# theEricMa/TriplaneTurbo

Hardware: AMD Instinct MI355X
Metric: rendered rays/sec (fwd+bwd) at 256x256 rays x 128 samples (higher is better)
Workload: dtype f32 (fp32-grade: exact 3-piece fp16 operand split, 6 x v_mfma_f32_32x32x16_f16 per k-step, fp32 accumulation)

## Files before the change

### include/tt_abi.h

```cpp
#ifndef TT_ABI_H
#define TT_ABI_H

#include <stdint.h>

#ifdef __cplusplus
extern "C" {
#endif

#define TT_ABI_VERSION 17
#define TT_CHANNELS 32
#define TT_HIDDEN 64

typedef enum {
    TT_OK = 0,
    TT_ERR_BAD_ARG = -1,
    TT_ERR_UNSUPPORTED = -2,
    TT_ERR_LAUNCH = -3,
    TT_ERR_DEVICE = -4
} tt_status;

typedef struct {
    const float* w1;
    const float* w2;
    const float* w3;
    const float* v1;
    const float* v2;
    const float* v3;
} tt_mlp_weights;

typedef struct {
    float* w1;
    float* w2;
    float* w3;
    float* v1;
    float* v2;
    float* v3;
} tt_mlp_grads;

typedef struct {
    int32_t n_prompts;
    int32_t views_per_prompt;
    int32_t plane_h, plane_w;
    int32_t rays_per_view;
    int32_t n_samples;
    int64_t n_rays;
    float radius;
    float sdf_bias_radius;
    float inv_std;
    float cos_anneal_ratio;
    float rgb_grad_shrink;
    int32_t flags;
    int32_t image_w;
    int32_t tile_sb;
    int32_t grad_copies;
    int32_t tile_chunk;
    float skip_eps_tex;
    float skip_eps_geo;
    const float* inv_std_dev;
    uint64_t* stats;
} tt_render_cfg;

#define TT_R_PER_SAMPLE 1
#define TT_R_EXACT_F32 2
#define TT_R_SPLIT2 32
#define TT_R_SPLIT3 64

#define TT_R_VOLSDF 128

#define TT_R_WGRAD_F32 4
#define TT_R_BWD_SOLO 8
#define TT_R_BWD_PAIR 16

#define TT_Q_NORMAL 1
#define TT_Q_TEX 2
#define TT_Q_EXACT_F32 4
#define TT_Q_SPLIT2 8
#define TT_Q_SPLIT3 16

const char* tt_strerror(int status);
int tt_abi_version(void);
const char* tt_source_hash(void);
int tt_debug_poison_queue(void* stream);

int tt_planes_pack(const float* space_cache, float* packed, int32_t n_prompts, int32_t plane_h, int32_t plane_w,
                   void* stream);
int tt_planes_unpack_grad(const float* grad_packed, float* grad_space_cache, int32_t n_prompts, int32_t plane_h,
                          int32_t plane_w, int32_t n_copies, void* stream);

int tt_query_points(const float* packed, const tt_mlp_weights* w, const float* points, int32_t n_batch,
                    int64_t n_points, int32_t n_prompts, int32_t views_per_prompt, int32_t plane_h, int32_t plane_w,
                    float radius, float sdf_bias_radius, int32_t flags, float* out_sdf, float* out_sdf_grad,
                    float* out_features, void* stream);

int tt_query_field(const float* packed, const tt_mlp_weights* w, const float* points, int32_t n_batch,
                   int64_t n_points, int32_t n_prompts, int32_t views_per_prompt, int32_t plane_h, int32_t plane_w,
                   float radius, float sdf_bias_radius, int32_t flags, float* out_sdf, float* out_deformation,
                   void* stream);

int tt_decode_rays(const float* packed, const tt_mlp_weights* w, const float* rays_o, const float* rays_d,
                   const float* t_starts, const float* t_ends, const tt_render_cfg* cfg, int32_t flags, float* sdf,
                   float* sdf_grad, float* features, void* stream);

enum tt_sample_placement { TT_PLACE_TT = 0, TT_PLACE_CENTER = 1 };
#define TT_PLACE_VOLSDF 0x100

int tt_sample_uniform(int64_t n_rays, int32_t n_samples, float near_plane, float far_plane, const float* jitter,
                      int32_t placement, float* t_starts, float* t_ends, void* stream);

int tt_sample_importance(const float* t_starts, const float* t_ends, const float* sdf, int64_t n_rays,
                         int32_t n_proposal, int32_t n_fine, float inv_std, const float* inv_std_dev,
                         float render_step_size, const float* u_jitter, int32_t placement, float* out_t_starts,
                         float* out_t_ends, void* stream);

int tt_render_fwd(const float* packed, const tt_mlp_weights* w, const float* rays_o, const float* rays_d,
                  const float* t_starts, const float* t_ends, const tt_render_cfg* cfg, float* opacity, float* depth,
                  float* rgb_fg, float* z_variance, float* normal_acc, float* weights, float* trans, float* sdf,
                  float* sdf_grad, float* features, void* stream);

int tt_render_fwd_h2mask(const float* packed, const tt_mlp_weights* w, const float* rays_o, const float* rays_d,
                         const float* t_starts, const float* t_ends, const tt_render_cfg* cfg, float* opacity,
                         float* depth, float* rgb_fg, float* z_variance, float* normal_acc, float* weights, float* trans,
                         float* sdf, float* sdf_grad, float* features, uint32_t* h2_mask, void* stream);

int tt_render_eval(const float* packed, const tt_mlp_weights* w, const float* rays_o, const float* rays_d,
                   const float* t_starts, const float* t_ends, const tt_render_cfg* cfg, float transmittance_eps,
                   float weight_eps, float* opacity, float* depth, float* rgb_fg, float* z_variance, float* normal_acc,
                   uint64_t* stats, void* stream);

int tt_march_fwd(const float* rays_d, const float* t_starts, const float* t_ends, const tt_render_cfg* cfg,
                 const float* sdf, const float* sdf_grad, const float* features, float* opacity, float* depth,
                 float* rgb_fg, float* z_variance, float* normal_acc, float* weights, float* trans, void* stream);

int tt_march_bwd(const float* rays_d, const float* t_starts, const float* t_ends, const tt_render_cfg* cfg,
                 const float* opacity, const float* depth, const float* trans, const float* sdf,
                 const float* sdf_grad, const float* features, const float* g_opacity, const float* g_depth,
                 const float* g_rgb_fg, const float* g_z_variance, const float* g_normal_acc, const float* g_weights,
                 const float* g_sdf, const float* g_sdf_grad, float* g_inv_std_rays, float* out_grad, void* stream);

int tt_render_bwd_geo(const float* packed, const tt_mlp_weights* w, const float* rays_o, const float* rays_d,
                      const float* t_starts, const float* t_ends, const tt_render_cfg* cfg, const float* opacity,
                      const float* depth, const float* trans, const float* sdf, const float* sdf_grad,
                      const float* features, const float* g_opacity, const float* g_depth, const float* g_rgb_fg,
                      const float* g_z_variance, const float* g_normal_acc, const float* g_weights,
                      const float* g_sdf, const float* g_sdf_grad, float* g_inv_std_rays, float* workspace,
                      float* grad_packed, const tt_mlp_grads* grads, void* stream);

int tt_render_bwd_geo_h2mask(const float* packed, const tt_mlp_weights* w, const float* rays_o, const float* rays_d,
                             const float* t_starts, const float* t_ends, const tt_render_cfg* cfg,
                             const float* opacity, const float* depth, const float* trans, const float* sdf,
                             const float* sdf_grad, const float* features, const float* g_opacity,
                             const float* g_depth, const float* g_rgb_fg, const float* g_z_variance,
                             const float* g_normal_acc, const float* g_weights, const float* g_sdf,
                             const float* g_sdf_grad, float* g_inv_std_rays, float* workspace, float* grad_packed,
                             const tt_mlp_grads* grads, const uint32_t* h2_mask, void* stream);

int tt_render_bwd_tex(const float* packed, const tt_mlp_weights* w, const float* rays_o, const float* rays_d,
                      const float* t_starts, const float* t_ends, const tt_render_cfg* cfg, const float* weights,
                      const float* features, const float* g_rgb_fg, const float* g_features, float* grad_packed,
                      const tt_mlp_grads* grads, void* stream);

int tt_points_bwd_geo(const float* packed, const tt_mlp_weights* w, const float* points, int32_t n_batch,
                      int64_t n_points, int32_t n_prompts, int32_t views_per_prompt, int32_t plane_h, int32_t plane_w,
                      float radius, float sdf_bias_radius, int32_t flags, const float* g_sdf, const float* g_sdf_grad,
                      float* workspace, float* grad_packed, const tt_mlp_grads* grads, void* stream);
int tt_points_bwd_tex(const float* packed, const tt_mlp_weights* w, const float* points, int32_t n_batch,
                      int64_t n_points, int32_t n_prompts, int32_t views_per_prompt, int32_t plane_h, int32_t plane_w,
                      float radius, int32_t plane_base, int32_t flags, const float* g_features, float* grad_packed,
                      const tt_mlp_grads* grads, void* stream);

int tt_points_bwd_x(const float* packed, const tt_mlp_weights* w, const float* points, int32_t n_batch,
                    int64_t n_points, int32_t n_prompts, int32_t views_per_prompt, int32_t plane_h, int32_t plane_w,
                    float radius, int32_t flags, const float* g_sdf, const float* g_sdf_grad, const float* g_features,
                    float* grad_points, void* stream);

typedef struct {
    int32_t n_levels;
    int32_t n_features_per_level;
    int32_t log2_hashmap_size;
    int32_t base_resolution;
    float per_level_scale;
} tt_hashgrid_cfg;
int64_t tt_hashgrid_n_params(const tt_hashgrid_cfg* cfg);
int tt_hashgrid_fwd(const float* x, int64_t n, const float* params, const tt_hashgrid_cfg* cfg, float* out,
                    void* stream);
int tt_hashgrid_bwd(const float* x, int64_t n, const float* g_out, const tt_hashgrid_cfg* cfg, float* grad_params,
                    void* stream);

int tt_patch_composite_fwd(const float* low, const float* patch, float* out, int32_t B, int32_t h, int32_t w, int32_t H,
                           int32_t W, int32_t C, int32_t PS, int32_t py, int32_t px, void* stream);
int tt_patch_composite_bwd(const float* g_out, float* g_low, float* g_patch, int32_t B, int32_t h, int32_t w, int32_t H,
                           int32_t W, int32_t C, int32_t PS, int32_t py, int32_t px, void* stream);

int tt_eikonal_fwd(const float* sdf_grad, int64_t n, float* loss, void* stream);
int tt_eikonal_bwd(const float* sdf_grad, const float* g_loss, int64_t n, float* g_sdf_grad, void* stream);

int tt_composite_fwd(const float* opacity, const float* depth, const float* rgb_fg, const float* normal_acc,
                     const float* bg, int32_t bg_stride, const float* camera_distances, const float* c2w, int64_t n_rays,
                     int32_t rays_per_view, int32_t mode, int32_t view_group, float* comp_rgb, float* disparity,
                     float* comp_normal, float* normal_cam_vis, float* normal_cam_vis_white, void* stream);
int tt_composite_bwd(const float* opacity, const float* depth, const float* rgb_fg, const float* normal_acc,
                     const float* bg, int32_t bg_stride, const float* camera_distances, const float* c2w, int64_t n_rays,
                     int32_t rays_per_view, int32_t mode, int32_t view_group, const float* g_comp_rgb,
                     const float* g_disparity, const float* g_comp_normal, const float* g_normal_cam_vis,
                     const float* g_normal_cam_vis_white, float* g_opacity, float* g_depth, float* g_rgb_fg,
                     float* g_normal_acc, float* g_bg, void* stream);

#define TT_DTYPE_F32 0
#define TT_DTYPE_F16 1
#define TT_DTYPE_F64 2
int tt_grid_sample_2d_grad2_typed(int32_t dtype, const void* grad2_grad_input, const void* grad2_grad_grid,
                                  const void* grad_output, const void* input, const void* grid, int32_t n, int32_t c,
                                  int32_t h, int32_t w, int64_t n_points_per_batch, int32_t padding_mode,
                                  int32_t align_corners, void* grad_grad_output, void* grad_input, void* grad_grid,
                                  void* stream);
int tt_grid_sample_2d_grad2(const float* grad2_grad_input, const float* grad2_grad_grid, const float* grad_output,
                            const float* input, const float* grid, int32_t n, int32_t c, int32_t h, int32_t w,
                            int64_t n_points_per_batch, int32_t padding_mode, int32_t align_corners,
                            float* grad_grad_output, float* grad_input, float* grad_grid, void* stream);

#define TT_MC_MAX_RES 512
int64_t tt_mc_workspace_bytes(int32_t res);
int tt_mc_count(const float* level, int32_t res, float isovalue, void* workspace, int32_t* out_totals, void* stream);
int tt_mc_emit(const float* level, const float* deformation, int32_t res, float isovalue, void* workspace, float* v_pos,
               int32_t* t_pos_idx, void* stream);
int tt_mc_bwd(const float* level, const float* deformation, int32_t res, float isovalue, void* workspace,
              const float* grad_v, float* grad_level, float* grad_deformation, void* stream);

int64_t tt_mt_workspace_bytes(int32_t n_edges, int32_t n_tets);
int tt_mt_count(const float* level, const int32_t* edges, const int32_t* tets, int32_t n_edges, int32_t n_tets,
                void* workspace, int32_t* out_totals, void* stream);
int tt_mt_emit(const float* pos, const float* level, const int32_t* edges, const int32_t* tet_edge, int32_t n_edges,
               int32_t n_tets, void* workspace, float* v_pos, int32_t* t_pos_idx, void* stream);
int tt_mt_bwd(const float* pos, const float* level, const int32_t* edges, const int32_t* vert_ptr,
              const int32_t* vert_col, int32_t n_vertices, int32_t n_edges, int32_t n_tets, void* workspace,
              const float* grad_v, float* grad_level, float* grad_pos, void* stream);

#define TT_RAST_MAX_TRIS (1 << 24)
int64_t tt_rast_workspace_bytes(int32_t B, int32_t T, int32_t H, int32_t W);
int tt_rast_fwd(const float* pos, const int32_t* tri, int32_t B, int32_t V, int32_t T, int32_t H, int32_t W,
                void* workspace, float* rast, void* stream);
int tt_rast_bwd(const float* pos, const int32_t* tri, const float* rast, const float* grad_rast, int32_t B, int32_t V,
                int32_t T, int32_t H, int32_t W, float* grad_pos, void* stream);
// ... 143 lines not shown
```

### triplaneturbo_amd/csrc/tt_backward.hip

```cpp
#include "tt_backward_common.h"

struct BwdGeoParams {
    const float* packed;
    MlpPtrs w;
    const float* rays_o;
    const float* rays_d;
    const float* t_starts;
    const float* t_ends;
    tt_render_cfg cfg;
    TileGeom geom;
    long long n_items;
    int* queue;
    const float* ws;
    const unsigned* h2_mask;
    int n_copies;
    float* grad_packed;
    MlpGradPtrs grads;
    unsigned long long* phase_cycles;
};

#define GEO_SCRATCH_FLOATS (2 * 64 * XS)
template <int PREC, bool FMASK>
struct GeoMap : LdsMap<PREC, LdsImage<64, 32>, LdsImage<64, 64, !(FMASK && PREC != PREC_F32)>, LdsRows<1, 64>,
                       LdsImage<32, 64>, LdsImage<64, 64>> {
// ... 177 lines not shown
                        wgrad16<64, 32>(accW1, Xs, Ys, i, hi);
                    } else {
                        stage_rows<64>(Xs, a1, i, hi);
                        stage_rows<32>(Ys, u, i, hi);
                        wgrad<64, 32>(accW1, Xs, Ys, i, hi);
                    }
                }
                TT_PHASE(7);
                float t1[32];
                mvx<PREC>(L, typename G::W1{}, qb, t1, i, hi);
#pragma unroll
                for (int r = 0; r < 32; ++r) t1[r] = h1[r] > 0.f ? t1[r] : 0.f;
                float v[32];
#pragma unroll
                for (int r = 0; r < 32; ++r) v[r] = fmaf(sbar * u1, h1[r], t1[r]);
                TT_PHASE(4);
                if (do_wgrad) {
                    if (WG16) {
                        stage_rows16_mask<64>(Xs, m2p, i, hi);
                        stage_rows16<64>(Ys, v, i, hi, sV);
                        wgrad16_mask<64, 64>(accW2, Xs, Ys, i, hi);
                    } else {
                        stage_rows_mask<64>(Xs, h2, i, hi);
                        stage_rows<64>(Ys, v, i, hi);
                        wgrad<64, 64>(accW2, Xs, Ys, i, hi);
                    }
                }
                TT_PHASE(8);
                if (region && !TT_DBG(cfg.flags, TT_DBG_NO_SCATTER)) {
                    scatter_clear<EXACT>(Xs, lane);
                    float* Qs = Xs + SCATTER_M_FLOATS;
                    TT_PHASE(9);
                    const int tex0 = (int)(pofs / TT_C);
                    auto corners = [&](int pl, PlaneRefs& refs) {
                        Corners c;
                        float coef[4];
                        geo_corner_coefs(pl, H, W, X, Y, Z, rvalid, sbar, gbx, gby, gbz, ju, jv, c, coef);
                        int aoff[4];
#pragma unroll
                        for (int q4 = 0; q4 < 4; ++q4) aoff[q4] = tex0 + (int)(pl * HW) + c.off[q4];
                        refs = plane_refs<!EXACT>(coef, aoff, c.hs, hi);
                    };
#ifdef TT_TUNING
                    unsigned long long* const sc_st = ph_acc + 14;
#else
                    unsigned long long* const sc_st = nullptr;
#endif
                    const ScatterQ<EXACT> sq{Qs, tags, i, hi};
                    if (one)
                        scatter_one_plane<EXACT>(grad_out, grad_bytes, sq, Xs, Qs + 32 * 33,
                                                 single_plane_index(pmask), corners, q, uq, sc_st);
                    else
                        scatter_planes<EXACT>(grad_out, grad_bytes, sq, Xs, Qs + 32 * 33, corners, [&](int) { return q; }, uq, sc_st);
                    TT_PHASE(10);
                }
            }
        }
    }
#ifdef TT_TUNING
    TT_PHASE(11);
    if (p.phase_cycles && lane == 0)
        for (int k = 0; k < 20; ++k) atomicAdd(p.phase_cycles + 20 + k, ph_acc[k]);
#endif
    __syncthreads();
    int parity = 0;
    flush_wgrad_reduced<64, 32>(L, parity, accW1, p.grads.w1, wave_in_blk, lane, 1.f / sA1, 1.f / sU);
    flush_d_reduced<64, 64>(L, parity, accW2, p.w.w2, p.w.w3, p.grads.w2, p.grads.w3, wave_in_blk, lane, 1.f / sV);
    tile_stats_flush(st);
}

#ifdef TT_TUNING
unsigned long long* g_phase_cycles = nullptr;
extern "C" int tt_tuning_phase_cycles(unsigned long long* out40) {
    if (!g_phase_cycles) {
        if (hipMalloc((void**)&g_phase_cycles, 40 * sizeof(unsigned long long)) != hipSuccess) return -4;
        if (hipMemset(g_phase_cycles, 0, 40 * sizeof(unsigned long long)) != hipSuccess) return -4;
    }
    if (hipDeviceSynchronize() != hipSuccess) return -4;
    if (out40 && hipMemcpy(out40, g_phase_cycles, 40 * sizeof(unsigned long long), hipMemcpyDeviceToHost) != hipSuccess)
        return -4;
    return hipMemset(g_phase_cycles, 0, 40 * sizeof(unsigned long long)) == hipSuccess ? 0 : -4;
}
#endif
static void launch_bwd_geo(const BwdGeoParams& p0, long long blocks, hipStream_t s) {
    BwdGeoParams p = p0;
#ifdef TT_TUNING
    p.phase_cycles = g_phase_cycles;
#else
    p.phase_cycles = nullptr;
#endif
    if (use_wg16(p.cfg)) {
        unsigned* bnd = reinterpret_cast<unsigned*>(p.queue) + TT_SLOT_BOUNDS;
        launch_planes_bound(p.packed, p.cfg, 0, bnd + TT_BOUND_PLANES, s);
        const long long n = p.cfg.n_rays * p.cfg.n_samples;
        hipLaunchKernelGGL(k_absmax4, dim3(absmax_blocks(n), 1), dim3(256), 0, s, reinterpret_cast<const f32x4*>(p.ws), n, n,
                           bnd + TT_BOUND_UP0, bnd + TT_BOUND_UP1);
    }
    tt_dispatch_prec(tt_prec_of_r(p.cfg.flags), [&](auto P) {
        constexpr int PREC = decltype(P)::value;
        const dim3 grid((unsigned)blocks), block(256);
        if (p.cfg.stats && p.h2_mask)
            hipLaunchKernelGGL((k_decode_bwd_geo<PREC, true, true>), grid, block, 0, s, p);
        else if (p.cfg.stats)
            hipLaunchKernelGGL((k_decode_bwd_geo<PREC, true>), grid, block, 0, s, p);
        else if (p.h2_mask)
            hipLaunchKernelGGL((k_decode_bwd_geo<PREC, false, true>), grid, block, 0, s, p);
        else
            hipLaunchKernelGGL((k_decode_bwd_geo<PREC>), grid, block, 0, s, p);
    });
}

static int render_bwd_geo(const float* packed, const tt_mlp_weights* w, const float* rays_o, const float* rays_d,
                          const float* t_starts, const float* t_ends, const tt_render_cfg* cfg, const float* opacity,
                          const float* depth, const float* trans, const float* sdf, const float* sdf_grad,
                          const float* features, const float* g_opacity, const float* g_depth, const float* g_rgb_fg,
                          const float* g_z_variance, const float* g_normal_acc, const float* g_weights,
                          const float* g_sdf, const float* g_sdf_grad, float* g_inv_std_rays, float* workspace,
                          float* grad_packed, const tt_mlp_grads* grads, const uint32_t* h2_mask, void* stream) {
    int st = tt_validate_cfg(cfg);
    if (st != TT_OK) return st;
    if (!packed || !w || !rays_o || !rays_d || !t_starts || !t_ends || !opacity || !depth || !trans || !sdf ||
        !sdf_grad || !features || !workspace || !grad_packed || !grads)
        return TT_ERR_BAD_ARG;
    if (!w->w1 || !w->w2 || !w->w3 || !grads->w1 || !grads->w2 || !grads->w3) return TT_ERR_BAD_ARG;
    if (grad_buffer_too_large(cfg)) return TT_ERR_UNSUPPORTED;
    int cus = tt_num_cus();
    if (cus <= 0) return TT_ERR_DEVICE;
    hipStream_t s = (hipStream_t)stream;
    st = tt_launch_march_bwd(rays_d, t_starts, t_ends, cfg, sdf, sdf_grad, features, trans, opacity, depth, g_opacity,
                             g_depth, g_rgb_fg, g_z_variance, g_normal_acc, g_weights, g_sdf, g_sdf_grad, g_inv_std_rays,
                             workspace, s);
    if (st != TT_OK) return st;
    BwdGeoParams p;
    tt_fill_rays(p, packed, w, rays_o, rays_d, t_starts, t_ends, *cfg);
    p.cfg.flags |= debug_flags();
    p.ws = workspace;
    p.h2_mask = h2_mask;
    p.grad_packed = grad_packed;
    p.n_copies = cfg->grad_copies > 0 ? cfg->grad_copies : 1;
    p.grads = to_gptrs(grads);
    st = tt_plan_queue(cfg, 4LL * cus, s, &p.geom, &p.n_items, &p.queue);
    if (st != TT_OK) return st;
    launch_bwd_geo(p, tt_persistent_blocks(p.n_items, cus, 4), s);
    return tt_check_launch();
}

extern "C" int tt_render_bwd_geo(const float* packed, const tt_mlp_weights* w, const float* rays_o,
                                 const float* rays_d, const float* t_starts, const float* t_ends,
                                 const tt_render_cfg* cfg, const float* opacity, const float* depth,
                                 const float* trans, const float* sdf, const float* sdf_grad, const float* features,
                                 const float* g_opacity, const float* g_depth, const float* g_rgb_fg,
                                 const float* g_z_variance, const float* g_normal_acc, const float* g_weights,
                                 const float* g_sdf, const float* g_sdf_grad, float* g_inv_std_rays, float* workspace,
                                 float* grad_packed, const tt_mlp_grads* grads, void* stream) {
    return render_bwd_geo(packed, w, rays_o, rays_d, t_starts, t_ends, cfg, opacity, depth, trans, sdf, sdf_grad, features,
                          g_opacity, g_depth, g_rgb_fg, g_z_variance, g_normal_acc, g_weights, g_sdf, g_sdf_grad,
                          g_inv_std_rays, workspace, grad_packed, grads, nullptr, stream);
}

extern "C" int tt_render_bwd_geo_h2mask(const float* packed, const tt_mlp_weights* w, const float* rays_o,
                                        const float* rays_d, const float* t_starts, const float* t_ends,
                                        const tt_render_cfg* cfg, const float* opacity, const float* depth,
                                        const float* trans, const float* sdf, const float* sdf_grad,
                                        const float* features, const float* g_opacity, const float* g_depth,
                                        const float* g_rgb_fg, const float* g_z_variance, const float* g_normal_acc,
                                        const float* g_weights, const float* g_sdf, const float* g_sdf_grad,
                                        float* g_inv_std_rays, float* workspace, float* grad_packed,
                                        const tt_mlp_grads* grads, const uint32_t* h2_mask, void* stream) {
    if (!h2_mask) return TT_ERR_BAD_ARG;
    return render_bwd_geo(packed, w, rays_o, rays_d, t_starts, t_ends, cfg, opacity, depth, trans, sdf, sdf_grad, features,
                          g_opacity, g_depth, g_rgb_fg, g_z_variance, g_normal_acc, g_weights, g_sdf, g_sdf_grad,
                          g_inv_std_rays, workspace, grad_packed, grads, h2_mask, stream);
}

__global__ void k_interleave_ws(const float* __restrict__ g_sdf, const float* __restrict__ g_sdf_grad,
                                float* __restrict__ ws, long long n) {
    const long long i = (long long)blockIdx.x * blockDim.x + threadIdx.x;
    if (i >= n) return;
    f32x4 o = {g_sdf ? g_sdf[i] : 0.f, g_sdf_grad ? g_sdf_grad[i * 3 + 0] : 0.f,
               g_sdf_grad ? g_sdf_grad[i * 3 + 1] : 0.f, g_sdf_grad ? g_sdf_grad[i * 3 + 2] : 0.f};
    *reinterpret_cast<f32x4*>(ws + i * 4) = o;
}

extern "C" int tt_points_bwd_geo(const float* packed, const tt_mlp_weights* w, const float* points, int32_t n_batch,
                                 int64_t n_points, int32_t n_prompts, int32_t views_per_prompt, int32_t plane_h,
                                 int32_t plane_w, float radius, float sdf_bias_radius, int32_t flags,
                                 const float* g_sdf, const float* g_sdf_grad, float* workspace, float* grad_packed,
                                 const tt_mlp_grads* grads, void* stream) {
    tt_render_cfg cfg;
    int st = points_cfg(&cfg, n_batch, n_points, n_prompts, views_per_prompt, plane_h, plane_w, radius,
                        sdf_bias_radius, 1, flags);
    if (st != TT_OK) return st;
    if (grad_buffer_too_large(&cfg)) return TT_ERR_UNSUPPORTED;
    if (!packed || !w || !points || !workspace || !grad_packed || !grads || (!g_sdf && !g_sdf_grad))
        return TT_ERR_BAD_ARG;
    if (!w->w1 || !w->w2 || !w->w3 || !grads->w1 || !grads->w2 || !grads->w3) return TT_ERR_BAD_ARG;
    int cus = tt_num_cus();
    if (cus <= 0) return TT_ERR_DEVICE;
    hipStream_t s = (hipStream_t)stream;
    const long long n = cfg.n_rays;
    hipLaunchKernelGGL(k_interleave_ws, dim3((unsigned)((n + 255) / 256)), dim3(256), 0, s, g_sdf, g_sdf_grad,
                       workspace, n);
    st = tt_check_launch();
    if (st != TT_OK) return st;
    BwdGeoParams p;
    tt_fill_rays(p, packed, w, points, nullptr, nullptr, nullptr, cfg);
    p.ws = workspace;
    p.h2_mask = nullptr;
    p.grad_packed = grad_packed;
    p.n_copies = 1;
    p.grads = to_gptrs(grads);
    st = tt_plan_queue(&cfg, 4LL * cus, s, &p.geom, &p.n_items, &p.queue);
    if (st != TT_OK) return st;
    launch_bwd_geo(p, tt_persistent_blocks(p.n_items, cus, 4), s);
    return tt_check_launch();
}
```

### triplaneturbo_amd/csrc/tt_backward_common.h

```cpp
#pragma once
#include "tt_device.h"
#include "tt_mfma16.h"
#include "tt_alpha.h"
#include "tt_launch.h"
#include <type_traits>

typedef int i32x4 __attribute__((ext_vector_type(4)));

#ifdef TT_TUNING
#define TT_PHASE(k)                                              \
    do {                                                         \
        __builtin_amdgcn_sched_barrier(0);                       \
        const unsigned long long t_now = __builtin_amdgcn_s_memtime(); \
        ph_acc[k] += t_now - ph_t;                               \
        ph_t = t_now;                                            \
        __builtin_amdgcn_sched_barrier(0);                       \
    } while (0)
#else
#define TT_PHASE(k) \
    do {            \
    } while (0)
#endif
#define XS 36

// ... 697 lines not shown
    float* const Qs = sq.Qs;
    const int i = sq.i, hi = sq.hi;
    const ScatterCtx cx = scatter_ctx<EXACT>(grad, grad_bytes, sq, Ls);
    typename std::conditional<EXACT, ScA32, ScA16>::type A;
    typename std::conditional<EXACT, ScB32, ScB16>::type B;
    PlaneRefs rc;
    corners(pl, rc);
    sq.hand_over(pl, tile, factor, rc.qs);
    const Sc2State sc = sc2_claim_rank(rc, cx.htab, cx.ctag, cx.cdump, cx.dummy, cx.lane, st);
    scatter_lost(rc, sc.l0, sc.l1, Qs, Ls, cx.grsrc, i, hi, [&]() { sq.stage_q(pl, tile); });
    m_store<EXACT>(M, sc2_row_a(sc.rx0), cx.mc, rc.c0);
    m_store<EXACT>(M, sc2_row_a(sc.rx1), cx.mc, rc.c1);
    const bool pass_b = sc.n > 64;
    f32x16 acc0, acc1;
    sc2_load_a(M, i, hi, sc.n, A);
    m_zero<EXACT>(M, sc2_row_a(sc.rx0), cx.mc);
    m_zero<EXACT>(M, sc2_row_a(sc.rx1), cx.mc);
    if (pass_b) {
        m_store<EXACT>(M, sc2_row_b(sc.rx0), cx.mc, rc.c0);
        m_store<EXACT>(M, sc2_row_b(sc.rx1), cx.mc, rc.c1);
    }
    sq.load_b(pl, tile, B);
    sc2_split_b(B);
    sc2_gemm(A, B, sc.n, acc0, acc1);
    if (pass_b) {
        sc2_flush(acc0, acc1, cx.ctag, 64, cx.grsrc, cx.lane_b, hi);
        sc2_load_a(M, i, hi, sc.n - 64, A);
        m_zero<EXACT>(M, sc2_row_b(sc.rx0), cx.mc);
        m_zero<EXACT>(M, sc2_row_b(sc.rx1), cx.mc);
        sc2_gemm(A, B, sc.n - 64, acc0, acc1);
        sc2_flush(acc0, acc1, cx.ctag + 64, sc.n - 64, cx.grsrc, cx.lane_b, hi);
    } else {
        sc2_flush(acc0, acc1, cx.ctag, sc.n, cx.grsrc, cx.lane_b, hi);
    }
}

struct BwdTexParams {
    const float* packed;
    MlpPtrs w;
    const float* rays_o;
    const float* rays_d;
    const float* t_starts;
    const float* t_ends;
    tt_render_cfg cfg;
    const float* weights;
    const float* features;
    const float* g_rgb;
    const float* g_features;
    TileGeom geom;
    long long n_items;
    int* queue;
    int n_copies;
    float* grad_packed;
    MlpGradPtrs grads;
    unsigned long long* phase_cycles;
};

static inline bool grad_buffer_too_large(const tt_render_cfg* cfg) {
    return (long long)cfg->n_prompts * 6 * cfg->plane_h * cfg->plane_w * TT_C * 4 >= (1LL << 32) - 256;
}

#ifdef TT_TUNING
extern unsigned long long* g_phase_cycles;
#endif
static __global__ __launch_bounds__(256) void k_absmax4(const f32x4* __restrict__ x, long long seg4, long long seg_stride4,
                                                 unsigned* __restrict__ out0, unsigned* __restrict__ out1) {
    const f32x4* seg = x + (long long)blockIdx.y * seg_stride4;
    const long long stride = (long long)gridDim.x * blockDim.x;
    float m0 = 0.f, m1 = 0.f;
    long long e = (long long)blockIdx.x * blockDim.x + threadIdx.x;
    for (; e + 3 * stride < seg4; e += 4 * stride) {
        const f32x4 a = seg[e], b = seg[e + stride], c = seg[e + 2 * stride], d = seg[e + 3 * stride];
        m0 = fmaxf(fmaxf(m0, __builtin_fabsf(a[0])), fmaxf(__builtin_fabsf(b[0]), fmaxf(__builtin_fabsf(c[0]), __builtin_fabsf(d[0]))));
#pragma unroll
        for (int k = 1; k < 4; ++k)
            m1 = fmaxf(fmaxf(m1, __builtin_fabsf(a[k])), fmaxf(__builtin_fabsf(b[k]), fmaxf(__builtin_fabsf(c[k]), __builtin_fabsf(d[k]))));
    }
    for (; e < seg4; e += stride) {
        const f32x4 v = seg[e];
        m0 = fmaxf(m0, __builtin_fabsf(v[0]));
        m1 = fmaxf(m1, fmaxf(__builtin_fabsf(v[1]), fmaxf(__builtin_fabsf(v[2]), __builtin_fabsf(v[3]))));
    }
    if (!out1) m0 = fmaxf(m0, m1);
    __shared__ unsigned w[2];
    if (threadIdx.x < 2) w[threadIdx.x] = 0u;
    __syncthreads();
    for (int o = 32; o > 0; o >>= 1) {
        m0 = fmaxf(m0, __shfl_xor(m0, o));
        m1 = fmaxf(m1, __shfl_xor(m1, o));
    }
    if ((threadIdx.x & 63) == 0) {
        atomicMax(&w[0], __builtin_bit_cast(unsigned, m0));
        atomicMax(&w[1], __builtin_bit_cast(unsigned, m1));
    }
    __syncthreads();
    if (threadIdx.x == 0) {
        if (w[0] > __hip_atomic_load(out0, __ATOMIC_RELAXED, __HIP_MEMORY_SCOPE_AGENT)) atomicMax(out0, w[0]);
        if (out1 && w[1] > __hip_atomic_load(out1, __ATOMIC_RELAXED, __HIP_MEMORY_SCOPE_AGENT)) atomicMax(out1, w[1]);
    }
}
static __global__ __launch_bounds__(256) void k_absmax1(const float* __restrict__ x, long long n, unsigned* __restrict__ out) {
    float m = 0.f;
    for (long long e = (long long)blockIdx.x * blockDim.x + threadIdx.x; e < n; e += (long long)gridDim.x * blockDim.x)
        m = fmaxf(m, __builtin_fabsf(x[e]));
    for (int o = 32; o > 0; o >>= 1) m = fmaxf(m, __shfl_xor(m, o));
    __shared__ unsigned w;
    if (threadIdx.x == 0) w = 0u;
    __syncthreads();
    if ((threadIdx.x & 63) == 0) atomicMax(&w, __builtin_bit_cast(unsigned, m));
    __syncthreads();
    if (threadIdx.x == 0 && w > __hip_atomic_load(out, __ATOMIC_RELAXED, __HIP_MEMORY_SCOPE_AGENT)) atomicMax(out, w);
}
static inline unsigned absmax_blocks(long long n) {
    long long b = (n + 256 * 8 - 1) / (256 * 8);
    return (unsigned)(b < 1 ? 1 : (b > 1024 ? 1024 : b));
}
static inline void launch_planes_bound(const float* packed, const tt_render_cfg& cfg, int first_plane, unsigned* out,
                                hipStream_t s) {
    const long long hw4 = (long long)cfg.plane_h * cfg.plane_w * TT_C / 4;
    hipLaunchKernelGGL(k_absmax4, dim3(absmax_blocks(3 * hw4), (unsigned)cfg.n_prompts), dim3(256), 0, s,
                       reinterpret_cast<const f32x4*>(packed) + first_plane * hw4, 3 * hw4, 6 * hw4, out,
                       (unsigned*)nullptr);
}

static inline bool use_wg16(const tt_render_cfg& cfg) { return !(cfg.flags & TT_R_EXACT_F32); }

static inline int points_cfg(tt_render_cfg* c, int32_t n_batch, int64_t n_points, int32_t n_prompts,
                      int32_t views_per_prompt, int32_t plane_h, int32_t plane_w, float radius, float sdf_bias_radius,
                      int32_t grad_copies, int32_t q_flags) {
    if (!tt_points_counts_ok(n_batch, n_points, n_prompts, views_per_prompt, q_flags) || n_points > 0x7fffffffLL)
        return TT_ERR_BAD_ARG;
    c->n_prompts = n_prompts;
    c->views_per_prompt = views_per_prompt;
    c->plane_h = plane_h;
    c->plane_w = plane_w;
    c->rays_per_view = (int32_t)n_points;
    c->n_samples = 1;
    c->n_rays = (int64_t)n_batch * n_points;
    c->radius = radius;
    c->sdf_bias_radius = sdf_bias_radius;
    c->inv_std = 1.f;
    c->inv_std_dev = nullptr;
    c->stats = nullptr;
    c->cos_anneal_ratio = 1.f;
    c->rgb_grad_shrink = 1.f;
    c->flags = (q_flags & TT_Q_EXACT_F32) ? TT_R_EXACT_F32 : ((q_flags & TT_Q_SPLIT2) ? TT_R_SPLIT2 : 0);
    c->image_w = 0;
    c->tile_sb = 1;
    c->tile_chunk = 0;
    c->grad_copies = grad_copies;
    c->skip_eps_tex = 0.f;
    c->skip_eps_geo = 0.f;
    return tt_validate_cfg(c);
}
```

### triplaneturbo_amd/csrc/tt_backward_tex.hip

```cpp
#include "tt_backward_common.h"

#define TEX_SCRATCH_FLOATS (128 * XS)
template <int PREC>
struct TexMap : LdsMap<PREC, LdsImage<64, 96>, LdsImage<64, 64>, LdsRows<3, 64>, LdsImage<96, 64, PREC != PREC_S3>,
                       LdsImage<64, 64, PREC != PREC_S3>> {
    static constexpr bool COPIES = PREC != PREC_S3;
    typedef typename TexMap::template at<0> V1;
    typedef typename TexMap::template at<1> V2;
    typedef typename TexMap::template at<2> V3;
    typedef typename TexMap::template at<3> V1T;
    typedef typename TexMap::template at<4> V2T;
};
__device__ __forceinline__ float uniform_f(float v) {
    return __builtin_bit_cast(float, __builtin_amdgcn_readfirstlane(__builtin_bit_cast(int, v)));
}

template <int PREC, bool STATS = false>
__global__ __launch_bounds__(256, 1) void k_decode_bwd_tex(BwdTexParams p) {
    constexpr bool EXACT = PREC == PREC_F32;
    constexpr bool WG16 = !EXACT;
    typedef TexMap<PREC> F;
    constexpr int NT = PrecNT<PREC>::value, WF = F::FLOATS;
    __shared__ __attribute__((aligned(16))) float Lt[WF + 4 * (TEX_SCRATCH_FLOATS + SCATTER_TAG_INTS)];
    stage_weights<PREC>(Lt, typename F::V1{}, p.w.v1);
// ... 251 lines not shown
                wgrad16<64, 64>(accV2, Xs, Xs + 64 * XS, i, hi);
            } else {
                stage_rows<64>(Xs, k2, i, hi);
                stage_rows<64>(Xs + 64 * XS, k1, i, hi);
                wgrad<64, 64>(accV2, Xs, Xs + 64 * XS, i, hi);
            }
            TT_PHASE(8);
        }
        if (region && !TT_DBG(cfg.flags, TT_DBG_NO_SCATTER)) {
            float* M = Xs;
            float* Es = Xs + (EXACT ? 65 * XS : SCATTER_M_FLOATS);
            scatter_clear<EXACT>(M, lane);
            const int tex0 = (int)(pofs / TT_C);
            float eb[48], ueb = 1.f;
            if constexpr (EXACT)
                mvtx_copy<PREC>(Lt, typename F::V1T{}, typename F::V1{}, kb1, eb, i, hi);
            else if constexpr (F::COPIES)
                mvtx_copy<PREC, true, true>(Lt, typename F::V1T{}, typename F::V1{}, kb1, eb, i, hi, 1.f, &ueb);
            else
                mvtx<PREC, true, true>(Lt, typename F::V1{}, kb1, eb, i, hi, 1.f, &ueb);
            TT_PHASE(9);
            auto corners = [&](int pl, PlaneRefs& refs) {
                Corners c;
                corners_setup(PLANE_U(pl, X, Y, Z), PLANE_V(pl, X, Y, Z), H, W, valid, c);
                int aoff[4];
#pragma unroll
                for (int q4 = 0; q4 < 4; ++q4)
                    aoff[q4] = tex0 + (int)((3 + pl) * HW) + c.off[q4];
                refs = plane_refs<!EXACT>(c.w, aoff, c.hs, hi);
            };
#ifdef TT_TUNING
            unsigned long long* const sc_st = scat_st;
#else
            unsigned long long* const sc_st = nullptr;
#endif
            const ScatterQ<EXACT> sq{Es, tags, i, hi};
            if (one) {
                float eb1[16];
#pragma unroll
                for (int r = 0; r < 16; ++r) eb1[r] = pl1 == 0 ? eb[r] : (pl1 == 1 ? eb[16 + r] : eb[32 + r]);
                scatter_one_plane<EXACT>(grad_out, grad_bytes, sq, M, Es + 32 * 33, pl1, corners, eb1, ueb, sc_st);
                TT_PHASE(10);
                continue;
            }
            scatter_planes<EXACT>(grad_out, grad_bytes, sq, M, Es + 32 * 33, corners, [&](int pl) { return eb + 16 * pl; }, ueb,
                                  sc_st);
            TT_PHASE(10);
        }
      }
    }
#ifdef TT_TUNING
    TT_PHASE(11);
    ph_acc[15] = scat_st[0];
    ph_acc[16] = scat_st[1];
    if (p.phase_cycles && lane == 0)
        for (int k = 0; k < 20; ++k) atomicAdd(p.phase_cycles + k, ph_acc[k]);
#endif
    __syncthreads();
    int parity = 0;
    {
        const float u1 = 1.f / sKB1, u2 = 1.f / sE;
#pragma unroll
        for (int m = 0; m < 2; ++m) {
            float* const base = p.grads.v1 + (32 * m) * 96 + i;
            flush_tile_reduced(Lt, parity, accV1a[m][0], wave_in_blk, lane, u1, u2,
                               [&](int r) { return base + LIDX(r, hi) * 96; });
            parity ^= 1;
            flush_tile_reduced(Lt, parity, accV1a[m][1], wave_in_blk, lane, u1, u2,
                               [&](int r) { return base + LIDX(r, hi) * 96 + 32; });
            parity ^= 1;
            flush_tile_reduced(Lt, parity, accV1b[m][0], wave_in_blk, lane, u1, u2,
                               [&](int r) { return base + LIDX(r, hi) * 96 + 64; });
            parity ^= 1;
        }
    }
    flush_wgrad_reduced<64, 64>(Lt, parity, accV2, p.grads.v2, wave_in_blk, lane, 1.f / sK2B, 1.f / sK1);
#pragma unroll
    for (int h2 = 0; h2 < 2; ++h2)
#pragma unroll
        for (int o = 0; o < 3; ++o) atomicAdd(p.grads.v3 + o * 64 + 32 * h2 + i, accV3[h2][o]);
    tile_stats_flush(st);
}

static void launch_bwd_tex(const BwdTexParams& p0, long long blocks, hipStream_t s) {
    BwdTexParams p = p0;
#ifdef TT_TUNING
    p.phase_cycles = g_phase_cycles;
#else
    p.phase_cycles = nullptr;
#endif
    if (use_wg16(p.cfg)) {
        unsigned* bnd = reinterpret_cast<unsigned*>(p.queue) + TT_SLOT_BOUNDS;
        launch_planes_bound(p.packed, p.cfg, 3, bnd + TT_BOUND_PLANES, s);
        if (p.g_rgb)
            hipLaunchKernelGGL(k_absmax1, dim3(absmax_blocks(p.cfg.n_rays * 3)), dim3(256), 0, s, p.g_rgb,
                               (long long)p.cfg.n_rays * 3, bnd + TT_BOUND_UP0);
        if (p.g_features) {
            const long long n = p.cfg.n_rays * p.cfg.n_samples * 3;
            hipLaunchKernelGGL(k_absmax1, dim3(absmax_blocks(n)), dim3(256), 0, s, p.g_features, n, bnd + TT_BOUND_UP1);
        }
    }
    tt_dispatch_prec(tt_prec_of_r(p.cfg.flags), [&](auto P) {
        constexpr int PREC = decltype(P)::value;
        if (p.cfg.stats)
            hipLaunchKernelGGL((k_decode_bwd_tex<PREC, true>), dim3((unsigned)blocks), dim3(256), 0, s, p);
        else
            hipLaunchKernelGGL((k_decode_bwd_tex<PREC>), dim3((unsigned)blocks), dim3(256), 0, s, p);
    });
}

extern "C" int tt_render_bwd_tex(const float* packed, const tt_mlp_weights* w, const float* rays_o,
                                 const float* rays_d, const float* t_starts, const float* t_ends,
                                 const tt_render_cfg* cfg, const float* weights, const float* features,
                                 const float* g_rgb_fg, const float* g_features, float* grad_packed,
                                 const tt_mlp_grads* grads, void* stream) {
    int st = tt_validate_cfg(cfg);
    if (st != TT_OK) return st;
    if (!packed || !w || !rays_o || !rays_d || !t_starts || !t_ends || !weights || !features || !grad_packed ||
        !grads)
        return TT_ERR_BAD_ARG;
    if (!w->v1 || !w->v2 || !w->v3 || !grads->v1 || !grads->v2 || !grads->v3) return TT_ERR_BAD_ARG;
    if (grad_buffer_too_large(cfg)) return TT_ERR_UNSUPPORTED;
    int cus = tt_num_cus();
    if (cus <= 0) return TT_ERR_DEVICE;
    hipStream_t s = (hipStream_t)stream;
    BwdTexParams p;
    tt_fill_rays(p, packed, w, rays_o, rays_d, t_starts, t_ends, *cfg);
    p.cfg.flags |= debug_flags();
    p.weights = weights;
    p.features = features;
    p.g_rgb = g_rgb_fg;
    p.g_features = g_features;
    p.grad_packed = grad_packed;
    p.n_copies = cfg->grad_copies > 0 ? cfg->grad_copies : 1;
    p.grads = to_gptrs(grads);
    st = tt_plan_queue(cfg, 4LL * cus, s, &p.geom, &p.n_items, &p.queue, 12);
    if (st != TT_OK) return st;
    launch_bwd_tex(p, tt_persistent_blocks(p.n_items, cus, 4), s);
    return tt_check_launch();
}

extern "C" int tt_points_bwd_tex(const float* packed, const tt_mlp_weights* w, const float* points, int32_t n_batch,
                                 int64_t n_points, int32_t n_prompts, int32_t views_per_prompt, int32_t plane_h,
                                 int32_t plane_w, float radius, int32_t plane_base, int32_t flags,
                                 const float* g_features, float* grad_packed, const tt_mlp_grads* grads,
                                 void* stream) {
    tt_render_cfg cfg;
    int st = points_cfg(&cfg, n_batch, n_points, n_prompts, views_per_prompt, plane_h, plane_w, radius, 0.5f, 1,
                        flags);
    if (st != TT_OK) return st;
    if (grad_buffer_too_large(&cfg)) return TT_ERR_UNSUPPORTED;
    if (!packed || !w || !points || !g_features || !grad_packed || !grads) return TT_ERR_BAD_ARG;
    if (!w->v1 || !w->v2 || !w->v3 || !grads->v1 || !grads->v2 || !grads->v3) return TT_ERR_BAD_ARG;
    if (plane_base != 0 && plane_base != 3) return TT_ERR_BAD_ARG;
    int cus = tt_num_cus();
    if (cus <= 0) return TT_ERR_DEVICE;
    const ptrdiff_t shift = (ptrdiff_t)(plane_base - 3) * plane_h * plane_w * TT_C;
    hipStream_t s = (hipStream_t)stream;
    BwdTexParams p;
    tt_fill_rays(p, packed + shift, w, points, nullptr, nullptr, nullptr, cfg);
    p.weights = nullptr;
    p.features = nullptr;
    p.g_rgb = nullptr;
    p.g_features = g_features;
    p.grad_packed = grad_packed + shift;
    p.n_copies = 1;
    p.grads = to_gptrs(grads);
    st = tt_plan_queue(&cfg, 4LL * cus, s, &p.geom, &p.n_items, &p.queue);
    if (st != TT_OK) return st;
    launch_bwd_tex(p, tt_persistent_blocks(p.n_items, cus, 4), s);
    return tt_check_launch();
}
```

### triplaneturbo_amd/csrc/tt_device.h

```cpp
#pragma once
#include <hip/hip_runtime.h>
#include <stdint.h>

typedef float f32x16 __attribute__((ext_vector_type(16)));
typedef float f32x4 __attribute__((ext_vector_type(4)));

#ifdef TT_TUNING
#define TT_DBG(flags, bit) (((flags) & (bit)) != 0)
#else
#define TT_DBG(flags, bit) false
#endif
#define TT_DBG_NO_SCATTER 0x100
#define TT_DBG_NO_WGRAD 0x200
#define TT_DBG_NO_GATHER 0x400
#define TT_DBG_NO_MLP 0x800
#define TT_DBG_NO_STORE 0x1000
#define TT_DBG_NO_ATOMICS 0x2000

#define TT_C 32
#define TT_TILE 32

#define LIDX(r, hi) (((r) & 3) + 8 * ((r) >> 2) + 4 * (hi))

#include "tt_mask.h"

struct MlpPtrs {
    const float* w1;
    const float* w2;
    const float* w3;
    const float* v1;
    const float* v2;
    const float* v3;
};

__device__ __forceinline__ void lds_load_matrix(float* dst, const float* __restrict__ src, int rows, int cols,
                                                int stride) {
    for (int e = threadIdx.x; e < rows * cols; e += blockDim.x) {
        int r = e / cols, c = e - r * cols;
        dst[r * stride + c] = src[e];
    }
}

template <int NOUT, int NIN>
__device__ __forceinline__ void mv_fwd(const float* Wl, const float (&x)[NIN / 2], float (&y)[NOUT / 2], int i,
                                       int hi) {
    constexpr int MT = NOUT / 32;
    f32x16 acc[MT];
    f32x4 a_cur[MT], a_nxt[MT];
    const float* row = Wl + i * (NIN + 4) + 4 * hi;
#pragma unroll
    for (int m = 0; m < MT; ++m) {
        acc[m] = f32x16{0.f, 0.f, 0.f, 0.f, 0.f, 0.f, 0.f, 0.f, 0.f, 0.f, 0.f, 0.f, 0.f, 0.f, 0.f, 0.f};
        a_cur[m] = *reinterpret_cast<const f32x4*>(row + 32 * m * (NIN + 4));
    }
#pragma unroll
    for (int g = 0; g < NIN / 8; ++g) {
        if (g + 1 < NIN / 8) {
#pragma unroll
            for (int m = 0; m < MT; ++m)
                a_nxt[m] = *reinterpret_cast<const f32x4*>(row + 32 * m * (NIN + 4) + 8 * (g + 1));
        }
#pragma unroll
        for (int k = 0; k < 4; ++k)
#pragma unroll
            for (int m = 0; m < MT; ++m)
                acc[m] = __builtin_amdgcn_mfma_f32_32x32x2f32(a_cur[m][k], x[4 * g + k], acc[m], 0, 0, 0);
#pragma unroll
        for (int m = 0; m < MT; ++m) a_cur[m] = a_nxt[m];
    }
#pragma unroll
    for (int m = 0; m < MT; ++m)
#pragma unroll
        for (int k = 0; k < 16; ++k) y[16 * m + k] = acc[m][k];
}

template <int NOUT, int NIN, int NG>
__device__ __forceinline__ void mv_fwd_cols(const float* Wl, const float (&x)[4 * NG], int g0, float (&y)[NOUT / 2], int i,
                                            int hi) {
    constexpr int MT = NOUT / 32;
    f32x16 acc[MT];
    const float* row = Wl + i * (NIN + 4) + 4 * hi + 8 * g0;
#pragma unroll
    for (int m = 0; m < MT; ++m)
        acc[m] = f32x16{0.f, 0.f, 0.f, 0.f, 0.f, 0.f, 0.f, 0.f, 0.f, 0.f, 0.f, 0.f, 0.f, 0.f, 0.f, 0.f};
#pragma unroll
    for (int g = 0; g < NG; ++g) {
        f32x4 a[MT];
#pragma unroll
        for (int m = 0; m < MT; ++m) a[m] = *reinterpret_cast<const f32x4*>(row + 32 * m * (NIN + 4) + 8 * g);
#pragma unroll
        for (int k = 0; k < 4; ++k)
#pragma unroll
            for (int m = 0; m < MT; ++m)
                acc[m] = __builtin_amdgcn_mfma_f32_32x32x2f32(a[m][k], x[4 * g + k], acc[m], 0, 0, 0);
    }
#pragma unroll
    for (int m = 0; m < MT; ++m)
#pragma unroll
        for (int k = 0; k < 16; ++k) y[16 * m + k] = acc[m][k];
}

template <int NOUT, int NIN, int STRIDE = NOUT + 4>
__device__ __forceinline__ void mv_bwd(const float* Wl, const float (&x)[NIN / 2], float (&y)[NOUT / 2], int i,
                                       int hi) {
    constexpr int MT = NOUT / 32;
    const float* base = Wl + 4 * hi * STRIDE + i;
    if (MT == 1) {
// ... 648 lines not shown
```

### triplaneturbo_amd/csrc/tt_forward.hip

```cpp
#ifndef TT_MV16_FENCE
#define TT_MV16_FENCE 1
#endif
#include "tt_device.h"
#include "tt_mfma16.h"
#include "tt_alpha.h"
#include "tt_launch.h"

__device__ __forceinline__ void rot_dst(int k3, int y, int x, int H, int W, int& h, int& w) {
    if (k3 == 0) {
        h = x;
        w = y;
    } else if (k3 == 1) {
        h = H - 1 - y;
        w = W - 1 - x;
    } else {
        h = x;
        w = H - 1 - y;
    }
}

template <bool UNPACK>
__global__ __launch_bounds__(256) void k_planes_pack(const float* __restrict__ src, float* __restrict__ dst, int H,
                                                     int W, int n_copies, size_t copy_stride) {
    extern __shared__ float tile[];
    const int y = blockIdx.x, plane = blockIdx.y;
    const int k3 = plane % 3;
    const size_t HW = (size_t)H * W;
    const float* nchw_c = (UNPACK ? dst : src) + (size_t)plane * TT_C * HW;
    float* nchw = const_cast<float*>(nchw_c);
    const float* nhwc_c = (UNPACK ? src : dst) + (size_t)plane * HW * TT_C;
    float* nhwc = const_cast<float*>(nhwc_c);
    const int ws = W + 1;
    if (!UNPACK) {
        for (int e = threadIdx.x; e < TT_C * W; e += blockDim.x) {
            int c = e / W, x = e - c * W;
            tile[c * ws + x] = nchw[(size_t)c * HW + (size_t)y * W + x];
        }
        __syncthreads();
        for (int e = threadIdx.x; e < TT_C * W; e += blockDim.x) {
            int x = e >> 5, c = e & 31, h, w;
            rot_dst(k3, y, x, H, W, h, w);
            nhwc[((size_t)h * W + w) * TT_C + c] = tile[c * ws + x];
        }
    } else {
        for (int e = threadIdx.x; e < TT_C * W; e += blockDim.x) {
            int x = e >> 5, c = e & 31, h, w;
            rot_dst(k3, y, x, H, W, h, w);
            const size_t o = ((size_t)h * W + w) * TT_C + c;
            float acc = nhwc[o];
            for (int k = 1; k < n_copies; ++k) acc += nhwc[o + (size_t)k * copy_stride];
            tile[c * ws + x] = acc;
        }
        __syncthreads();
        for (int e = threadIdx.x; e < TT_C * W; e += blockDim.x) {
            int c = e / W, x = e - c * W;
            nchw[(size_t)c * HW + (size_t)y * W + x] = tile[c * ws + x];
        }
    }
}

__host__ __device__ inline int pack4_row_stride(int W) { return W + (36 - W % 32) % 32; }
template <bool UNPACK>
__global__ __launch_bounds__(256) void k_planes_pack4(const float* __restrict__ src, float* __restrict__ dst, int H,
                                                      int W, int n_copies, size_t copy_stride) {
    extern __shared__ __attribute__((aligned(16))) float tile[];
    const int y = blockIdx.x, plane = blockIdx.y;
    const int k3 = plane % 3;
    const size_t HW = (size_t)H * W;
    const float* nchw_c = (UNPACK ? dst : src) + (size_t)plane * TT_C * HW + (size_t)y * W;
    float* nchw = const_cast<float*>(nchw_c);
    const float* nhwc_c = (UNPACK ? src : dst) + (size_t)plane * HW * TT_C;
    float* nhwc = const_cast<float*>(nhwc_c);
    const int RS = pack4_row_stride(W), W4 = W >> 2;
    const int c_lane = threadIdx.x & 31, x4_0 = threadIdx.x >> 5;
    if (!UNPACK) {
        for (int e4 = threadIdx.x; e4 < TT_C * W4; e4 += 256) {
            const int c = e4 / W4, x4 = e4 - c * W4;
            *reinterpret_cast<f32x4*>(tile + c * RS + 4 * x4) =
                *reinterpret_cast<const f32x4*>(nchw_c + (size_t)c * HW + 4 * x4);
        }
        __syncthreads();
        for (int x4 = x4_0; x4 < W4; x4 += 8) {
            const f32x4 v = *reinterpret_cast<const f32x4*>(tile + c_lane * RS + 4 * x4);
#pragma unroll
            for (int j = 0; j < 4; ++j) {
                int h, w;
                rot_dst(k3, y, 4 * x4 + j, H, W, h, w);
                nhwc[((size_t)h * W + w) * TT_C + c_lane] = v[j];
            }
        }
    } else {
        for (int x4 = x4_0; x4 < W4; x4 += 8) {
            f32x4 v;
#pragma unroll
            for (int j = 0; j < 4; ++j) {
                int h, w;
                rot_dst(k3, y, 4 * x4 + j, H, W, h, w);
                const size_t o = ((size_t)h * W + w) * TT_C + c_lane;
                float acc = nhwc_c[o];
                for (int k = 1; k < n_copies; ++k) acc += nhwc_c[o + (size_t)k * copy_stride];
                v[j] = acc;
            }
            *reinterpret_cast<f32x4*>(tile + c_lane * RS + 4 * x4) = v;
        }
        __syncthreads();
        for (int e4 = threadIdx.x; e4 < TT_C * W4; e4 += 256) {
            const int c = e4 / W4, x4 = e4 - c * W4;
            *reinterpret_cast<f32x4*>(nchw + (size_t)c * HW + 4 * x4) =
                *reinterpret_cast<const f32x4*>(tile + c * RS + 4 * x4);
        }
    }
}

template <int PREC>
using FwdMap = DecodeMap<PREC, 96>;

struct DecodeCfg {
    const float* planes;
    unsigned tex0;
    float* T;
    int H, W;
    float radius;
    float ju, jv;
    int dbg;
    TileStats st = {nullptr};
};


template <int PREC>
__device__ __forceinline__ void decode_tex_fwd(const float* L, const DecodeCfg& dc, float X, float Y, float Z,
                                               bool valid, int i, int hi, float (&c)[3]) {
    typedef FwdMap<PREC> F;
    c[0] = c[1] = c[2] = 0.f;
    float e[48];
    unsigned pmask;
    bool any = gather_tex_cp(dc.planes, dc.tex0, dc.H, dc.W, X, Y, Z, valid, 32 * hi + i, dc.T, e, pmask);
    if (TT_DBG(dc.dbg, TT_DBG_NO_MLP)) {
        float t = 0.f;
#pragma unroll
        for (int r = 0; r < 48; ++r) t += e[r];
        c[0] = c[1] = c[2] = t;
    } else if (__any(any)) {
        float k1[32], k2[32], u1, u2;
        if (single_plane(pmask)) {
            tile_stat(dc.st, TT_STAT_SINGLE);
            float e1[16];
            live_block16(e, e1);
            mvx_plane<PREC, true>(L, typename F::V1{}, e1, single_plane_index(pmask), k1, i, hi, &u1);
        } else {
            mvx<PREC, true>(L, typename F::V1{}, e, k1, i, hi, 1.f, &u1);
        }
#pragma unroll
        for (int r = 0; r < 32; ++r) k1[r] = fmaxf(k1[r], 0.f);
        mvx<PREC, true>(L, typename F::V2{}, k1, k2, i, hi, u1, &u2);
#pragma unroll
        for (int r = 0; r < 32; ++r) k2[r] = fmaxf(k2[r], 0.f);
#pragma unroll
        for (int o = 0; o < 3; ++o) c[o] = dot_lds<64>(lds_at(L, typename F::V3{}) + 64 * o, k2, hi) * u2;
    }
}

__device__ __forceinline__ unsigned sign_mask32(const float (&h)[32]) {
    unsigned m = 0u;
#pragma unroll
    for (int g = 3; g >= 0; --g)
        asm("v_cmp_lt_f32 vcc, 0, %8\n\tv_addc_co_u32 %0, vcc, %0, %0, vcc\n\t"
            "v_cmp_lt_f32 vcc, 0, %7\n\tv_addc_co_u32 %0, vcc, %0, %0, vcc\n\t"
            "v_cmp_lt_f32 vcc, 0, %6\n\tv_addc_co_u32 %0, vcc, %0, %0, vcc\n\t"
            "v_cmp_lt_f32 vcc, 0, %5\n\tv_addc_co_u32 %0, vcc, %0, %0, vcc\n\t"
            "v_cmp_lt_f32 vcc, 0, %4\n\tv_addc_co_u32 %0, vcc, %0, %0, vcc\n\t"
            "v_cmp_lt_f32 vcc, 0, %3\n\tv_addc_co_u32 %0, vcc, %0, %0, vcc\n\t"
            "v_cmp_lt_f32 vcc, 0, %2\n\tv_addc_co_u32 %0, vcc, %0, %0, vcc\n\t"
            "v_cmp_lt_f32 vcc, 0, %1\n\tv_addc_co_u32 %0, vcc, %0, %0, vcc"
// ... 391 lines not shown
            }
            const float X = scale_coord(px, dc.radius), Y = scale_coord(py, dc.radius), Z = scale_coord(pz, dc.radius);
            const float livef = ray_okf * (__builtin_fabsf(T) < p.eps_T ? 0.f : 1.f);
            const bool live = livef != 0.f;
            {
                float s0, gq[3];
                decode_geo_fwd<true, PREC>(L, dc, X, Y, Z, live, i, hi, s0, gq);
                ++n_geo;
                float nrm;
                long long rr = ray;
                asm volatile("" : "+v"(rr));
                const float* ro = p.rays_o + rr * 3;
                const float* rd = p.rays_d + rr * 3;
                const float ts = p.t_starts[rr * S + si], te = p.t_ends[rr * S + si];
                dt = te - ts;
                const float ox = ro[0], oy = ro[1], oz = ro[2];
                const float dx = rd[0], dy = rd[1], dz = rd[2];
                sample_position(ox, oy, oz, dx, dy, dz, ts, te, tm, px, py, pz);
                sdf = s0 + sphere_bias(px, py, pz, cfg.sdf_bias_radius, nrm);
                const float gx = gq[0] + px / nrm, gy = gq[1] + py / nrm, gz = gq[2] + pz / nrm;
                const float gn = fmaxf(sqrtf(gx * gx + gy * gy + gz * gz), 1e-12f);
                const float ign = rcp_(gn);
                ux = gx * ign, uy = gy * ign, uz = gz * ign;
                cosv = dx * ux + dy * uy + dz * uz;
            }
            float alpha = (cfg.flags & TT_R_VOLSDF) ? volsdf_alpha_terms(sdf, dt, kstd).alpha
                                                    : neus_alpha_terms(sdf, cosv, dt, kstd, cfg.cos_anneal_ratio).alpha;
            if (!live) alpha = 0.f;
            const float wgt = alpha * T;
            T *= 1.f - alpha;
            acc0 = fmaf(wgt, lof, acc0);
            acc1 = fmaf(wgt * lof, tm, acc1);
            acc2 = fmaf(wgt * lof * tm, tm, acc2);
            acc3 = fmaf(wgt, hi ? uz : ux, acc3);
            acc4 = fmaf(wgt * lof, uy, acc4);
            const bool want_tex = __builtin_fabsf(wgt) > p.eps_w;
            if (__any(want_tex)) {
                float c[3];
                if constexpr (PREC == PREC_F32) {
                    long long rr = ray;
                    asm volatile("" : "+v"(rr));
                    const float* ro = p.rays_o + rr * 3;
                    const float* rd = p.rays_d + rr * 3;
                    float tm2, qx, qy, qz;
                    sample_position(ro[0], ro[1], ro[2], rd[0], rd[1], rd[2], p.t_starts[rr * S + si], p.t_ends[rr * S + si], tm2,
                                    qx, qy, qz);
                    decode_tex_fwd<PREC>(L, dc, scale_coord(qx, dc.radius), scale_coord(qy, dc.radius),
                                         scale_coord(qz, dc.radius), want_tex, i, hi, c);
                } else {
                    decode_tex_fwd<PREC>(L, dc, X, Y, Z, want_tex, i, hi, c);
                }
                ++n_tex;
                if (want_tex) {
                    const float wh = wgt * hif;
                    acc0 = fmaf(wh, sigmoid_(c[0]) * 1.002f - 0.001f, acc0);
                    acc1 = fmaf(wh, sigmoid_(c[1]) * 1.002f - 0.001f, acc1);
                    acc2 = fmaf(wh, sigmoid_(c[2]) * 1.002f - 0.001f, acc2);
                }
            }
            if (p.eps_T > 0.f && !__any(ray_okf * (__builtin_fabsf(T) < p.eps_T ? 0.f : 1.f) != 0.f)) break;
        }
        if (ray_ok) {
            if (hi == 0) {
                const float op = acc0, dep = acc1, wt2 = acc2;
                p.opacity[ray] = op;
                p.depth[ray] = dep;
                p.z_var[ray] = wt2 - 2.f * dep * dep + dep * dep * op;
                p.nacc[ray * 3 + 0] = acc3;
                p.nacc[ray * 3 + 1] = acc4;
            } else {
                p.rgb_fg[ray * 3 + 0] = acc0;
                p.rgb_fg[ray * 3 + 1] = acc1;
                p.rgb_fg[ray * 3 + 2] = acc2;
                p.nacc[ray * 3 + 2] = acc3;
            }
        }
    }
    if (p.stats && lane == 0) {
        atomicAdd(p.stats + 0, n_geo);
        atomicAdd(p.stats + 1, n_tex);
    }
}

extern "C" int tt_planes_pack(const float* space_cache, float* packed, int32_t n_prompts, int32_t plane_h,
                              int32_t plane_w, void* stream) {
    if (!space_cache || !packed || n_prompts <= 0 || plane_h <= 0 || plane_w <= 0) return TT_ERR_BAD_ARG;
    if (plane_h != plane_w) return TT_ERR_UNSUPPORTED;
    dim3 grid(plane_h, n_prompts * 6);
    if (plane_w % 4 == 0 && ((uintptr_t)space_cache & 15) == 0) {
        size_t lds = (size_t)TT_C * pack4_row_stride(plane_w) * sizeof(float);
        hipLaunchKernelGGL(k_planes_pack4<false>, grid, dim3(256), lds, (hipStream_t)stream, space_cache, packed,
                           plane_h, plane_w, 1, (size_t)0);
    } else {
        size_t lds = (size_t)TT_C * (plane_w + 1) * sizeof(float);
        hipLaunchKernelGGL(k_planes_pack<false>, grid, dim3(256), lds, (hipStream_t)stream, space_cache, packed,
                           plane_h, plane_w, 1, (size_t)0);
    }
    return tt_check_launch();
}

extern "C" int tt_planes_unpack_grad(const float* grad_packed, float* grad_space_cache, int32_t n_prompts,
                                     int32_t plane_h, int32_t plane_w, int32_t n_copies, void* stream) {
    if (!grad_packed || !grad_space_cache || n_prompts <= 0 || plane_h <= 0 || plane_w <= 0 || n_copies <= 0)
        return TT_ERR_BAD_ARG;
    if (plane_h != plane_w) return TT_ERR_UNSUPPORTED;
    dim3 grid(plane_h, n_prompts * 6);
    const size_t copy_stride = (size_t)n_prompts * 6 * plane_h * plane_w * TT_C;
    if (plane_w % 4 == 0 && ((uintptr_t)grad_space_cache & 15) == 0) {
        size_t lds = (size_t)TT_C * pack4_row_stride(plane_w) * sizeof(float);
        hipLaunchKernelGGL(k_planes_pack4<true>, grid, dim3(256), lds, (hipStream_t)stream, grad_packed,
                           grad_space_cache, plane_h, plane_w, n_copies, copy_stride);
    } else {
        size_t lds = (size_t)TT_C * (plane_w + 1) * sizeof(float);
        hipLaunchKernelGGL(k_planes_pack<true>, grid, dim3(256), lds, (hipStream_t)stream, grad_packed,
                           grad_space_cache, plane_h, plane_w, n_copies, copy_stride);
    }
    return tt_check_launch();
}

extern "C" int tt_query_points(const float* packed, const tt_mlp_weights* w, const float* points, int32_t n_batch,
                               int64_t n_points, int32_t n_prompts, int32_t views_per_prompt, int32_t plane_h,
                               int32_t plane_w, float radius, float sdf_bias_radius, int32_t flags, float* out_sdf,
                               float* out_sdf_grad, float* out_features, void* stream) {
    if (!packed || !w || !points) return TT_ERR_BAD_ARG;
    const int st = tt_validate_points(n_batch, n_points, n_prompts, views_per_prompt, plane_h, plane_w, radius, flags);
    if (st != TT_OK) return st;
    const bool need_n = (flags & TT_Q_NORMAL) != 0, need_t = (flags & TT_Q_TEX) != 0;
    if (!w->w1 || !w->w2 || !w->w3 || (need_t && (!w->v1 || !w->v2 || !w->v3))) return TT_ERR_BAD_ARG;
    QueryParams p;
    tt_fill_points(p, packed, w, points, n_batch, n_points, views_per_prompt, plane_h, plane_w, radius);
    p.bias_radius = sdf_bias_radius;
    p.out_sdf = out_sdf;
    p.out_grad = out_sdf_grad;
    p.out_feat = out_features;
    const int cus = tt_num_cus();
    if (cus <= 0) return TT_ERR_DEVICE;
    const dim3 grid = tt_point_blocks(n_points, n_batch, DECODE_THREADS / 64, cus);
    tt_dispatch(tt_prec_of_q(flags), need_n, need_t, [&](auto P, auto N, auto T) {
        hipLaunchKernelGGL((k_query_points<decltype(N)::value, decltype(T)::value, decltype(P)::value>), grid,
                           dim3(DECODE_THREADS), 0, (hipStream_t)stream, p);
    });
    return tt_check_launch();
}

bool tt_planes_too_large(long long n_prompts, int plane_h, int plane_w) {
    return n_prompts * 6 * plane_h * plane_w * TT_C * 4 >= (1LL << 32);
}

int tt_validate_cfg(const tt_render_cfg* cfg) {
    if (!cfg) return TT_ERR_BAD_ARG;
    if (cfg->n_prompts <= 0 || cfg->views_per_prompt <= 0 || cfg->rays_per_view <= 0 || cfg->n_samples <= 0 ||
        cfg->n_rays <= 0)
        return TT_ERR_BAD_ARG;
    if (cfg->n_rays != (int64_t)cfg->n_prompts * cfg->views_per_prompt * cfg->rays_per_view) return TT_ERR_BAD_ARG;
    if (cfg->plane_h <= 0 || cfg->plane_h != cfg->plane_w) return TT_ERR_UNSUPPORTED;
    if (tt_planes_too_large(cfg->n_prompts, cfg->plane_h, cfg->plane_w)) return TT_ERR_UNSUPPORTED;
    if (!(cfg->radius > 0.f) || (!cfg->inv_std_dev && !(cfg->inv_std > 0.f))) return TT_ERR_BAD_ARG;
    if (cfg->flags < 0) return TT_ERR_BAD_ARG;
    {
        const int pbits = cfg->flags & (TT_R_EXACT_F32 | TT_R_SPLIT2 | TT_R_SPLIT3);
        if (pbits & (pbits - 1)) return TT_ERR_BAD_ARG;
    }
    if (cfg->flags & (TT_R_BWD_PAIR | TT_R_WGRAD_F32)) return TT_ERR_UNSUPPORTED;
    if (!(cfg->skip_eps_tex >= 0.f) || !(cfg->skip_eps_geo >= 0.f)) return TT_ERR_BAD_ARG;
    return TT_OK;
}

long long tt_make_geom(const tt_render_cfg* cfg, long long wave_slots, TileGeom* g, int default_order,
                       int steps_per_item, int min_items_per_slot) {
    g->n_rays = cfg->n_rays;
    g->rays_per_view = cfg->rays_per_view;
    g->n_samples = cfg->n_samples;
    g->image_w = 0;
    g->image_h = 0;
    g->bpr = g->bpv = 0;
    int sb = cfg->tile_sb;
#ifdef TT_TUNING
    if (const char* e = getenv("TT_SB")) sb = atoi(e);
#endif
    if (!(sb == 1 || sb == 2 || sb == 4 || sb == 8 || sb == 16 || sb == 32)) sb = 2;
    while (sb > 1 && sb > cfg->n_samples) sb /= 2;
    g->sb = sb;
    static const int BW[6] = {8, 4, 4, 2, 2, 1}, BH[6] = {4, 4, 2, 2, 1, 1};
    int l2 = 0;
    while ((1 << l2) < sb) ++l2;
    g->bw = BW[l2];
    g->bh = BH[l2];
    const int rb = 32 / sb;
    long long n_blocks;
    if (cfg->image_w > 0 && cfg->rays_per_view % cfg->image_w == 0) {
        g->image_w = cfg->image_w;
        g->image_h = cfg->rays_per_view / cfg->image_w;
        g->bpr = (g->image_w + g->bw - 1) / g->bw;
        g->bpv = g->bpr * ((g->image_h + g->bh - 1) / g->bh);
        n_blocks = (cfg->n_rays / cfg->rays_per_view) * g->bpv;
    } else {
        n_blocks = (cfg->n_rays + rb - 1) / rb;
    }
// ... 188 lines not shown
```

### triplaneturbo_amd/csrc/tt_host.cpp

```cpp
#include "tt_host.h"

#include <stdio.h>
#include <stdlib.h>

#include <algorithm>
#include <cmath>
#include <mutex>
#include <vector>

extern "C" const char* tt_strerror(int status) {
    switch (status) {
        case TT_OK: return "ok";
        case TT_ERR_BAD_ARG: return "bad argument (null pointer, non-positive size or inconsistent shape)";
        case TT_ERR_UNSUPPORTED: return "unsupported configuration (planes must be square, C=32, hidden=64)";
        case TT_ERR_LAUNCH: return "HIP kernel launch failed";
        case TT_ERR_DEVICE: return "HIP device query failed / not a gfx950 device";
        default: return "unknown tt_status";
    }
}

extern "C" int tt_abi_version(void) { return TT_ABI_VERSION; }

#ifndef TT_SOURCE_HASH_STR
#define TT_SOURCE_HASH_STR "unknown"
#endif
static const char k_source_hash[] = "TT_SOURCE_HASH=" TT_SOURCE_HASH_STR;
extern "C" const char* tt_source_hash(void) { return k_source_hash + 15; }

int tt_check_launch() { return hipGetLastError() == hipSuccess ? TT_OK : TT_ERR_LAUNCH; }

int tt_num_cus() {
    int dev = 0, cus = 0;
    if (hipGetDevice(&dev) != hipSuccess) return -1;
    if (hipDeviceGetAttribute(&cus, hipDeviceAttributeMultiprocessorCount, dev) != hipSuccess) return -1;
    return cus;
}

namespace {
constexpr int kMaxDevices = 64, kStreams = 256, kRing = 4, kGraphSlots = 4096, kSlotInts = TT_SLOT_INTS;
struct DeviceScratch {
    int* base = nullptr;
    hipStream_t streams[kStreams];
    unsigned next[kStreams];
    int n_streams = 0;
    int evict = 0;
    unsigned n_graph = 0;
    bool evict_warned = false;
};
DeviceScratch g_scratch[kMaxDevices];
std::mutex g_scratch_mu;
}

__global__ void k_zero_slot(int* slot) { slot[threadIdx.x] = 0; }

int* tt_queue_counters(hipStream_t stream) {
    int dev = 0;
    if (hipGetDevice(&dev) != hipSuccess || dev < 0 || dev >= kMaxDevices) return nullptr;
    hipStreamCaptureStatus cap = hipStreamCaptureStatusNone;
    if (hipStreamIsCapturing(stream, &cap) != hipSuccess) return nullptr;
    int* slot = nullptr;
    {
        std::lock_guard<std::mutex> lk(g_scratch_mu);
        DeviceScratch& d = g_scratch[dev];
        if (!d.base) {
            if (cap != hipStreamCaptureStatusNone) return nullptr;
            void* ptr = nullptr;
            if (hipMalloc(&ptr, (size_t)(kStreams * kRing + kGraphSlots) * kSlotInts * sizeof(int)) != hipSuccess)
                return nullptr;
            d.base = static_cast<int*>(ptr);
        }
        if (cap != hipStreamCaptureStatusNone) {
            if (d.n_graph == kGraphSlots)
                fprintf(stderr, "libtt_hip: %d launches captured on device %d; work-queue slots of captured launches are "
                                "reused from now on -- graphs holding more than %d launches in total must not replay "
                                "concurrently\n", kGraphSlots, dev, kGraphSlots);
            slot = d.base + (size_t)(kStreams * kRing + (d.n_graph++ % kGraphSlots)) * kSlotInts;
        } else {
            int k = 0;
            while (k < d.n_streams && d.streams[k] != stream) ++k;
            if (k == d.n_streams) {
                if (d.n_streams == kStreams) {
                    if (!d.evict_warned) {
                        d.evict_warned = true;
                        fprintf(stderr, "libtt_hip: more than %d streams have launched on device %d; the oldest stream's "
                                        "work-queue ring is recycled (safe unless more than %d streams have launches in "
                                        "flight at once)\n", kStreams, dev, kStreams);
                    }
                    k = d.evict;
                    d.evict = (d.evict + 1) % kStreams;
                } else {
                    ++d.n_streams;
                }
                d.streams[k] = stream;
                d.next[k] = 0;
            }
            slot = d.base + (size_t)(k * kRing + (d.next[k]++ % kRing)) * kSlotInts;
        }
    }
    hipLaunchKernelGGL(k_zero_slot, dim3(1), dim3(kSlotInts), 0, stream, slot);
    if (hipGetLastError() != hipSuccess) return nullptr;
    return slot;
}

extern "C" int tt_debug_poison_queue(void* stream) {
    for (int r = 0; r < kRing; ++r) {
        int* slot = tt_queue_counters((hipStream_t)stream);
        if (!slot) return TT_ERR_DEVICE;
        if (hipMemsetAsync(slot, 0x7f, kSlotInts * sizeof(int), (hipStream_t)stream) != hipSuccess) return TT_ERR_DEVICE;
    }
    return TT_OK;
}

namespace {
struct UvShelf {
    std::vector<double> w, h;
    std::vector<long long> bw, bh;
    std::vector<int> order;
    int N = 0, pad = 0;

    bool pack(double s, int32_t* off) {
        const int C = (int)w.size();
        for (int c = 0; c < C; ++c) {
            bw[c] = (long long)std::ceil(w[c] * s) + 2ll * pad + 1;
            bh[c] = (long long)std::ceil(h[c] * s) + 2ll * pad + 1;
            order[c] = c;
        }
        std::sort(order.begin(), order.end(), [&](int a, int b) {
            if (bh[a] != bh[b]) return bh[a] > bh[b];
            if (bw[a] != bw[b]) return bw[a] > bw[b];
            return a < b;
        });
        long long x = 0, y = 0, shelf = 0;
        for (int c : order) {
            if (bw[c] > N || bh[c] > N) return false;
            if (x + bw[c] > N) {
                y += shelf;
                x = 0;
                shelf = 0;
            }
            if (shelf == 0) shelf = bh[c];
            if (y + shelf > N) return false;
            if (off) {
                off[2 * c] = (int32_t)x;
                off[2 * c + 1] = (int32_t)y;
            }
            x += bw[c];
        }
        return true;
    }
};
}

extern "C" int tt_uv_pack(const float* chart_box, int32_t C, int32_t N, int32_t padding, int32_t* offsets,
                          float* scale) {
    if (C < 1 || C > TT_UV_MAX_FACES || N < 1 || N > TT_UV_MAX_TEX || padding < 0 || padding > TT_UV_MAX_PADDING)
        return TT_ERR_BAD_ARG;
    if (!chart_box || !offsets || !scale) return TT_ERR_BAD_ARG;
    UvShelf p;
    p.w.resize(C);
    p.h.resize(C);
    p.bw.resize(C);
    p.bh.resize(C);
    p.order.resize(C);
    p.N = N;
    p.pad = padding;
    double m = 0.0;
    for (int c = 0; c < C; ++c) {
        p.w[c] = (double)chart_box[4 * c + 2] - (double)chart_box[4 * c];
        p.h[c] = (double)chart_box[4 * c + 3] - (double)chart_box[4 * c + 1];
        if (!(p.w[c] >= 0.0 && p.h[c] >= 0.0 && p.w[c] < 1e30 && p.h[c] < 1e30)) return TT_ERR_BAD_ARG;
        m = std::max(m, std::max(p.w[c], p.h[c]));
    }
    if (m == 0.0) {
        if (!p.pack(1.0, offsets)) return TT_ERR_UNSUPPORTED;
        *scale = 1.0f;
        return TT_OK;
    }
    double lo = 0.0, hi = (double)(float)(((double)N - 2.0 * padding) / m);
    if (!(hi > 0.0)) return TT_ERR_UNSUPPORTED;
    for (int it = 0; it < 200 && hi - lo > TT_UV_PACK_REL_PREC * hi; ++it) {
        const double mid = (double)(float)(0.5 * (lo + hi));
        if (!(mid > lo && mid < hi)) break;
        if (p.pack(mid, nullptr)) lo = mid;
        else hi = mid;
    }
    if (!(lo > 0.0) || !p.pack(lo, offsets)) return TT_ERR_UNSUPPORTED;
// ... 4 lines not shown
```

### triplaneturbo_amd/csrc/tt_host.h

```cpp
#pragma once
#include <hip/hip_runtime.h>

#include <type_traits>

#include "../../include/tt_abi.h"

int tt_check_launch();
int tt_num_cus();
int tt_validate_cfg(const tt_render_cfg* cfg);
bool tt_planes_too_large(long long n_prompts, int plane_h, int plane_w);

enum { PREC_S2 = 0, PREC_F32 = 1, PREC_S3 = 2 };
static inline int tt_prec_of_r(int flags) {
    return (flags & TT_R_EXACT_F32) ? PREC_F32 : ((flags & TT_R_SPLIT2) ? PREC_S2 : PREC_S3);
}
static inline int tt_prec_of_q(int flags) {
    return (flags & TT_Q_EXACT_F32) ? PREC_F32 : ((flags & TT_Q_SPLIT2) ? PREC_S2 : PREC_S3);
}
static inline bool tt_qflags_ok(int flags) {
    const int pbits = flags & (TT_Q_EXACT_F32 | TT_Q_SPLIT2 | TT_Q_SPLIT3);
    return (pbits & (pbits - 1)) == 0;
}

template <class F>
static inline void tt_dispatch_prec(int prec, F&& f) {
    if (prec == PREC_F32)
        f(std::integral_constant<int, PREC_F32>{});
    else if (prec == PREC_S3)
        f(std::integral_constant<int, PREC_S3>{});
    else
        f(std::integral_constant<int, PREC_S2>{});
}
template <class F>
static inline void tt_dispatch(int prec, bool need_n, bool need_t, F&& f) {
    if (need_n && need_t)
        tt_dispatch_prec(prec, [&](auto P) { f(P, std::true_type{}, std::true_type{}); });
    else if (need_n)
        tt_dispatch_prec(prec, [&](auto P) { f(P, std::true_type{}, std::false_type{}); });
    else if (need_t)
        tt_dispatch_prec(prec, [&](auto P) { f(P, std::false_type{}, std::true_type{}); });
    else
        tt_dispatch_prec(prec, [&](auto P) { f(P, std::false_type{}, std::false_type{}); });
}

static inline long long tt_persistent_blocks(long long n_items, int cus, int waves_per_block) {
    long long blocks = cus;
    const long long need = (n_items + waves_per_block - 1) / waves_per_block;
    if (blocks > need) blocks = need;
    return (blocks + 7) / 8 * 8;
}

static inline bool tt_points_counts_ok(int32_t n_batch, int64_t n_points, int32_t n_prompts, int32_t views_per_prompt,
                                       int32_t q_flags) {
    return n_batch > 0 && n_points > 0 && n_prompts > 0 && views_per_prompt > 0 &&
           (int64_t)n_prompts * views_per_prompt == n_batch && tt_qflags_ok(q_flags);
}
static inline int tt_validate_points(int32_t n_batch, int64_t n_points, int32_t n_prompts, int32_t views_per_prompt,
                                     int32_t plane_h, int32_t plane_w, float radius, int32_t q_flags) {
    if (!tt_points_counts_ok(n_batch, n_points, n_prompts, views_per_prompt, q_flags) || !(radius > 0.f))
        return TT_ERR_BAD_ARG;
    if (plane_h != plane_w || plane_h <= 0) return TT_ERR_UNSUPPORTED;
    return TT_OK;
}

#define TT_ITEM_BLOCK 256
static inline unsigned tt_grid(long long n) { return (unsigned)((n + TT_ITEM_BLOCK - 1) / TT_ITEM_BLOCK); }

struct TtCarver {
    char* base;
    long long off = 0;
    template <typename T>
    T* take(long long count) {
        T* p = base ? (T*)(base + off) : nullptr;
        off += ((long long)sizeof(T) * count + 255) & ~255ll;
        return p;
    }
    long long bytes() const { return off; }
};

long long tt_mesh_components_bytes(long long T);

struct TileGeom;
long long tt_make_geom(const tt_render_cfg* cfg, long long wave_slots, TileGeom* g, int default_order,
                       int steps_per_item = 6, int min_items_per_slot = 8);

int* tt_queue_counters(hipStream_t stream);
#define TT_SLOT_INTS 32
#define TT_SLOT_BOUNDS 16
#define TT_BOUND_PLANES 0
#define TT_BOUND_UP0 1
#define TT_BOUND_UP1 2
#define TT_SLOT_EIKONAL 24

int tt_launch_march_fwd(const float* rays_d, const float* t_starts, const float* t_ends, const tt_render_cfg* cfg,
                        const float* sdf, const float* sdf_grad, const float* features, float* opacity, float* depth,
                        float* rgb_fg, float* z_variance, float* normal_acc, float* weights, float* trans,
                        hipStream_t stream);
int tt_launch_march_bwd(const float* rays_d, const float* t_starts, const float* t_ends, const tt_render_cfg* cfg,
                        const float* sdf, const float* sdf_grad, const float* features, const float* trans,
                        const float* opacity, const float* depth, const float* g_opacity, const float* g_depth,
                        const float* g_rgb_fg, const float* g_z_variance, const float* g_normal_acc,
                        const float* g_weights, const float* g_sdf, const float* g_sdf_grad, float* g_inv_std_rays,
                        float* ws, hipStream_t stream);
```

### triplaneturbo_amd/csrc/tt_march.hip

```cpp
#include "tt_device.h"
#include "tt_alpha.h"
#include "tt_host.h"

struct MarchFwdParams {
    const float* rays_d;
    const float* t_starts;
    const float* t_ends;
    const float* sdf;
    const float* sdf_grad;
    const float* features;
    long long n_rays;
    int S;
    float inv_std, ratio;
    int volsdf;
    const float* inv_std_dev;
    float* opacity;
    float* depth;
    float* rgb_fg;
    float* z_var;
    float* nacc;
    float* weights;
    float* trans;
};

// ... 123 lines not shown
    const long long wave = (long long)blockIdx.x * (blockDim.x >> 6) + (threadIdx.x >> 6);
    const long long n_waves = (long long)gridDim.x * (blockDim.x >> 6);
    const int S = p.S;
    const float kstd = load_inv_std(p.inv_std_dev, p.inv_std);
    for (long long ray = wave; ray < p.n_rays; ray += n_waves) {
        const float dx = p.rays_d[ray * 3 + 0], dy = p.rays_d[ray * 3 + 1], dz = p.rays_d[ray * 3 + 2];
        FwdAcc a = {1.f, 0.f, 0.f, 0.f, 0.f, 0.f, 0.f, 0.f, 0.f};
        float zv = 0.f;
        if constexpr (NP > 0) {
            FwdIn in[NP];
#pragma unroll
            for (int k = 0; k < NP; ++k) {
                const int si = 64 * k + lane;
                in[k] = march_load_fwd(p, ray * S + (si < S ? si : 0));
            }
            float w[NP], tmid[NP];
#pragma unroll
            for (int k = 0; k < NP; ++k) {
                const int si = 64 * k + lane;
                float Ti;
                march_pass_fwd(p, kstd, in[k], si < S, lane, dx, dy, dz, a, w[k], Ti, tmid[k]);
                if (si < S) {
                    p.weights[ray * S + si] = w[k];
                    p.trans[ray * S + si] = Ti;
                }
            }
            march_reduce_fwd(a);
#pragma unroll
            for (int k = 0; k < NP; ++k) {
                const float dd = tmid[k] - a.d;
                zv = fmaf(w[k], dd * dd, zv);
            }
        } else {
            for (int base = 0; base < S; base += 64) {
                const int si = base + lane;
                const bool valid = si < S;
                const long long sidx = ray * S + (valid ? si : 0);
                const FwdIn v = march_load_fwd(p, sidx);
                float wgt, Ti, tm;
                march_pass_fwd(p, kstd, v, valid, lane, dx, dy, dz, a, wgt, Ti, tm);
                if (valid) {
                    p.weights[sidx] = wgt;
                    p.trans[sidx] = Ti;
                }
            }
            march_reduce_fwd(a);
            for (int si = lane; si < S; si += 64) {
                const long long sidx = ray * S + si;
                const float tm = (p.t_starts[sidx] + p.t_ends[sidx]) / 2.f;
                const float dd = tm - a.d;
                zv = fmaf(p.weights[sidx], dd * dd, zv);
            }
        }
        zv = wave_sum(zv);
        if (lane == 0) march_store_ray(p, ray, a, zv);
    }
}

struct MarchBwdParams {
    const float* rays_d;
    const float* t_starts;
    const float* t_ends;
    const float* sdf;
    const float* sdf_grad;
    const float* features;
    const float* trans;
    const float* opacity;
    const float* depth;
    const float* g_opacity;
    const float* g_depth;
    const float* g_rgb;
    const float* g_zvar;
    const float* g_nacc;
    const float* g_weights;
    const float* g_sdf;
    const float* g_sdf_grad;
    long long n_rays;
    int S;
    float inv_std, ratio;
    int volsdf;
    const float* inv_std_dev;
    float* g_inv_std_rays;
    float* ws;
};

struct BwdIn {
    float ts, te, sdf, gx, gy, gz, f0, f1, f2, trans, gw, gs, ggx, ggy, ggz;
};
__device__ __forceinline__ BwdIn march_load_bwd(const MarchBwdParams& p, long long sidx) {
    BwdIn v;
    v.ts = p.t_starts[sidx];
    v.te = p.t_ends[sidx];
    v.sdf = p.sdf[sidx];
    v.gx = p.sdf_grad[sidx * 3 + 0];
    v.gy = p.sdf_grad[sidx * 3 + 1];
    v.gz = p.sdf_grad[sidx * 3 + 2];
    v.f0 = p.features[sidx * 3 + 0];
    v.f1 = p.features[sidx * 3 + 1];
    v.f2 = p.features[sidx * 3 + 2];
    v.trans = p.trans[sidx];
    v.gw = p.g_weights ? p.g_weights[sidx] : 0.f;
    v.gs = p.g_sdf ? p.g_sdf[sidx] : 0.f;
    v.ggx = p.g_sdf_grad ? p.g_sdf_grad[sidx * 3 + 0] : 0.f;
    v.ggy = p.g_sdf_grad ? p.g_sdf_grad[sidx * 3 + 1] : 0.f;
    v.ggz = p.g_sdf_grad ? p.g_sdf_grad[sidx * 3 + 2] : 0.f;
    return v;
}
struct RayBar {
    float dx, dy, dz, op, D, b_op, b_d, b_z, b_r, b_g, b_b, b_nx, b_ny, b_nz;
};
__device__ __forceinline__ f32x4 march_pass_bwd(const MarchBwdParams& p, float kstd, const BwdIn& v, bool valid, int lane,
                                                const RayBar& rb, float& Rcarry, float& dk) {
    const float tm = (v.ts + v.te) / 2.f;
    const float gn_raw = sqrtf(v.gx * v.gx + v.gy * v.gy + v.gz * v.gz);
    const float gn = fmaxf(gn_raw, 1e-12f);
    const float ign = rcp_(gn);
    const float nx = v.gx * ign, ny = v.gy * ign, nz = v.gz * ign;
    const float cosv = rb.dx * nx + rb.dy * ny + rb.dz * nz;
    const AlphaTerms a = p.volsdf ? volsdf_alpha_terms(v.sdf, v.te - v.ts, kstd)
                                  : neus_alpha_terms(v.sdf, cosv, v.te - v.ts, kstd, p.ratio);
    const float alpha = valid ? a.alpha : 0.f;
    const float Ti = valid ? v.trans : 0.f;
    const float wgt = alpha * Ti;
    const float rr = sigmoid_(v.f0) * 1.002f - 0.001f, rg = sigmoid_(v.f1) * 1.002f - 0.001f,
                rbl = sigmoid_(v.f2) * 1.002f - 0.001f;
    const float dd = tm - rb.D;
    float V = rb.b_op + rb.b_d * tm + rb.b_z * (dd * dd - 2.f * tm * rb.D * (1.f - rb.op)) +
              (rb.b_r * rr + rb.b_g * rg + rb.b_b * rbl) + (rb.b_nx * nx + rb.b_ny * ny + rb.b_nz * nz);
    V += v.gw;
    if (!valid) V = 0.f;
    const float Rnext = wave_affine_prev(1.f - alpha, V * alpha, Rcarry);
    const float dalpha = Ti * (V - Rnext);
    const float drat = dalpha * a.pass * (valid ? 1.f : 0.f);
    float sbar, dcos;
    if (p.volsdf) {
        sbar = drat * a.d_sdf;
        dcos = 0.f;
        dk += drat * a.d_k;
    } else {
        const float iden = rcp_(a.den);
        const float dnum = drat * iden, dden = -drat * a.rat * iden;
        const float dargA = (dnum + dden) * a.sA * (1.f - a.sA), dargB = (-dnum) * a.sB * (1.f - a.sB);
        const float dA = dargA * kstd, dB = dargB * kstd;
        dk += dargA * a.prev_sdf + dargB * a.next_sdf;
        sbar = dA + dB;
        dcos = a.half * (dB - dA) * a.dic_dcos;
    }
    const float nbx = wgt * rb.b_nx + dcos * rb.dx, nby = wgt * rb.b_ny + dcos * rb.dy,
                nbz = wgt * rb.b_nz + dcos * rb.dz;
    float gbx, gby, gbz;
    if (gn_raw > 1e-12f) {
        const float nd = nx * nbx + ny * nby + nz * nbz;
        gbx = (nbx - nx * nd) * ign;
        gby = (nby - ny * nd) * ign;
        gbz = (nbz - nz * nd) * ign;
    } else {
        gbx = nbx * 1e12f;
        gby = nby * 1e12f;
        gbz = nbz * 1e12f;
    }
    f32x4 o = {sbar + v.gs, gbx + v.ggx, gby + v.ggy, gbz + v.ggz};
    return o;
}

template <int NP>
__global__ __launch_bounds__(256) void k_march_bwd(MarchBwdParams p) {
    const int lane = threadIdx.x & 63;
    const long long wave = (long long)blockIdx.x * (blockDim.x >> 6) + (threadIdx.x >> 6);
    const long long n_waves = (long long)gridDim.x * (blockDim.x >> 6);
    const int S = p.S;
    const float kstd = load_inv_std(p.inv_std_dev, p.inv_std);
    for (long long ray = wave; ray < p.n_rays; ray += n_waves) {
        RayBar rb;
        rb.dx = p.rays_d[ray * 3 + 0];
        rb.dy = p.rays_d[ray * 3 + 1];
        rb.dz = p.rays_d[ray * 3 + 2];
        rb.op = p.opacity[ray];
        rb.D = p.depth[ray];
        rb.b_op = p.g_opacity ? p.g_opacity[ray] : 0.f;
        rb.b_d = p.g_depth ? p.g_depth[ray] : 0.f;
        rb.b_z = p.g_zvar ? p.g_zvar[ray] : 0.f;
        rb.b_r = p.g_rgb ? p.g_rgb[ray * 3 + 0] : 0.f;
        rb.b_g = p.g_rgb ? p.g_rgb[ray * 3 + 1] : 0.f;
        rb.b_b = p.g_rgb ? p.g_rgb[ray * 3 + 2] : 0.f;
        rb.b_nx = p.g_nacc ? p.g_nacc[ray * 3 + 0] : 0.f;
        rb.b_ny = p.g_nacc ? p.g_nacc[ray * 3 + 1] : 0.f;
        rb.b_nz = p.g_nacc ? p.g_nacc[ray * 3 + 2] : 0.f;
        float Rcarry = 0.f, dk = 0.f;
        if constexpr (NP > 0) {
            BwdIn in[NP];
#pragma unroll
            for (int k = 0; k < NP; ++k) {
                const int si = 64 * k + 63 - lane;
                in[k] = march_load_bwd(p, ray * S + (si < S ? si : 0));
            }
#pragma unroll
            for (int k = NP - 1; k >= 0; --k) {
                const int si = 64 * k + 63 - lane;
                const f32x4 o = march_pass_bwd(p, kstd, in[k], si < S, lane, rb, Rcarry, dk);
                if (si < S) *reinterpret_cast<f32x4*>(p.ws + (ray * S + si) * 4) = o;
            }
        } else {
            for (int base = ((S - 1) / 64) * 64; base >= 0; base -= 64) {
                const int si = base + 63 - lane;
                const bool valid = si < S;
                const long long sidx = ray * S + (valid ? si : 0);
                const BwdIn v = march_load_bwd(p, sidx);
                const f32x4 o = march_pass_bwd(p, kstd, v, valid, lane, rb, Rcarry, dk);
                if (valid) *reinterpret_cast<f32x4*>(p.ws + sidx * 4) = o;
            }
        }
        if (p.g_inv_std_rays) {
            dk = wave_sum(dk);
            if (lane == 0) p.g_inv_std_rays[ray] = dk;
        }
    }
}

static unsigned march_blocks(long long n_rays) {
    long long blocks = (n_rays + 3) / 4;
    const long long cap = 1LL << 22;
    if (blocks > cap) blocks = cap;
    return (unsigned)(blocks < 1 ? 1 : blocks);
}

int tt_launch_march_fwd(const float* rays_d, const float* t_starts, const float* t_ends, const tt_render_cfg* cfg,
                        const float* sdf, const float* sdf_grad, const float* features, float* opacity, float* depth,
                        float* rgb_fg, float* z_variance, float* normal_acc, float* weights, float* trans,
                        hipStream_t stream) {
    MarchFwdParams p;
    p.rays_d = rays_d;
    p.t_starts = t_starts;
    p.t_ends = t_ends;
    p.sdf = sdf;
    p.sdf_grad = sdf_grad;
    p.features = features;
    p.n_rays = cfg->n_rays;
    p.S = cfg->n_samples;
    p.inv_std = cfg->inv_std;
    p.inv_std_dev = cfg->inv_std_dev;
    p.volsdf = (cfg->flags & TT_R_VOLSDF) ? 1 : 0;
    p.ratio = cfg->cos_anneal_ratio;
    p.opacity = opacity;
    p.depth = depth;
    p.rgb_fg = rgb_fg;
    p.z_var = z_variance;
    p.nacc = normal_acc;
    p.weights = weights;
    p.trans = trans;
    const dim3 grid(march_blocks(cfg->n_rays)), blk(256);
    if (p.S <= 64)
        hipLaunchKernelGGL(k_march_fwd<1>, grid, blk, 0, stream, p);
    else if (p.S <= 128)
        hipLaunchKernelGGL(k_march_fwd<2>, grid, blk, 0, stream, p);
    else if (p.S <= 256)
        hipLaunchKernelGGL(k_march_fwd<4>, grid, blk, 0, stream, p);
    else
        hipLaunchKernelGGL(k_march_fwd<0>, grid, blk, 0, stream, p);
    return tt_check_launch();
}

int tt_launch_march_bwd(const float* rays_d, const float* t_starts, const float* t_ends, const tt_render_cfg* cfg,
                        const float* sdf, const float* sdf_grad, const float* features, const float* trans,
                        const float* opacity, const float* depth, const float* g_opacity, const float* g_depth,
                        const float* g_rgb_fg, const float* g_z_variance, const float* g_normal_acc,
                        const float* g_weights, const float* g_sdf, const float* g_sdf_grad, float* g_inv_std_rays,
                        float* ws, hipStream_t stream) {
    MarchBwdParams p;
    p.rays_d = rays_d;
    p.t_starts = t_starts;
    p.t_ends = t_ends;
    p.sdf = sdf;
    p.sdf_grad = sdf_grad;
    p.features = features;
    p.trans = trans;
    p.opacity = opacity;
    p.depth = depth;
    p.g_opacity = g_opacity;
    p.g_depth = g_depth;
    p.g_rgb = g_rgb_fg;
    p.g_zvar = g_z_variance;
    p.g_nacc = g_normal_acc;
    p.g_weights = g_weights;
    p.g_sdf = g_sdf;
    p.g_sdf_grad = g_sdf_grad;
    p.n_rays = cfg->n_rays;
    p.S = cfg->n_samples;
    p.inv_std = cfg->inv_std;
    p.inv_std_dev = cfg->inv_std_dev;
    p.volsdf = (cfg->flags & TT_R_VOLSDF) ? 1 : 0;
    p.g_inv_std_rays = g_inv_std_rays;
    p.ratio = cfg->cos_anneal_ratio;
    p.ws = ws;
    const dim3 grid(march_blocks(cfg->n_rays)), blk(256);
    if (p.S <= 64)
        hipLaunchKernelGGL(k_march_bwd<1>, grid, blk, 0, stream, p);
    else if (p.S <= 128)
        hipLaunchKernelGGL(k_march_bwd<2>, grid, blk, 0, stream, p);
    else if (p.S <= 256)
        hipLaunchKernelGGL(k_march_bwd<4>, grid, blk, 0, stream, p);
    else
        hipLaunchKernelGGL(k_march_bwd<0>, grid, blk, 0, stream, p);
    return tt_check_launch();
}

extern "C" int tt_march_fwd(const float* rays_d, const float* t_starts, const float* t_ends, const tt_render_cfg* cfg,
                            const float* sdf, const float* sdf_grad, const float* features, float* opacity,
                            float* depth, float* rgb_fg, float* z_variance, float* normal_acc, float* weights,
                            float* trans, void* stream) {
    int st = tt_validate_cfg(cfg);
    if (st != TT_OK) return st;
    if (!rays_d || !t_starts || !t_ends || !sdf || !sdf_grad || !features || !opacity || !depth || !rgb_fg ||
        !z_variance || !normal_acc || !weights || !trans)
        return TT_ERR_BAD_ARG;
    return tt_launch_march_fwd(rays_d, t_starts, t_ends, cfg, sdf, sdf_grad, features, opacity, depth, rgb_fg,
                               z_variance, normal_acc, weights, trans, (hipStream_t)stream);
}

extern "C" int tt_march_bwd(const float* rays_d, const float* t_starts, const float* t_ends, const tt_render_cfg* cfg,
                            const float* opacity, const float* depth, const float* trans, const float* sdf,
                            const float* sdf_grad, const float* features, const float* g_opacity,
                            const float* g_depth, const float* g_rgb_fg, const float* g_z_variance,
                            const float* g_normal_acc, const float* g_weights, const float* g_sdf,
                            const float* g_sdf_grad, float* g_inv_std_rays, float* out_grad, void* stream) {
    int st = tt_validate_cfg(cfg);
    if (st != TT_OK) return st;
    if (!rays_d || !t_starts || !t_ends || !opacity || !depth || !trans || !sdf || !sdf_grad || !features || !out_grad)
        return TT_ERR_BAD_ARG;
    return tt_launch_march_bwd(rays_d, t_starts, t_ends, cfg, sdf, sdf_grad, features, trans, opacity, depth,
                               g_opacity, g_depth, g_rgb_fg, g_z_variance, g_normal_acc, g_weights, g_sdf, g_sdf_grad,
                               g_inv_std_rays, out_grad, (hipStream_t)stream);
}
```

### triplaneturbo_amd/functional.py

```python
from __future__ import annotations

from typing import Dict, Optional, Sequence

import torch
import torch.nn.functional as F

from . import ops

Tensor = torch.Tensor


class LazyOutputs(dict):

    def __init__(self, *a, **k):
        super().__init__(*a, **k)
        self._lazy = {}

    def set_lazy(self, key, fn):
        self._lazy[key] = fn

    def _materialise(self, key):
        fn = self._lazy.pop(key)
        val = fn()
        super().__setitem__(key, val)
        return val

    def __getitem__(self, key):
        if key in self._lazy:
            return self._materialise(key)
        return super().__getitem__(key)

    def __setitem__(self, key, value):
        self._lazy.pop(key, None)
        super().__setitem__(key, value)

    def __contains__(self, key):
        return key in self._lazy or super().__contains__(key)

    def get(self, key, default=None):
        return self[key] if key in self else default

    def eager_keys(self):
        return list(super().keys())

    def _all(self):
        for k in list(self._lazy):
            self._materialise(k)

    def keys(self):
        self._all()
        return super().keys()

    def items(self):
        self._all()
        return super().items()

    def values(self):
        self._all()
        return super().values()

    def __iter__(self):
        self._all()
        return super().__iter__()

    def __len__(self):
        return super().__len__() + len(self._lazy)

    def update(self, *a, **k):
        for key, v in dict(*a, **k).items():
            self[key] = v


def volume_render(space_cache: Tensor, sdf_w: Sequence[Tensor], feat_w: Sequence[Tensor], rays_o: Tensor,
                  rays_d: Tensor, t_starts: Tensor, t_ends: Tensor, bg_color: Tensor, camera_distances: Tensor,
                  c2w: Tensor, rc: ops.RenderConfig, training: bool = True,
                  normal_direction: str = "camera", comp_rgb_bg: Optional[Tensor] = None,
                  packed: Optional[Tensor] = None, eval_termination_eps: float = 0.0) -> Dict[str, Tensor]:
    B, Hh, Ww, _ = rays_o.shape
    n_rays = B * Hh * Ww
    S = t_starts.shape[1]
    ro = rays_o.reshape(n_rays, 3)
    rd = rays_d.reshape(n_rays, 3)
    if not training and not torch.is_grad_enabled() and eval_termination_eps > 0.0:
        pk = packed if packed is not None else ops.planes_pack(space_cache)
        r = ops.render_eval_raw(pk, sdf_w, feat_w, ro.contiguous(), rd.contiguous(), t_starts.contiguous(),
                                t_ends.contiguous(), Hh * Ww, rc, image_w=Ww,
                                transmittance_eps=eval_termination_eps, weight_eps=eval_termination_eps / max(S, 1))
    else:
        r = ops.render_samples(space_cache, sdf_w, feat_w, ro, rd, t_starts, t_ends, Hh * Ww, rc, image_w=Ww,
                               packed=packed)
    opacity, depth, comp_rgb_fg, z_variance = r["opacity"], r["depth"], r["rgb_fg"], r["z_variance"]

    if normal_direction not in ("camera", "front", "world"):
        raise ValueError(normal_direction)
    bg = bg_color if bg_color.ndim == 1 else bg_color.reshape(n_rays, -1)
    if comp_rgb_bg is None:
        comp_rgb_bg = bg[None, :].expand(n_rays, -1) if bg.ndim == 1 else bg
    n_prompts = packed.shape[0] if packed is not None else space_cache.shape[0]
    comp = ops.composite(opacity, depth, comp_rgb_fg, r["normal_acc"], bg.contiguous(), camera_distances, c2w,
                         Hh * Ww, normal_direction, view_group=B // n_prompts)
    comp_rgb, disparity, comp_normal, vis, vis_white = comp
    out = LazyOutputs({
        "comp_rgb": comp_rgb.view(B, Hh, Ww, -1),
        "comp_rgb_fg": comp_rgb_fg.view(B, Hh, Ww, -1),
        "comp_rgb_bg": comp_rgb_bg.reshape(B, Hh, Ww, -1),
        "opacity": opacity.view(B, Hh, Ww, 1),
        "depth": depth.view(B, Hh, Ww, 1),
        "z_variance": z_variance.view(B, Hh, Ww, 1),
        "disparity": disparity.view(B, Hh, Ww, 1),
        "comp_normal": comp_normal.view(B, Hh, Ww, 3),
    })
    if vis is not None:
        out["comp_normal_cam_vis"] = vis.view(B, Hh, Ww, 3)
    if vis_white is not None:
        out["comp_normal_cam_vis_white"] = vis_white.view(B, Hh, Ww, 3)

    if training:
        grad_mode = torch.is_grad_enabled()

        def lazy(fn):
            def run():
                with torch.set_grad_enabled(grad_mode):
                    return fn()
            return run

        cache = {}

        def shared(name, fn):
            if name not in cache:
                cache[name] = fn()
            return cache[name]

        t_pos = lambda: shared("t", lambda: ((t_starts + t_ends) / 2.0).reshape(-1, 1))
        ridx = lambda: shared("ri", lambda: torch.arange(n_rays, device=ro.device).unsqueeze(-1).expand(-1, S).reshape(-1))
        t_dirs = lambda: shared("td", lambda: rd[ridx()])
        points = lambda: shared("p", lambda: ro[ridx()] + t_dirs() * t_pos())
        normal = lambda: shared("n", lambda: F.normalize(r["sdf_grad"], dim=-1))
        out["weights"] = r["weights"]
        out["sdf"] = r["sdf"]
        out["features"] = r["features"]
        out["sdf_grad"] = r["sdf_grad"]
        out.set_lazy("t_points", lazy(t_pos))
        out.set_lazy("t_intervals", lazy(lambda: (t_ends - t_starts).reshape(-1, 1)))
        out.set_lazy("t_dirs", lazy(t_dirs))
        out.set_lazy("ray_indices", lazy(ridx))
        out.set_lazy("points", lazy(points))
        out.set_lazy("sdf_orig", lazy(lambda: r["sdf"] - ((points() ** 2).sum(dim=-1, keepdim=True).sqrt()
                                                          - rc.sdf_bias_radius)))
        out.set_lazy("normal", lazy(normal))
        out.set_lazy("shading_normal", lazy(normal))
        out["inv_std"] = (rc.inv_std_t.detach().reshape(()) if rc.inv_std_t is not None else
                          torch.full((), float(rc.inv_std), device=ro.device))
    return out
```

### triplaneturbo_amd/ops.py

```python
from __future__ import annotations

import ctypes
import dataclasses
from dataclasses import dataclass
from functools import cached_property
from typing import List, NamedTuple, Optional, Sequence, Tuple, Union

import numpy as np
import torch

from . import _lib

Tensor = torch.Tensor


class KernelTimer:

    def __init__(self):
        self.events = []

    def summary(self, median: bool = False):
        torch.cuda.synchronize()
        acc = {}
        for label, a, b in self.events:
# ... 65 lines not shown
    if not t.is_cuda:
        raise RuntimeError(f"{name} must live on the GPU (triplaneturbo_amd has no CPU path)")
    if t.device.index != torch.cuda.current_device():
        raise RuntimeError(f"{name} lives on {t.device} but the current device is cuda:{torch.cuda.current_device()}; "
                           f"call torch.cuda.set_device (one process per GPU)")


def _chk(t: Tensor, name: str, shape: Optional[Sequence[Optional[int]]] = None, dtype=torch.float32) -> Tensor:
    _chk_gpu(t, name)
    if t.dtype != dtype:
        raise TypeError(f"{name} must be {dtype}, got {t.dtype}")
    if shape is not None and (t.dim() != len(shape) or any(e not in (None, n) for e, n in zip(shape, t.shape))):
        raise ValueError(f"{name} has shape {tuple(t.shape)}, expected {str(tuple(shape)).replace('None', '*')}")
    return t.contiguous()


def _chk_index(t: Tensor, name: str, width: int, rows: Optional[int] = None) -> Tensor:
    _chk_gpu(t, name)
    if t.dtype not in (torch.int32, torch.int64) or t.dim() != 2 or t.shape[1] != width:
        raise TypeError(f"{name} must be (N,{width}) int32 / int64, got {tuple(t.shape)} {t.dtype}")
    if rows is not None and t.shape[0] != rows:
        raise ValueError(f"{name} has {t.shape[0]} rows, expected {rows}")
    return t


def _minmax(*tables: Tensor) -> Tensor:
    return torch.stack([x for t in tables for x in (t.aminmax() if t.numel() else t.new_tensor([0, -1]).unbind())])


def _chk_range(name: str, lo: int, hi: int, n: int) -> None:
    if lo < 0 or hi >= n:
        raise ValueError(f"{name} holds an index outside [0, {n})")


def _chk_size(what: str, **counts: int) -> None:
    if max(counts.values()) > _lib.TT_MESH_MAX_ITEMS:
        sizes = ", ".join(f"{k}={v}" for k, v in counts.items())
        raise ValueError(f"{what}: {sizes} (limit TT_MESH_MAX_ITEMS = {_lib.TT_MESH_MAX_ITEMS})")


def _csr(row: Tensor, col: Optional[Tensor], n_rows: int, n_cols: int) -> Tuple[Tensor, Tensor]:
    order = torch.sort(row if col is None else torch.add(col, row, alpha=max(n_cols, 1)), stable=True)[1]
    out = (order if col is None else col[order]).int().contiguous()
    ptr = torch.zeros(n_rows + 1, dtype=torch.int64, device=row.device)
    ptr[1:] = torch.cumsum(torch.bincount(row, minlength=n_rows), 0)
    return ptr.int().contiguous(), out


def _weights_struct(sdf_w: Sequence[Tensor], net2_w: Optional[Sequence[Tensor]], net2: str = "feat v",
                    net2_in: int = 96):
    sw = [_chk(sdf_w[0], "sdf w1", (64, 32)), _chk(sdf_w[1], "sdf w2", (64, 64)), _chk(sdf_w[2], "sdf w3", (1, 64))]
    fw: List[Optional[Tensor]] = [None, None, None]
    if net2_w is not None:
        fw = [_chk(net2_w[0], net2 + "1", (64, net2_in)), _chk(net2_w[1], net2 + "2", (64, 64)),
              _chk(net2_w[2], net2 + "3", (3, 64))]
    st = _lib.MlpWeights(*[_ptr(t) for t in sw + fw])
    return st, sw + fw


@dataclass
class RenderConfig:
    radius: float = 1.0
    sdf_bias_radius: float = 0.5
    inv_std: float = 100.0
    cos_anneal_ratio: float = 1.0
    rgb_grad_shrink: float = 1.0
    tile_sb: int = 0
    grad_copies: int = 1
    tile_chunk: int = 0
    precision: Optional[str] = None
    exact_f32: bool = False
    use_volsdf: bool = False

    @property
    def prec(self) -> str:
        return _lib.resolve_precision(self.precision, self.exact_f32)
    skip_eps_tex: float = 0.0
    skip_eps_geo: float = 0.0
    inv_std_t: Optional[Tensor] = None
    stats: Optional[Tensor] = None
    fwd_mask: bool = True


def planes_pack(space_cache: Tensor) -> Tensor:
    space_cache = _chk(space_cache, "space_cache", (None, 6, 32, None, None))
    P, _, _, H, W = space_cache.shape
    out = torch.empty((P, 6, H, W, 32), device=space_cache.device, dtype=torch.float32)
    _launch("tt_planes_pack", space_cache, out, P, H, W)
    return out


def planes_unpack_grad(grad_packed: Tensor) -> Tensor:
    grad_packed = _chk(grad_packed, "grad_packed")
    copies = grad_packed.shape[0] if grad_packed.ndim == 6 else 1
    P, _, H, W, _ = grad_packed.shape[-5:]
    out = torch.empty((P, 6, 32, H, W), device=grad_packed.device, dtype=torch.float32)
    _launch("tt_planes_unpack_grad", grad_packed, out, P, H, W, copies)
    return out


class _PackPlanesFn(torch.autograd.Function):

    @staticmethod
    def forward(ctx, space_cache):
        return planes_pack(space_cache)

    @staticmethod
    @torch.autograd.function.once_differentiable
    def backward(ctx, grad_packed):
        return planes_unpack_grad(grad_packed.contiguous())


def pack_planes(space_cache: Tensor) -> Tensor:
    return _PackPlanesFn.apply(space_cache)


def query_points(packed: Tensor, sdf_w: Sequence[Tensor], feat_w: Optional[Sequence[Tensor]], points: Tensor,
                 views_per_prompt: int = 1, radius: float = 1.0, sdf_bias_radius: float = 0.5,
                 need_normal: bool = True, need_features: bool = True, exact_f32: bool = False,
                 precision: Optional[str] = None):
    packed = _chk(packed, "packed")
    points = _chk(points, "points")
    B, N, _ = points.shape
    P, _, H, W, _ = packed.shape
    wst, keep = _weights_struct(sdf_w, feat_w if need_features else None)
    dev = points.device
    sdf = torch.empty((B * N, 1), device=dev, dtype=torch.float32)
    grad = torch.empty((B * N, 3), device=dev, dtype=torch.float32) if need_normal else None
    feat = torch.empty((B * N, 3), device=dev, dtype=torch.float32) if need_features else None
    flags = (_lib.TT_Q_NORMAL if need_normal else 0) | (_lib.TT_Q_TEX if need_features else 0) | _lib.q_flag(
        _lib.resolve_precision(precision, exact_f32))
    _launch("tt_query_points", packed, wst, points, B, N, P, views_per_prompt, H, W, radius, sdf_bias_radius, flags,
            sdf, grad, feat, label="tt_query_points")
    return sdf, grad, feat


def query_field(packed: Tensor, sdf_w: Sequence[Tensor], deform_w: Sequence[Tensor], points: Tensor,
                views_per_prompt: int = 1, radius: float = 1.0, sdf_bias_radius: float = 0.5, exact_f32: bool = False,
                precision: Optional[str] = None):
    packed = _chk(packed, "packed")
    points = _chk(points, "points")
    B, N, _ = points.shape
    P, _, H, W, _ = packed.shape
    wst, keep = _weights_struct(sdf_w, deform_w, "def d", 32)
    sdf = torch.empty((B * N, 1), device=points.device, dtype=torch.float32)
    deform = torch.empty((B * N, 3), device=points.device, dtype=torch.float32)
    _launch("tt_query_field", packed, wst, points, B, N, P, views_per_prompt, H, W, radius, sdf_bias_radius,
            _lib.q_flag(_lib.resolve_precision(precision, exact_f32)), sdf, deform, label="tt_query_field")
    return sdf, deform


class _QueryPointsFn(torch.autograd.Function):

    @staticmethod
    def forward(ctx, space_cache, w1, w2, w3, v1, v2, v3, points, views_per_prompt, radius, sdf_bias_radius,
                need_normal, prec):
        ctx.set_materialize_grads(False)
        packed = planes_pack(space_cache)
        sdf, grad, feat = query_points(packed, (w1, w2, w3), (v1, v2, v3), points, views_per_prompt, radius,
                                       sdf_bias_radius, need_normal=need_normal, need_features=True,
                                       precision=prec)
        ctx.save_for_backward(packed, w1, w2, w3, v1, v2, v3, points)
        ctx.meta = (views_per_prompt, radius, sdf_bias_radius, _lib.q_flag(prec))
        if grad is None:
            grad = sdf.new_zeros((sdf.shape[0], 3))
            ctx.mark_non_differentiable(grad)
        return sdf, grad, feat

    @staticmethod
    @torch.autograd.function.once_differentiable
    def backward(ctx, g_sdf, g_grad, g_feat):
        packed, w1, w2, w3, v1, v2, v3, points = ctx.saved_tensors
        vpp, radius, bias_r, qf = ctx.meta
        B, N, _ = points.shape
        P, _, H, W, _ = packed.shape
        wst, keep = _weights_struct((w1, w2, w3), (v1, v2, v3))
        g_sdf, g_grad, g_feat = _contig(g_sdf), _contig(g_grad), _contig(g_feat)
        gw = [None] * 6
        g_cache = None
        if any(ctx.needs_input_grad[:7]):
            grad_packed = torch.zeros_like(packed)
            gw = [torch.zeros_like(t) for t in (w1, w2, w3, v1, v2, v3)]
            gst = _grads_struct(gw)
            if g_sdf is not None or g_grad is not None:
                ws = torch.empty((B * N, 4), device=packed.device, dtype=torch.float32)
                _launch("tt_points_bwd_geo", packed, wst, points, B, N, P, vpp, H, W, radius, bias_r, qf, g_sdf, g_grad,
                        ws, grad_packed, gst)
            if g_feat is not None:
                _launch("tt_points_bwd_tex", packed, wst, points, B, N, P, vpp, H, W, radius, 3, qf, g_feat,
                        grad_packed, gst)
            g_cache = planes_unpack_grad(grad_packed) if ctx.needs_input_grad[0] else None
        g_points = None
        if ctx.needs_input_grad[7]:
            g_points = torch.empty_like(points)
            _launch("tt_points_bwd_x", packed, wst, points, B, N, P, vpp, H, W, radius, qf, g_sdf, g_grad, g_feat,
                    g_points)
        return (g_cache, *gw, g_points, None, None, None, None, None)


def query_points_grad(space_cache: Tensor, sdf_w: Sequence[Tensor], feat_w: Sequence[Tensor], points: Tensor,
                      views_per_prompt: int = 1, radius: float = 1.0, sdf_bias_radius: float = 0.5,
                      need_normal: bool = True, exact_f32: bool = False, precision: Optional[str] = None):
    return _QueryPointsFn.apply(space_cache, sdf_w[0], sdf_w[1], sdf_w[2], feat_w[0], feat_w[1], feat_w[2],
                                _chk(points, "points"), int(views_per_prompt), float(radius), float(sdf_bias_radius),
                                bool(need_normal), _lib.resolve_precision(precision, bool(exact_f32)))


class _QueryFieldFn(torch.autograd.Function):

    @staticmethod
    def forward(ctx, space_cache, w1, w2, w3, d1, d2, d3, points, views_per_prompt, radius, sdf_bias_radius,
                prec):
        ctx.set_materialize_grads(False)
        packed = planes_pack(space_cache)
        sdf, deform = query_field(packed, (w1, w2, w3), (d1, d2, d3), points, views_per_prompt, radius,
                                  sdf_bias_radius, precision=prec)
        ctx.save_for_backward(packed, w1, w2, w3, d1, d2, d3, points)
        ctx.meta = (views_per_prompt, radius, sdf_bias_radius, _lib.q_flag(prec))
        return sdf, deform

    @staticmethod
    @torch.autograd.function.once_differentiable
    def backward(ctx, g_sdf, g_def):
        packed, w1, w2, w3, d1, d2, d3, points = ctx.saved_tensors
        vpp, radius, bias_r, qf = ctx.meta
        B, N, _ = points.shape
        P, _, H, W, _ = packed.shape
        d1x3 = d1.repeat(1, 3).contiguous()
        keep = [w1.contiguous(), w2.contiguous(), w3.contiguous(), d1x3, d2.contiguous(), d3.contiguous()]
        wst = _lib.MlpWeights(*[_ptr(t) for t in keep])
        grad_packed = torch.zeros_like(packed)
        gw = [torch.zeros_like(t) for t in (w1, w2, w3, d1x3, d2, d3)]
        gst = _grads_struct(gw)
        if g_sdf is not None:
            ws = torch.empty((B * N, 4), device=packed.device, dtype=torch.float32)
            _launch("tt_points_bwd_geo", packed, wst, points, B, N, P, vpp, H, W, radius, bias_r, qf,
                    g_sdf.contiguous(), None, ws, grad_packed, gst)
        if g_def is not None:
            _launch("tt_points_bwd_tex", packed, wst, points, B, N, P, vpp, H, W, radius, 0, qf, g_def.contiguous(),
                    grad_packed, gst)
        gw[3] = gw[3].view(64, 3, 32).sum(dim=1)
        g_cache = planes_unpack_grad(grad_packed) if ctx.needs_input_grad[0] else None
        return (g_cache, *gw, None, None, None, None, None)


def query_field_grad(space_cache: Tensor, sdf_w: Sequence[Tensor], deform_w: Sequence[Tensor], points: Tensor,
                     views_per_prompt: int = 1, radius: float = 1.0, sdf_bias_radius: float = 0.5,
                     exact_f32: bool = False, precision: Optional[str] = None):
    return _QueryFieldFn.apply(space_cache, sdf_w[0], sdf_w[1], sdf_w[2], deform_w[0], deform_w[1], deform_w[2],
                               _chk(points, "points"), int(views_per_prompt), float(radius), float(sdf_bias_radius),
                               _lib.resolve_precision(precision, bool(exact_f32)))


def _inv_std_args(rc: RenderConfig):
    inv_std = min(max(float(rc.inv_std), 1.0e-6), 1.0e6)
    if rc.inv_std_t is None:
        return inv_std, None
    t = _chk(rc.inv_std_t, "inv_std_t")
    if t.numel() != 1:
        raise ValueError("inv_std_t must hold one float")
    if t.data_ptr() != rc.inv_std_t.data_ptr():
        raise ValueError("inv_std_t must be a contiguous float32 CUDA tensor (the kernels read it in place)")
    return inv_std, t.data_ptr()


def _make_cfg(packed: Tensor, n_rays: int, rays_per_view: int, n_samples: int, rc: RenderConfig,
              per_sample: bool, image_w: int = 0, stats_row: int = 0) -> "_lib.RenderCfg":
    P, _, H, W, _ = packed.shape
    n_views = n_rays // rays_per_view
    if n_views * rays_per_view != n_rays or n_views % P != 0:
        raise ValueError(f"n_rays={n_rays} is not views*rays_per_view with views a multiple of P={P}")
    inv_std, inv_std_dev = _inv_std_args(rc)
    stats = None
    if rc.stats is not None:
        if rc.stats.dtype != torch.int64 or not rc.stats.is_cuda or tuple(rc.stats.shape) != (3, 4):
            raise ValueError("stats must be a CUDA int64 tensor of shape (3, 4)")
        stats = rc.stats.data_ptr() + 32 * stats_row
    return _lib.RenderCfg(P, n_views // P, H, W, rays_per_view, n_samples, n_rays, rc.radius, rc.sdf_bias_radius,
                          inv_std, rc.cos_anneal_ratio, rc.rgb_grad_shrink,
                          (_lib.TT_R_PER_SAMPLE if per_sample else 0) | _lib.r_flag(rc.prec) |
                          (_lib.TT_R_VOLSDF if rc.use_volsdf else 0),
                          image_w if (image_w > 0 and rays_per_view % image_w == 0) else 0, int(rc.tile_sb),
                          max(1, int(rc.grad_copies)), max(0, int(rc.tile_chunk)), max(0.0, float(rc.skip_eps_tex)),
                          max(0.0, float(rc.skip_eps_geo)), inv_std_dev, stats)


def _ray_args(packed: Tensor, rays_o: Tensor, rays_d: Tensor, t_starts: Tensor, t_ends: Tensor):
    packed = _chk(packed, "packed")
    rays_o, rays_d = _chk(rays_o, "rays_o"), _chk(rays_d, "rays_d")
    t_starts, t_ends = _chk(t_starts, "t_starts"), _chk(t_ends, "t_ends")
    n_rays, S = t_starts.shape
    if rays_o.shape != (n_rays, 3) or rays_d.shape != (n_rays, 3) or t_ends.shape != (n_rays, S):
        raise ValueError("ray / interval shapes disagree")
    return packed, rays_o, rays_d, t_starts, t_ends


def _ray_outputs(n_rays: int, device, S: Optional[int] = None) -> dict:
    f32 = dict(device=device, dtype=torch.float32)
    out = {"opacity": torch.empty((n_rays, 1), **f32), "depth": torch.empty((n_rays, 1), **f32),
           "rgb_fg": torch.empty((n_rays, 3), **f32), "z_variance": torch.empty((n_rays, 1), **f32),
           "normal_acc": torch.empty((n_rays, 3), **f32)}
    if S is not None:
        out.update(weights=torch.empty((n_rays * S, 1), **f32), trans=torch.empty((n_rays * S, 1), **f32))
    return out


def render_forward_raw(packed: Tensor, sdf_w: Sequence[Tensor], feat_w: Sequence[Tensor], rays_o: Tensor,
                       rays_d: Tensor, t_starts: Tensor, t_ends: Tensor, rays_per_view: int, rc: RenderConfig,
                       per_sample: bool = True, image_w: int = 0, h2_mask: Union[bool, Tensor] = False):
    packed, rays_o, rays_d, t_starts, t_ends = _ray_args(packed, rays_o, rays_d, t_starts, t_ends)
    n_rays, S = t_starts.shape
    cfg = _make_cfg(packed, n_rays, rays_per_view, S, rc, per_sample, image_w)
    wst, keep = _weights_struct(sdf_w, feat_w)
    f32 = dict(device=packed.device, dtype=torch.float32)
    out = _ray_outputs(n_rays, packed.device, S)
    out.update(sdf=torch.empty((n_rays * S, 1), **f32), sdf_grad=torch.empty((n_rays * S, 3), **f32),
               features=torch.empty((n_rays * S, 3), **f32))
    if h2_mask is not False:
        if h2_mask is True:
            h2_mask = torch.empty((n_rays * S, 2), device=packed.device, dtype=torch.int32)
        out["h2_mask"] = _chk(h2_mask, "h2_mask", (n_rays * S, 2), torch.int32)
        if out["h2_mask"].data_ptr() != h2_mask.data_ptr():
            raise ValueError("h2_mask must be contiguous (the kernel writes it in place)")
        _launch("tt_render_fwd_h2mask", packed, wst, rays_o, rays_d, t_starts, t_ends, cfg, *out.values(),
                label="tt_render_fwd")
    else:
        _launch("tt_render_fwd", packed, wst, rays_o, rays_d, t_starts, t_ends, cfg, *out.values(),
                label="tt_render_fwd")
    return out


@torch.no_grad()
def render_eval_raw(packed: Tensor, sdf_w: Sequence[Tensor], feat_w: Sequence[Tensor], rays_o: Tensor, rays_d: Tensor,
                    t_starts: Tensor, t_ends: Tensor, rays_per_view: int, rc: RenderConfig, image_w: int = 0,
                    transmittance_eps: float = 0.0, weight_eps: float = 0.0, stats: Optional[Tensor] = None):
    packed, rays_o, rays_d, t_starts, t_ends = _ray_args(packed, rays_o, rays_d, t_starts, t_ends)
    n_rays, S = t_starts.shape
    cfg = _make_cfg(packed, n_rays, rays_per_view, S, rc, False, image_w)
    wst, keep = _weights_struct(sdf_w, feat_w)
    out = _ray_outputs(n_rays, packed.device)
    if stats is not None and (stats.dtype != torch.int64 or stats.numel() < 2 or not stats.is_cuda):
        raise ValueError("stats must be a CUDA int64 tensor with 2 elements")
    _launch("tt_render_eval", packed, wst, rays_o, rays_d, t_starts, t_ends, cfg, float(transmittance_eps),
            float(weight_eps), *out.values(), stats, label="tt_render_eval")
    return out


def _placement(name: str) -> int:
    if name not in _lib.PLACEMENTS:
        raise ValueError(f"placement must be one of {sorted(_lib.PLACEMENTS)}, got {name!r}")
    return _lib.PLACEMENTS[name]


@torch.no_grad()
def sample_uniform(n_rays: int, n_samples: int, near: float, far: float, device, jitter: Optional[Tensor] = None,
                   placement: str = "tt"):
    device = torch.device(device)
    place = _placement(placement)
    if device.type != "cuda":
        raise RuntimeError("triplaneturbo_amd samplers run on the GPU only (no CPU fallback)")
    f32 = dict(device=device, dtype=torch.float32)
    ts, te = torch.empty((n_rays, n_samples), **f32), torch.empty((n_rays, n_samples), **f32)
    if jitter is not None:
        jitter = _chk(jitter, "jitter")
        if jitter.shape != (n_rays, n_samples + 1):
            raise ValueError("jitter must be (n_rays, n_samples + 1)")
    with torch.cuda.device(device):
        _launch("tt_sample_uniform", n_rays, n_samples, float(near), float(far), jitter, place, ts, te)
    return ts, te


@torch.no_grad()
def sample_importance(t_starts: Tensor, t_ends: Tensor, sdf: Tensor, n_fine: int, inv_std: float,
                      render_step_size: float, u_jitter: Optional[Tensor] = None, placement: str = "tt",
                      inv_std_t: Optional[Tensor] = None, use_volsdf: bool = False):
    place = _placement(placement) | (_lib.TT_PLACE_VOLSDF if use_volsdf else 0)
    if inv_std_t is not None:
        inv_std_t = _chk(inv_std_t.detach(), "inv_std_t")
    t_starts, t_ends, sdf = _chk(t_starts, "t_starts"), _chk(t_ends, "t_ends"), _chk(sdf, "sdf")
    n_rays, K = t_starts.shape
    if t_ends.shape != (n_rays, K) or sdf.numel() != n_rays * K:
        raise ValueError("proposal intervals / sdf shapes disagree")
    if u_jitter is not None:
        u_jitter = _chk(u_jitter, "u_jitter")
        if u_jitter.shape != (n_rays, n_fine + 1):
            raise ValueError("u_jitter must be (n_rays, n_fine + 1)")
    f32 = dict(device=t_starts.device, dtype=torch.float32)
    M = K + n_fine + 1
    ots, ote = torch.empty((n_rays, M), **f32), torch.empty((n_rays, M), **f32)
    _launch("tt_sample_importance", t_starts, t_ends, sdf, n_rays, K, int(n_fine), float(inv_std), inv_std_t,
            float(render_step_size), u_jitter, place, ots, ote, label="tt_sample_importance")
    return ots, ote


def _march_cfg(rc: RenderConfig, n_rays: int, S: int) -> "_lib.RenderCfg":
    inv_std, inv_std_dev = _inv_std_args(rc)
    return _lib.RenderCfg(n_prompts=1, views_per_prompt=1, plane_h=1, plane_w=1, rays_per_view=n_rays, n_samples=S,
                          n_rays=n_rays, radius=rc.radius, sdf_bias_radius=rc.sdf_bias_radius, inv_std=inv_std,
                          cos_anneal_ratio=rc.cos_anneal_ratio, rgb_grad_shrink=rc.rgb_grad_shrink,
                          flags=_lib.TT_R_VOLSDF if rc.use_volsdf else 0, image_w=0,
                          tile_sb=0, grad_copies=1, tile_chunk=0, inv_std_dev=inv_std_dev)


@torch.no_grad()
def march_forward_raw(rays_d: Tensor, t_starts: Tensor, t_ends: Tensor, sdf: Tensor, sdf_grad: Tensor,
                      features: Tensor, rc: RenderConfig, out: Optional[dict] = None):
    rays_d, t_starts, t_ends = _chk(rays_d, "rays_d"), _chk(t_starts, "t_starts"), _chk(t_ends, "t_ends")
    sdf, sdf_grad, features = _chk(sdf, "sdf"), _chk(sdf_grad, "sdf_grad"), _chk(features, "features")
    n_rays, S = t_starts.shape
    if sdf.numel() != n_rays * S or sdf_grad.numel() != 3 * n_rays * S or features.numel() != 3 * n_rays * S:
        raise ValueError("per-sample tensors do not match (n_rays, S)")
    cfg = _march_cfg(rc, n_rays, S)
    if out is None:
        out = _ray_outputs(n_rays, rays_d.device, S)
    _launch("tt_march_fwd", rays_d, t_starts, t_ends, cfg, sdf, sdf_grad, features, out["opacity"], out["depth"],
            out["rgb_fg"], out["z_variance"], out["normal_acc"], out["weights"], out["trans"], label="tt_march_fwd")
    return out


@torch.no_grad()
def march_backward_raw(rays_d: Tensor, t_starts: Tensor, t_ends: Tensor, fwd: dict, sdf: Tensor, sdf_grad: Tensor,
                       features: Tensor, rc: RenderConfig, g_opacity=None, g_depth=None, g_rgb_fg=None,
                       g_z_variance=None, g_normal_acc=None, g_weights=None, g_sdf=None, g_sdf_grad=None,
                       out: Optional[Tensor] = None, g_inv_std_rays: Optional[Tensor] = None):
    n_rays, S = t_starts.shape
    cfg = _march_cfg(rc, n_rays, S)
    if out is None:
        out = torch.empty((n_rays * S, 4), device=rays_d.device, dtype=torch.float32)
    gs = [_contig(t)
          for t in (g_opacity, g_depth, g_rgb_fg, g_z_variance, g_normal_acc, g_weights, g_sdf, g_sdf_grad)]
    _launch("tt_march_bwd", rays_d, t_starts, t_ends, cfg, fwd["opacity"], fwd["depth"], fwd["trans"], sdf, sdf_grad,
            features, *gs, g_inv_std_rays, out, label="tt_march_bwd")
    return out


def _zeros_like_flat(tensors: Sequence[Tensor]) -> List[Tensor]:
    sizes = [t.numel() for t in tensors]
    flat = torch.zeros(sum(sizes), device=tensors[0].device, dtype=tensors[0].dtype)
    out, ofs = [], 0
    for t, n in zip(tensors, sizes):
        out.append(flat[ofs:ofs + n].view_as(t))
        ofs += n
    return out


def _grads_struct(tensors: Sequence[Tensor]):
    return _lib.MlpWeights(*[_ptr(t) for t in tensors])


class _TriplaneRenderFn(torch.autograd.Function):

    @staticmethod
    def forward(ctx, packed, w1, w2, w3, v1, v2, v3, rays_o, rays_d, t_starts, t_ends, rays_per_view, rc,
                image_w, inv_std_t=None):
        need_grad = any(ctx.needs_input_grad[:7]) or ctx.needs_input_grad[14]
        if inv_std_t is not None:
            rc = dataclasses.replace(rc, inv_std_t=inv_std_t.detach())
        ctx.set_materialize_grads(False)
        raw = render_forward_raw(packed, (w1, w2, w3), (v1, v2, v3), rays_o, rays_d, t_starts, t_ends, rays_per_view,
                                 rc, per_sample=True, image_w=image_w, h2_mask=need_grad and rc.fwd_mask)
        ctx.rays_per_view = rays_per_view
        ctx.rc = rc
        ctx.image_w = image_w
        ctx.inv_std_shape = None if inv_std_t is None else tuple(inv_std_t.shape)
        if need_grad:
            ctx.save_for_backward(packed, w1, w2, w3, v1, v2, v3, rays_o, rays_d, t_starts, t_ends, raw["opacity"],
                                  raw["depth"], raw["trans"], raw["weights"], raw["features"], raw["sdf"],
                                  raw["sdf_grad"], *([raw["h2_mask"]] if rc.fwd_mask else []))
        ctx.mark_non_differentiable(raw["trans"])
        return (raw["opacity"], raw["depth"], raw["rgb_fg"], raw["z_variance"], raw["normal_acc"], raw["weights"],
                raw["sdf"], raw["sdf_grad"], raw["features"], raw["trans"])

    @staticmethod
    @torch.autograd.function.once_differentiable
    def backward(ctx, g_op, g_depth, g_rgb, g_zvar, g_nacc, g_weights, g_sdf, g_sdf_grad, g_features, _g_trans):
        (packed, w1, w2, w3, v1, v2, v3, rays_o, rays_d, t_starts, t_ends, opacity, depth, trans, weights,
         features, sdf, sdf_grad) = ctx.saved_tensors[:18]
        h2_mask = ctx.saved_tensors[18:]
        n_rays, S = t_starts.shape
        cfg = _make_cfg(packed, n_rays, ctx.rays_per_view, S, ctx.rc, True, ctx.image_w, stats_row=1)
        cfg_tex = _make_cfg(packed, n_rays, ctx.rays_per_view, S, ctx.rc, True, ctx.image_w, stats_row=2)
        workspace = torch.empty((n_rays * S, 4), device=packed.device, dtype=torch.float32)
        wst, keep = _weights_struct((w1, w2, w3), (v1, v2, v3))
        copies = max(1, int(ctx.rc.grad_copies))
        grad_packed = torch.zeros((copies,) + tuple(packed.shape), device=packed.device, dtype=torch.float32)
        gw = _zeros_like_flat((w1, w2, w3, v1, v2, v3))
        gst = _grads_struct(gw)

        g_op, g_depth, g_rgb, g_zvar, g_nacc, g_weights, g_sdf, g_sdf_grad, g_features = (
            _contig(t) for t in (g_op, g_depth, g_rgb, g_zvar, g_nacc, g_weights, g_sdf, g_sdf_grad, g_features))
        g_k_rays = None
        if ctx.needs_input_grad[14]:
            g_k_rays = torch.empty((n_rays,), device=packed.device, dtype=torch.float32)
        _launch("tt_render_bwd_geo_h2mask" if h2_mask else "tt_render_bwd_geo", packed, wst, rays_o, rays_d, t_starts,
                t_ends, cfg, opacity, depth, trans, sdf, sdf_grad, features, g_op, g_depth, g_rgb, g_zvar, g_nacc,
                g_weights, g_sdf, g_sdf_grad, g_k_rays, workspace, grad_packed, gst, *h2_mask, label="tt_render_bwd_geo")
        _launch("tt_render_bwd_tex", packed, wst, rays_o, rays_d, t_starts, t_ends, cfg_tex, weights, features, g_rgb,
                g_features, grad_packed, gst, label="tt_render_bwd_tex")
        g_packed = None
        if ctx.needs_input_grad[0]:
            g_packed = grad_packed[0] if copies == 1 else grad_packed.sum(dim=0)
        g_inv_std = None
        if g_k_rays is not None:
            g_inv_std = g_k_rays.double().sum().float().reshape(ctx.inv_std_shape)
        return (g_packed, *gw, None, None, None, None, None, None, None, g_inv_std)


def render_samples(space_cache: Optional[Tensor], sdf_w: Sequence[Tensor], feat_w: Sequence[Tensor], rays_o: Tensor,
                   rays_d: Tensor, t_starts: Tensor, t_ends: Tensor, rays_per_view: int, rc: RenderConfig,
                   image_w: int = 0, packed: Optional[Tensor] = None):
    names = ("opacity", "depth", "rgb_fg", "z_variance", "normal_acc", "weights", "sdf", "sdf_grad", "features",
             "trans")
    if packed is None:
        packed = pack_planes(space_cache)
    outs = _TriplaneRenderFn.apply(packed, sdf_w[0], sdf_w[1], sdf_w[2], feat_w[0], feat_w[1], feat_w[2],
                                   rays_o.contiguous(), rays_d.contiguous(), t_starts.contiguous(),
                                   t_ends.contiguous(), rays_per_view, rc, int(image_w), rc.inv_std_t)
    return dict(zip(names, outs))


@torch.no_grad()
def decode_rays(packed: Tensor, sdf_w: Sequence[Tensor], feat_w: Optional[Sequence[Tensor]], rays_o: Tensor,
                rays_d: Tensor, t_starts: Tensor, t_ends: Tensor, rays_per_view: int, rc: RenderConfig,
                need_normal: bool = False, need_features: bool = False, image_w: int = 0):
    packed, rays_o, rays_d, t_starts, t_ends = _ray_args(packed, rays_o, rays_d, t_starts, t_ends)
    n_rays, S = t_starts.shape
    cfg = _make_cfg(packed, n_rays, rays_per_view, S, rc, False, image_w)
    wst, keep = _weights_struct(sdf_w, feat_w if need_features else None)
    f32 = dict(device=packed.device, dtype=torch.float32)
    sdf = torch.empty((n_rays, S), **f32)
    grad = torch.empty((n_rays, S, 3), **f32) if need_normal else None
    feat = torch.empty((n_rays, S, 3), **f32) if need_features else None
    flags = (_lib.TT_Q_NORMAL if need_normal else 0) | (_lib.TT_Q_TEX if need_features else 0)
    _launch("tt_decode_rays", packed, wst, rays_o, rays_d, t_starts, t_ends, cfg, flags, sdf, grad, feat,
            label="tt_decode_rays")
    return sdf, grad, feat


class _PatchCompositeFn(torch.autograd.Function):

    @staticmethod
    def forward(ctx, low, patch, py, px, H, W, detach_low):
        low, patch = _chk(low, "low"), _chk(patch, "patch")
        B, h, w, C = low.shape
        PS = patch.shape[1]
        if patch.shape != (B, PS, PS, C):
            raise ValueError(f"patch {tuple(patch.shape)} does not match low {tuple(low.shape)}")
        out = torch.empty((B, H, W, C), device=low.device, dtype=torch.float32)
        _launch("tt_patch_composite_fwd", low, patch, out, B, h, w, H, W, C, PS, py, px)
        ctx.meta = (B, h, w, H, W, C, PS, py, px, detach_low)
        return out

    @staticmethod
    @torch.autograd.function.once_differentiable
    def backward(ctx, g_out):
        B, h, w, H, W, C, PS, py, px, detach_low = ctx.meta
        want_low = ctx.needs_input_grad[0] and not detach_low
        g_low = torch.empty((B, h, w, C), device=g_out.device, dtype=torch.float32) if want_low else None
        g_patch = torch.empty((B, PS, PS, C), device=g_out.device, dtype=torch.float32)
        _launch("tt_patch_composite_bwd", g_out.contiguous(), g_low, g_patch, B, h, w, H, W, C, PS, py, px)
        return g_low, (g_patch if ctx.needs_input_grad[1] else None), None, None, None, None, None


def patch_composite(low: Tensor, patch: Tensor, py: int, px: int, H: int, W: int, detach_low: bool = False) -> Tensor:
    return _PatchCompositeFn.apply(low, patch, int(py), int(px), int(H), int(W), bool(detach_low))


_COMPOSITE_MODES = {"world": 0, "camera": 1, "front": 2}


class _CompositeFn(torch.autograd.Function):

    @staticmethod
    def forward(ctx, opacity, depth, rgb_fg, normal_acc, bg, cam_dist, c2w, rays_per_view, mode, view_group):
        opacity, depth = _chk(opacity, "opacity"), _chk(depth, "depth")
        rgb_fg, normal_acc = _chk(rgb_fg, "rgb_fg"), _chk(normal_acc, "normal_acc")
        bg, cam_dist = _chk(bg, "bg_color"), _chk(cam_dist, "camera_distances")
        n = opacity.numel()
        if rays_per_view <= 0 or n % rays_per_view != 0:
            raise ValueError(f"n_rays={n} is not a multiple of rays_per_view={rays_per_view}")
        views = n // rays_per_view
        if cam_dist.numel() != views:
            raise ValueError(f"camera_distances has {cam_dist.numel()} elements, expected one per view ({views})")
        if c2w is None:
            if mode != 0:
                raise ValueError("c2w is required for normal_direction 'camera' / 'front' (renderer :478-530)")
        else:
            c2w = _chk(c2w, "c2w", (views, 4, 4))
        if view_group <= 0 or views % view_group != 0:
            raise ValueError(f"view_group={view_group} does not divide the number of views ({views})")
        bg_stride = 0 if bg.numel() == 3 else 3
        if bg_stride and bg.numel() != 3 * n:
            raise ValueError("bg_color must have 3 or 3 * n_rays elements")
        f32 = dict(device=opacity.device, dtype=torch.float32)
        comp_rgb, comp_normal = torch.empty((n, 3), **f32), torch.empty((n, 3), **f32)
        disparity = torch.empty((n, 1), **f32)
        vis = torch.empty((n, 3), **f32) if mode == 1 else None
        vis_white = torch.empty((n, 3), **f32) if mode != 0 else None
        _launch("tt_composite_fwd", opacity, depth, rgb_fg, normal_acc, bg, bg_stride, cam_dist, c2w, n, rays_per_view,
                mode, view_group, comp_rgb, disparity, comp_normal, vis, vis_white)
        ctx.save_for_backward(opacity, depth, rgb_fg, normal_acc, bg, cam_dist, *(() if c2w is None else (c2w,)))
        ctx.meta = (n, bg_stride, rays_per_view, mode, view_group)
        ctx.set_materialize_grads(False)
        dummy = comp_rgb.new_zeros(0)
        outs = (comp_rgb, disparity, comp_normal, vis if vis is not None else dummy,
                vis_white if vis_white is not None else dummy)
        return outs
# ... 768 lines not shown
```

### triplaneturbo_amd/renderer.py

```python
from __future__ import annotations

from dataclasses import dataclass
from typing import Any, Dict, Optional

import math

import torch
import torch.nn as nn
import torch.nn.functional as F

from . import functional, ops, sampler
from .registry import BaseModule, C, find, register

Tensor = torch.Tensor


class LearnedVariance(nn.Module):

    def __init__(self, init_val, requires_grad=True):
        super().__init__()
        self.register_parameter("_inv_std", nn.Parameter(torch.tensor(float(init_val)), requires_grad=requires_grad))

    @property
    def inv_std(self):
# ... 76 lines not shown
        if c.estimator != "importance":
            raise NotImplementedError("estimator must be 'importance' (the reference raises for 'occgrid', :83-85)")
        assert c.normal_direction in ["front", "camera", "world"]
        self.geometry, self.material, self.background = geometry, material, background
        if material is not None and not isinstance(material, NoMaterial):
            raise NotImplementedError("the fused path implements NoMaterial (sigmoid-mipnerf) only")
        self.variance = LearnedVariance(c.learned_variance_init, requires_grad=bool(c.trainable_variance))
        self.render_step_size = 1.732 * 2 * c.radius / c.num_samples_per_ray
        self.cos_anneal_ratio = 1.0
        self.randomized = c.randomized
        self.rgb_grad_shrink = C(c.rgb_grad_shrink, 0, 0)
        self.register_buffer("bbox", torch.as_tensor([[-c.radius] * 3, [c.radius] * 3], dtype=torch.float32))
        self.tile_sb_importance = None
        self.sampler_placement = "tt"
        self.grad_skip_eps_tex = 0.0
        self.grad_skip_eps_geo = 0.0
        self.eval_termination_eps = 0.0
        self.precision = None

    def _inv_std_value(self) -> float:
        p = self.variance._inv_std
        key = (p._version, p.data_ptr())
        if getattr(self, "_inv_std_cache", (None, None))[0] != key:
            self._inv_std_cache = (key, min(max(math.exp(float(p.detach()) * 10.0), 1.0e-6), 1.0e6))
        return self._inv_std_cache[1]

    def set_inv_std(self, inv_std: float) -> None:
        with torch.no_grad():
            self.variance._inv_std.fill_(math.log(float(inv_std)) / 10.0)
        self._inv_std_cache = (None, None)

    def _load_from_state_dict(self, *args, **kwargs):
        self._inv_std_cache = (None, None)
        return super()._load_from_state_dict(*args, **kwargs)

    def _render_config(self) -> ops.RenderConfig:
        g = self.geometry.cfg
        rc = ops.RenderConfig(radius=self.cfg.radius, sdf_bias_radius=float(g.sdf_bias_params),
                              cos_anneal_ratio=float(self.cos_anneal_ratio),
                              rgb_grad_shrink=float(self.rgb_grad_shrink), skip_eps_tex=float(self.grad_skip_eps_tex),
                              skip_eps_geo=float(self.grad_skip_eps_geo), precision=self.precision,
                              use_volsdf=bool(self.cfg.use_volsdf))
        if self.cfg.trainable_variance:
            rc.inv_std_t = self.variance.inv_std.clamp(1.0e-6, 1.0e6).float()
        else:
            rc.inv_std = self._inv_std_value()
        return rc

    def sample(self, space_cache: Tensor, rays_o: Tensor, rays_d: Tensor, generator=None, packed=None):
        B, Hh, Ww, _ = rays_o.shape
        n_rays = B * Hh * Ww
        rc = self._render_config()
        sw, _ = self.geometry.mlp_weights()
        packed = ops.planes_pack(space_cache.detach()) if packed is None else packed.detach()
        ro, rd = rays_o.reshape(-1, 3).contiguous(), rays_d.reshape(-1, 3).contiguous()

        def sdf_fn(ts, te):
            sdf, _, _ = ops.decode_rays(packed, [w.detach() for w in sw], None, ro, rd, ts, te, Hh * Ww, rc,
                                        image_w=Ww)
            return sdf

        return sampler.importance_sampling(
            sdf_fn, n_rays, self.cfg.num_samples_per_ray_importance, self.cfg.num_samples_per_ray,
            self.cfg.near_plane, self.cfg.far_plane, rc.inv_std, self.render_step_size, device=rays_o.device,
            stratified=self.randomized, generator=generator, placement=self.sampler_placement,
            inv_std_t=rc.inv_std_t, use_volsdf=rc.use_volsdf)

    def forward(self, rays_o: Tensor, rays_d: Tensor, light_positions: Optional[Tensor] = None,
                bg_color: Optional[Tensor] = None, noise: Optional[Tensor] = None,
                space_cache: Optional[Tensor] = None, text_embed: Optional[Tensor] = None,
                camera_distances: Optional[Tensor] = None, c2w: Optional[Tensor] = None, t_starts=None, t_ends=None,
                **kwargs) -> Dict[str, Tensor]:
        B, Hh, Ww, _ = rays_o.shape
        if space_cache is None:
            space_cache = self.geometry.generate_space_cache(styles=noise, text_embed=text_embed)
        if not torch.is_tensor(space_cache):
            raise NotImplementedError("dict space caches (hyper-net variants, renderer :128-141) are out of scope")
        P = space_cache.shape[0]
        if text_embed is not None:
            assert text_embed.shape[0] == P
        assert B % P == 0, "batch of views must be a multiple of the number of prompts"
        grad_on = torch.is_grad_enabled()
        packed = kwargs.pop("packed", None)
        tile_sb = kwargs.pop("tile_sb", None)
        pitch_w = kwargs.pop("ray_pitch_w", None)
        if packed is None:
            with (torch.enable_grad() if grad_on else torch.no_grad()):
                packed = ops.pack_planes(space_cache)
        importance_sampled = t_starts is None
        if t_starts is None:
            t_starts, t_ends = self.sample(space_cache, rays_o, rays_d, packed=packed)
        if bg_color is None:
            text_bg = kwargs.get("text_embed_bg", text_embed)
            comp_rgb_bg = self.background(dirs=rays_d, text_embed=text_bg) if getattr(
                self.background, "enabling_hypernet", False) else self.background(dirs=rays_d)
            bg_color = comp_rgb_bg
        else:
            comp_rgb_bg = None
        sw, fw = self.geometry.mlp_weights()
        rc = self._render_config()
        if importance_sampled:
            rc.tile_sb = int(tile_sb) if tile_sb is not None else self._tile_sb_for(
                int(pitch_w) if pitch_w else rays_o.shape[2], space_cache.shape[-1])
        ctx = torch.enable_grad() if grad_on else torch.no_grad()
        with ctx:
            out = functional.volume_render(space_cache, sw, fw, rays_o, rays_d, t_starts, t_ends, bg_color,
                                           camera_distances, c2w, rc, training=self.training,
                                           normal_direction=self.cfg.normal_direction, comp_rgb_bg=comp_rgb_bg,
                                           packed=packed, eval_termination_eps=self.eval_termination_eps)
        if self.training:
            out["inv_std"] = self.variance.inv_std
        return out

    def _tile_sb_for(self, image_w: int, plane_w: int) -> int:
        if self.tile_sb_importance is not None:
            return int(self.tile_sb_importance)
        pitch = plane_w / max(image_w, 1)
        return 2 if pitch <= 1.0 else (4 if pitch <= 3.0 else 8)

    def update_step(self, epoch: int, global_step: int, on_load_weights: bool = False) -> None:
        self._inv_std_cache = (None, None)
        self.rgb_grad_shrink = C(self.cfg.rgb_grad_shrink, epoch, global_step)
        self.cos_anneal_ratio = 1.0 if self.cfg.cos_anneal_end_steps == 0 else min(
            1.0, global_step / self.cfg.cos_anneal_end_steps)

    def train(self, mode=True):
        self.randomized = mode and self.cfg.randomized
        if hasattr(self.geometry, "train"):
            self.geometry.train(mode)
        return super().train(mode=mode)

    def eval(self):
        self.randomized = False
        if hasattr(self.geometry, "eval"):
            self.geometry.eval()
        return super().eval()


@register("patch-renderer")
class PatchRenderer(BaseModule):

    @dataclass
    class Config(BaseModule.Config):
        radius: float = 1.0
        patch_size: int = 128
        base_renderer_type: str = ""
        base_renderer: Optional[dict] = None
        global_detach: bool = False
        global_downsample: int = 4

    cfg: Config

    def configure(self, geometry, material, background) -> None:
        self.base_renderer = find(self.cfg.base_renderer_type)(self.cfg.base_renderer, geometry=geometry,
                                                               material=material, background=background)
        self.tile_sb_global = None
        self.tile_sb_patch = None

    def forward(self, rays_o: Tensor, rays_d: Tensor, light_positions: Optional[Tensor] = None,
                bg_color: Optional[Tensor] = None, **kwargs) -> Dict[str, Tensor]:
        B, H, W, _ = rays_o.shape
        if not self.base_renderer.training:
            return self.base_renderer(rays_o, rays_d, light_positions, bg_color, **kwargs)
        sc = kwargs.get("space_cache")
        if torch.is_tensor(sc) and kwargs.get("packed") is None:
            with (torch.enable_grad() if torch.is_grad_enabled() else torch.no_grad()):
                kwargs["packed"] = ops.pack_planes(sc)
        ds = self.cfg.global_downsample
        g_o = F.interpolate(rays_o.permute(0, 3, 1, 2).contiguous(), (H // ds, W // ds), mode="bilinear").permute(0, 2, 3, 1)
        g_d = F.interpolate(rays_d.permute(0, 3, 1, 2).contiguous(), (H // ds, W // ds), mode="bilinear").permute(0, 2, 3, 1)
        kw_g = dict(kwargs, ray_pitch_w=W // ds) if self.tile_sb_global is None else dict(kwargs, tile_sb=self.tile_sb_global)
        kw_p = dict(kwargs, ray_pitch_w=W) if self.tile_sb_patch is None else dict(kwargs, tile_sb=self.tile_sb_patch)
        out_global = self.base_renderer(g_o.contiguous(), g_d.contiguous(), light_positions, bg_color, **kw_g)
        PS = self.cfg.patch_size
        px = torch.randint(0, W - PS, (1,)).item()
        py = torch.randint(0, H - PS, (1,)).item()
        out = self.base_renderer(rays_o[:, py:py + PS, px:px + PS].contiguous(),
                                 rays_d[:, py:py + PS, px:px + PS].contiguous(), light_positions, bg_color, **kw_p)
        eager = out.eager_keys() if hasattr(out, "eager_keys") else list(out)
        valid = [k for k in eager if torch.is_tensor(out[k]) and out[k].ndim == out["comp_rgb"].ndim
                 and out[k][..., 0].shape == out["comp_rgb"][..., 0].shape]
        grad_mode = torch.is_grad_enabled()
        detach = self.cfg.global_detach

        def composite(low: Tensor, patch: Tensor):
            def run():
                with torch.set_grad_enabled(grad_mode):
                    return ops.patch_composite(low, patch, py, px, H, W, detach_low=detach)
            return run

        if not isinstance(out_global, functional.LazyOutputs):
            out_global = functional.LazyOutputs(out_global)
        for k in valid:
            out_global.set_lazy(k, composite(dict.__getitem__(out_global, k), out[k]))
        return out_global

    def update_step(self, epoch: int, global_step: int, on_load_weights: bool = False) -> None:
        self.base_renderer.update_step(epoch, global_step, on_load_weights)

    def train(self, mode=True):
        return self.base_renderer.train(mode)

    def eval(self):
        return self.base_renderer.eval()
```

Baseline: 8.104 million.

## Compute plane absmax bounds during packing and fuse bounds into march backward

Plane-magnitude bounds are now computed once when the triplanes are packed and passed down to the backward geometry and texture kernels, so the separate per-backward plane bound reduction launches are skipped. The march backward kernel also writes the upstream-gradient bound directly, and the absmax reduction copies the precomputed plane bound into the queue slot. This removes several small reduction kernels and passes over the planes per step, at the cost of more API surface and carrying an extra bounds tensor through autograd.

```diff
diff --git a/include/tt_abi.h b/include/tt_abi.h
--- a/include/tt_abi.h
+++ b/include/tt_abi.h
@@ -84,6 +84,8 @@
 
 int tt_planes_pack(const float* space_cache, float* packed, int32_t n_prompts, int32_t plane_h, int32_t plane_w,
                    void* stream);
+int tt_planes_pack_bounds(const float* space_cache, float* packed, int32_t n_prompts, int32_t plane_h, int32_t plane_w,
+                          uint32_t* bounds, void* stream);
 int tt_planes_unpack_grad(const float* grad_packed, float* grad_space_cache, int32_t n_prompts, int32_t plane_h,
                           int32_t plane_w, int32_t n_copies, void* stream);
 
@@ -136,6 +138,12 @@
                  const float* sdf_grad, const float* features, const float* g_opacity, const float* g_depth,
                  const float* g_rgb_fg, const float* g_z_variance, const float* g_normal_acc, const float* g_weights,
                  const float* g_sdf, const float* g_sdf_grad, float* g_inv_std_rays, float* out_grad, void* stream);
+int tt_march_bwd_bounds(const float* rays_d, const float* t_starts, const float* t_ends, const tt_render_cfg* cfg,
+                        const float* opacity, const float* depth, const float* trans, const float* sdf,
+                        const float* sdf_grad, const float* features, const float* g_opacity, const float* g_depth,
+                        const float* g_rgb_fg, const float* g_z_variance, const float* g_normal_acc,
+                        const float* g_weights, const float* g_sdf, const float* g_sdf_grad, float* g_inv_std_rays,
+                        float* out_grad, uint32_t* out_bounds, void* stream);
 
 int tt_render_bwd_geo(const float* packed, const tt_mlp_weights* w, const float* rays_o, const float* rays_d,
                       const float* t_starts, const float* t_ends, const tt_render_cfg* cfg, const float* opacity,
@@ -154,10 +162,24 @@
                              const float* g_sdf_grad, float* g_inv_std_rays, float* workspace, float* grad_packed,
                              const tt_mlp_grads* grads, const uint32_t* h2_mask, void* stream);
 
+int tt_render_bwd_geo_bounds(const float* packed, const tt_mlp_weights* w, const float* rays_o, const float* rays_d,
+                             const float* t_starts, const float* t_ends, const tt_render_cfg* cfg,
+                             const float* opacity, const float* depth, const float* trans, const float* sdf,
+                             const float* sdf_grad, const float* features, const float* g_opacity,
+                             const float* g_depth, const float* g_rgb_fg, const float* g_z_variance,
+                             const float* g_normal_acc, const float* g_weights, const float* g_sdf,
+                             const float* g_sdf_grad, float* g_inv_std_rays, float* workspace, float* grad_packed,
+                             const tt_mlp_grads* grads, const uint32_t* h2_mask, const uint32_t* plane_bounds,
+                             void* stream);
+
 int tt_render_bwd_tex(const float* packed, const tt_mlp_weights* w, const float* rays_o, const float* rays_d,
                       const float* t_starts, const float* t_ends, const tt_render_cfg* cfg, const float* weights,
                       const float* features, const float* g_rgb_fg, const float* g_features, float* grad_packed,
                       const tt_mlp_grads* grads, void* stream);
+int tt_render_bwd_tex_bounds(const float* packed, const tt_mlp_weights* w, const float* rays_o, const float* rays_d,
+                             const float* t_starts, const float* t_ends, const tt_render_cfg* cfg, const float* weights,
+                             const float* features, const float* g_rgb_fg, const float* g_features, float* grad_packed,
+                             const tt_mlp_grads* grads, const uint32_t* plane_bounds, void* stream);
 
 int tt_points_bwd_geo(const float* packed, const tt_mlp_weights* w, const float* points, int32_t n_batch,
                       int64_t n_points, int32_t n_prompts, int32_t views_per_prompt, int32_t plane_h, int32_t plane_w,
diff --git a/triplaneturbo_amd/csrc/tt_backward.hip b/triplaneturbo_amd/csrc/tt_backward.hip
--- a/triplaneturbo_amd/csrc/tt_backward.hip
+++ b/triplaneturbo_amd/csrc/tt_backward.hip
@@ -283,14 +283,14 @@
     return hipMemset(g_phase_cycles, 0, 40 * sizeof(unsigned long long)) == hipSuccess ? 0 : -4;
 }
 #endif
-static void launch_bwd_geo(const BwdGeoParams& p0, long long blocks, hipStream_t s) {
+static void launch_bwd_geo(const BwdGeoParams& p0, long long blocks, hipStream_t s, bool bounds_ready) {
     BwdGeoParams p = p0;
 #ifdef TT_TUNING
     p.phase_cycles = g_phase_cycles;
 #else
     p.phase_cycles = nullptr;
 #endif
-    if (use_wg16(p.cfg)) {
+    if (use_wg16(p.cfg) && !bounds_ready) {
         unsigned* bnd = reinterpret_cast<unsigned*>(p.queue) + TT_SLOT_BOUNDS;
         launch_planes_bound(p.packed, p.cfg, 0, bnd + TT_BOUND_PLANES, s);
         const long long n = p.cfg.n_rays * p.cfg.n_samples;
@@ -317,7 +317,8 @@
                           const float* features, const float* g_opacity, const float* g_depth, const float* g_rgb_fg,
                           const float* g_z_variance, const float* g_normal_acc, const float* g_weights,
                           const float* g_sdf, const float* g_sdf_grad, float* g_inv_std_rays, float* workspace,
-                          float* grad_packed, const tt_mlp_grads* grads, const uint32_t* h2_mask, void* stream) {
+                          float* grad_packed, const tt_mlp_grads* grads, const uint32_t* h2_mask,
+                          const uint32_t* plane_bounds, void* stream) {
     int st = tt_validate_cfg(cfg);
     if (st != TT_OK) return st;
     if (!packed || !w || !rays_o || !rays_d || !t_starts || !t_ends || !opacity || !depth || !trans || !sdf ||
@@ -328,10 +329,6 @@
     int cus = tt_num_cus();
     if (cus <= 0) return TT_ERR_DEVICE;
     hipStream_t s = (hipStream_t)stream;
-    st = tt_launch_march_bwd(rays_d, t_starts, t_ends, cfg, sdf, sdf_grad, features, trans, opacity, depth, g_opacity,
-                             g_depth, g_rgb_fg, g_z_variance, g_normal_acc, g_weights, g_sdf, g_sdf_grad, g_inv_std_rays,
-                             workspace, s);
-    if (st != TT_OK) return st;
     BwdGeoParams p;
     tt_fill_rays(p, packed, w, rays_o, rays_d, t_starts, t_ends, *cfg);
     p.cfg.flags |= debug_flags();
@@ -342,7 +339,14 @@
     p.grads = to_gptrs(grads);
     st = tt_plan_queue(cfg, 4LL * cus, s, &p.geom, &p.n_items, &p.queue);
     if (st != TT_OK) return st;
-    launch_bwd_geo(p, tt_persistent_blocks(p.n_items, cus, 4), s);
+    unsigned* bnd = use_wg16(p.cfg) ? reinterpret_cast<unsigned*>(p.queue) + TT_SLOT_BOUNDS : nullptr;
+    st = tt_launch_march_bwd(rays_d, t_starts, t_ends, cfg, sdf, sdf_grad, features, trans, opacity, depth, g_opacity,
+                             g_depth, g_rgb_fg, g_z_variance, g_normal_acc, g_weights, g_sdf, g_sdf_grad, g_inv_std_rays,
+                             workspace, bnd ? bnd + TT_BOUND_UP0 : nullptr, bnd ? plane_bounds : nullptr,
+                             bnd ? bnd + TT_BOUND_PLANES : nullptr, s);
+    if (st != TT_OK) return st;
+    if (bnd && !plane_bounds) launch_planes_bound(p.packed, p.cfg, 0, bnd + TT_BOUND_PLANES, s);
+    launch_bwd_geo(p, tt_persistent_blocks(p.n_items, cus, 4), s, true);
     return tt_check_launch();
 }
 
@@ -356,7 +360,7 @@
                                  float* grad_packed, const tt_mlp_grads* grads, void* stream) {
     return render_bwd_geo(packed, w, rays_o, rays_d, t_starts, t_ends, cfg, opacity, depth, trans, sdf, sdf_grad, features,
                           g_opacity, g_depth, g_rgb_fg, g_z_variance, g_normal_acc, g_weights, g_sdf, g_sdf_grad,
-                          g_inv_std_rays, workspace, grad_packed, grads, nullptr, stream);
+                          g_inv_std_rays, workspace, grad_packed, grads, nullptr, nullptr, stream);
 }
 
 extern "C" int tt_render_bwd_geo_h2mask(const float* packed, const tt_mlp_weights* w, const float* rays_o,
@@ -371,7 +375,23 @@
     if (!h2_mask) return TT_ERR_BAD_ARG;
     return render_bwd_geo(packed, w, rays_o, rays_d, t_starts, t_ends, cfg, opacity, depth, trans, sdf, sdf_grad, features,
                           g_opacity, g_depth, g_rgb_fg, g_z_variance, g_normal_acc, g_weights, g_sdf, g_sdf_grad,
-                          g_inv_std_rays, workspace, grad_packed, grads, h2_mask, stream);
+                          g_inv_std_rays, workspace, grad_packed, grads, h2_mask, nullptr, stream);
+}
+
+extern "C" int tt_render_bwd_geo_bounds(const float* packed, const tt_mlp_weights* w, const float* rays_o,
+                                        const float* rays_d, const float* t_starts, const float* t_ends,
+                                        const tt_render_cfg* cfg, const float* opacity, const float* depth,
+                                        const float* trans, const float* sdf, const float* sdf_grad,
+                                        const float* features, const float* g_opacity, const float* g_depth,
+                                        const float* g_rgb_fg, const float* g_z_variance, const float* g_normal_acc,
+                                        const float* g_weights, const float* g_sdf, const float* g_sdf_grad,
+                                        float* g_inv_std_rays, float* workspace, float* grad_packed,
+                                        const tt_mlp_grads* grads, const uint32_t* h2_mask,
+                                        const uint32_t* plane_bounds, void* stream) {
+    if (!plane_bounds) return TT_ERR_BAD_ARG;
+    return render_bwd_geo(packed, w, rays_o, rays_d, t_starts, t_ends, cfg, opacity, depth, trans, sdf, sdf_grad, features,
+                          g_opacity, g_depth, g_rgb_fg, g_z_variance, g_normal_acc, g_weights, g_sdf, g_sdf_grad,
+                          g_inv_std_rays, workspace, grad_packed, grads, h2_mask, plane_bounds, stream);
 }
 
 __global__ void k_interleave_ws(const float* __restrict__ g_sdf, const float* __restrict__ g_sdf_grad,
@@ -413,6 +433,6 @@
     p.grads = to_gptrs(grads);
     st = tt_plan_queue(&cfg, 4LL * cus, s, &p.geom, &p.n_items, &p.queue);
     if (st != TT_OK) return st;
-    launch_bwd_geo(p, tt_persistent_blocks(p.n_items, cus, 4), s);
+    launch_bwd_geo(p, tt_persistent_blocks(p.n_items, cus, 4), s, false);
     return tt_check_launch();
 }
diff --git a/triplaneturbo_amd/csrc/tt_backward_common.h b/triplaneturbo_amd/csrc/tt_backward_common.h
--- a/triplaneturbo_amd/csrc/tt_backward_common.h
+++ b/triplaneturbo_amd/csrc/tt_backward_common.h
@@ -803,34 +803,15 @@
         m1 = fmaxf(m1, fmaxf(__builtin_fabsf(v[1]), fmaxf(__builtin_fabsf(v[2]), __builtin_fabsf(v[3]))));
     }
     if (!out1) m0 = fmaxf(m0, m1);
-    __shared__ unsigned w[2];
-    if (threadIdx.x < 2) w[threadIdx.x] = 0u;
-    __syncthreads();
-    for (int o = 32; o > 0; o >>= 1) {
-        m0 = fmaxf(m0, __shfl_xor(m0, o));
-        m1 = fmaxf(m1, __shfl_xor(m1, o));
-    }
-    if ((threadIdx.x & 63) == 0) {
-        atomicMax(&w[0], __builtin_bit_cast(unsigned, m0));
-        atomicMax(&w[1], __builtin_bit_cast(unsigned, m1));
-    }
-    __syncthreads();
-    if (threadIdx.x == 0) {
-        if (w[0] > __hip_atomic_load(out0, __ATOMIC_RELAXED, __HIP_MEMORY_SCOPE_AGENT)) atomicMax(out0, w[0]);
-        if (out1 && w[1] > __hip_atomic_load(out1, __ATOMIC_RELAXED, __HIP_MEMORY_SCOPE_AGENT)) atomicMax(out1, w[1]);
-    }
-}
-static __global__ __launch_bounds__(256) void k_absmax1(const float* __restrict__ x, long long n, unsigned* __restrict__ out) {
+    block_raise_max(m0, m1, out0, out1);
+}
+static __global__ __launch_bounds__(256) void k_absmax1(const float* __restrict__ x, long long n, unsigned* __restrict__ out,
+                                                 const unsigned* __restrict__ hand_src, unsigned* __restrict__ hand_dst) {
     float m = 0.f;
     for (long long e = (long long)blockIdx.x * blockDim.x + threadIdx.x; e < n; e += (long long)gridDim.x * blockDim.x)
         m = fmaxf(m, __builtin_fabsf(x[e]));
-    for (int o = 32; o > 0; o >>= 1) m = fmaxf(m, __shfl_xor(m, o));
-    __shared__ unsigned w;
-    if (threadIdx.x == 0) w = 0u;
-    __syncthreads();
-    if ((threadIdx.x & 63) == 0) atomicMax(&w, __builtin_bit_cast(unsigned, m));
-    __syncthreads();
-    if (threadIdx.x == 0 && w > __hip_atomic_load(out, __ATOMIC_RELAXED, __HIP_MEMORY_SCOPE_AGENT)) atomicMax(out, w);
+    block_raise_max(m, 0.f, out, nullptr);
+    if (hand_src && blockIdx.x == 0 && threadIdx.x == 0) *hand_dst = *hand_src;
 }
 static inline unsigned absmax_blocks(long long n) {
     long long b = (n + 256 * 8 - 1) / (256 * 8);
diff --git a/triplaneturbo_amd/csrc/tt_backward_tex.hip b/triplaneturbo_amd/csrc/tt_backward_tex.hip
--- a/triplaneturbo_amd/csrc/tt_backward_tex.hip
+++ b/triplaneturbo_amd/csrc/tt_backward_tex.hip
@@ -357,7 +357,7 @@
     tile_stats_flush(st);
 }
 
-static void launch_bwd_tex(const BwdTexParams& p0, long long blocks, hipStream_t s) {
+static void launch_bwd_tex(const BwdTexParams& p0, long long blocks, hipStream_t s, const unsigned* plane_bounds) {
     BwdTexParams p = p0;
 #ifdef TT_TUNING
     p.phase_cycles = g_phase_cycles;
@@ -366,13 +366,15 @@
 #endif
     if (use_wg16(p.cfg)) {
         unsigned* bnd = reinterpret_cast<unsigned*>(p.queue) + TT_SLOT_BOUNDS;
-        launch_planes_bound(p.packed, p.cfg, 3, bnd + TT_BOUND_PLANES, s);
+        const unsigned* hand = plane_bounds && (p.g_rgb || p.g_features) ? plane_bounds + 1 : nullptr;
+        if (!hand) launch_planes_bound(p.packed, p.cfg, 3, bnd + TT_BOUND_PLANES, s);
         if (p.g_rgb)
             hipLaunchKernelGGL(k_absmax1, dim3(absmax_blocks(p.cfg.n_rays * 3)), dim3(256), 0, s, p.g_rgb,
-                               (long long)p.cfg.n_rays * 3, bnd + TT_BOUND_UP0);
+                               (long long)p.cfg.n_rays * 3, bnd + TT_BOUND_UP0, hand, bnd + TT_BOUND_PLANES);
         if (p.g_features) {
             const long long n = p.cfg.n_rays * p.cfg.n_samples * 3;
-            hipLaunchKernelGGL(k_absmax1, dim3(absmax_blocks(n)), dim3(256), 0, s, p.g_features, n, bnd + TT_BOUND_UP1);
+            hipLaunchKernelGGL(k_absmax1, dim3(absmax_blocks(n)), dim3(256), 0, s, p.g_features, n, bnd + TT_BOUND_UP1,
+                               p.g_rgb ? (const unsigned*)nullptr : hand, bnd + TT_BOUND_PLANES);
         }
     }
     tt_dispatch_prec(tt_prec_of_r(p.cfg.flags), [&](auto P) {
@@ -384,11 +386,10 @@
     });
 }
 
-extern "C" int tt_render_bwd_tex(const float* packed, const tt_mlp_weights* w, const float* rays_o,
-                                 const float* rays_d, const float* t_starts, const float* t_ends,
-                                 const tt_render_cfg* cfg, const float* weights, const float* features,
-                                 const float* g_rgb_fg, const float* g_features, float* grad_packed,
-                                 const tt_mlp_grads* grads, void* stream) {
+static int render_bwd_tex(const float* packed, const tt_mlp_weights* w, const float* rays_o, const float* rays_d,
+                          const float* t_starts, const float* t_ends, const tt_render_cfg* cfg, const float* weights,
+                          const float* features, const float* g_rgb_fg, const float* g_features, float* grad_packed,
+                          const tt_mlp_grads* grads, const uint32_t* plane_bounds, void* stream) {
     int st = tt_validate_cfg(cfg);
     if (st != TT_OK) return st;
     if (!packed || !w || !rays_o || !rays_d || !t_starts || !t_ends || !weights || !features || !grad_packed ||
@@ -411,8 +412,27 @@
     p.grads = to_gptrs(grads);
     st = tt_plan_queue(cfg, 4LL * cus, s, &p.geom, &p.n_items, &p.queue, 12);
     if (st != TT_OK) return st;
-    launch_bwd_tex(p, tt_persistent_blocks(p.n_items, cus, 4), s);
+    launch_bwd_tex(p, tt_persistent_blocks(p.n_items, cus, 4), s, plane_bounds);
     return tt_check_launch();
+}
+
+extern "C" int tt_render_bwd_tex(const float* packed, const tt_mlp_weights* w, const float* rays_o,
+                                 const float* rays_d, const float* t_starts, const float* t_ends,
+                                 const tt_render_cfg* cfg, const float* weights, const float* features,
+                                 const float* g_rgb_fg, const float* g_features, float* grad_packed,
+                                 const tt_mlp_grads* grads, void* stream) {
+    return render_bwd_tex(packed, w, rays_o, rays_d, t_starts, t_ends, cfg, weights, features, g_rgb_fg, g_features,
+                          grad_packed, grads, nullptr, stream);
+}
+
+extern "C" int tt_render_bwd_tex_bounds(const float* packed, const tt_mlp_weights* w, const float* rays_o,
+                                        const float* rays_d, const float* t_starts, const float* t_ends,
+                                        const tt_render_cfg* cfg, const float* weights, const float* features,
+                                        const float* g_rgb_fg, const float* g_features, float* grad_packed,
+                                        const tt_mlp_grads* grads, const uint32_t* plane_bounds, void* stream) {
+    if (!plane_bounds) return TT_ERR_BAD_ARG;
+    return render_bwd_tex(packed, w, rays_o, rays_d, t_starts, t_ends, cfg, weights, features, g_rgb_fg, g_features,
+                          grad_packed, grads, plane_bounds, stream);
 }
 
 extern "C" int tt_points_bwd_tex(const float* packed, const tt_mlp_weights* w, const float* points, int32_t n_batch,
@@ -443,6 +463,6 @@
     p.grads = to_gptrs(grads);
     st = tt_plan_queue(&cfg, 4LL * cus, s, &p.geom, &p.n_items, &p.queue);
     if (st != TT_OK) return st;
-    launch_bwd_tex(p, tt_persistent_blocks(p.n_items, cus, 4), s);
+    launch_bwd_tex(p, tt_persistent_blocks(p.n_items, cus, 4), s, nullptr);
     return tt_check_launch();
 }
diff --git a/triplaneturbo_amd/csrc/tt_device.h b/triplaneturbo_amd/csrc/tt_device.h
--- a/triplaneturbo_amd/csrc/tt_device.h
+++ b/triplaneturbo_amd/csrc/tt_device.h
@@ -23,6 +23,25 @@
 #define LIDX(r, hi) (((r) & 3) + 8 * ((r) >> 2) + 4 * (hi))
 
 #include "tt_mask.h"
+
+__device__ __forceinline__ void block_raise_max(float m0, float m1, unsigned* out0, unsigned* out1) {
+    __shared__ unsigned w[2];
+    if (threadIdx.x < 2) w[threadIdx.x] = 0u;
+    __syncthreads();
+    for (int o = 32; o > 0; o >>= 1) {
+        m0 = fmaxf(m0, __shfl_xor(m0, o));
+        m1 = fmaxf(m1, __shfl_xor(m1, o));
+    }
+    if ((threadIdx.x & 63) == 0) {
+        atomicMax(&w[0], __builtin_bit_cast(unsigned, m0));
+        atomicMax(&w[1], __builtin_bit_cast(unsigned, m1));
+    }
+    __syncthreads();
+    if (threadIdx.x == 0) {
+        if (w[0] > __hip_atomic_load(out0, __ATOMIC_RELAXED, __HIP_MEMORY_SCOPE_AGENT)) atomicMax(out0, w[0]);
+        if (out1 && w[1] > __hip_atomic_load(out1, __ATOMIC_RELAXED, __HIP_MEMORY_SCOPE_AGENT)) atomicMax(out1, w[1]);
+    }
+}
 
 struct MlpPtrs {
     const float* w1;
diff --git a/triplaneturbo_amd/csrc/tt_forward.hip b/triplaneturbo_amd/csrc/tt_forward.hip
--- a/triplaneturbo_amd/csrc/tt_forward.hip
+++ b/triplaneturbo_amd/csrc/tt_forward.hip
@@ -19,9 +19,9 @@
     }
 }
 
-template <bool UNPACK>
+template <bool UNPACK, bool BOUNDS = false>
 __global__ __launch_bounds__(256) void k_planes_pack(const float* __restrict__ src, float* __restrict__ dst, int H,
-                                                     int W, int n_copies, size_t copy_stride) {
+                                                     int W, int n_copies, size_t copy_stride, unsigned* bounds) {
     extern __shared__ float tile[];
     const int y = blockIdx.x, plane = blockIdx.y;
     const int k3 = plane % 3;
@@ -32,9 +32,12 @@
     float* nhwc = const_cast<float*>(nhwc_c);
     const int ws = W + 1;
     if (!UNPACK) {
+        float m = 0.f;
         for (int e = threadIdx.x; e < TT_C * W; e += blockDim.x) {
             int c = e / W, x = e - c * W;
-            tile[c * ws + x] = nchw[(size_t)c * HW + (size_t)y * W + x];
+            const float v = nchw[(size_t)c * HW + (size_t)y * W + x];
+            tile[c * ws + x] = v;
+            if (BOUNDS) m = fmaxf(m, __builtin_fabsf(v));
         }
         __syncthreads();
         for (int e = threadIdx.x; e < TT_C * W; e += blockDim.x) {
@@ -42,6 +45,7 @@
             rot_dst(k3, y, x, H, W, h, w);
             nhwc[((size_t)h * W + w) * TT_C + c] = tile[c * ws + x];
         }
+        if constexpr (BOUNDS) block_raise_max(m, 0.f, bounds + (plane % 6) / 3, nullptr);
     } else {
         for (int e = threadIdx.x; e < TT_C * W; e += blockDim.x) {
             int x = e >> 5, c = e & 31, h, w;
@@ -60,9 +64,9 @@
 }
 
 __host__ __device__ inline int pack4_row_stride(int W) { return W + (36 - W % 32) % 32; }
-template <bool UNPACK>
+template <bool UNPACK, bool BOUNDS = false>
 __global__ __launch_bounds__(256) void k_planes_pack4(const float* __restrict__ src, float* __restrict__ dst, int H,
-                                                      int W, int n_copies, size_t copy_stride) {
+                                                      int W, int n_copies, size_t copy_stride, unsigned* bounds) {
     extern __shared__ __attribute__((aligned(16))) float tile[];
     const int y = blockIdx.x, plane = blockIdx.y;
     const int k3 = plane % 3;
@@ -74,10 +78,14 @@
     const int RS = pack4_row_stride(W), W4 = W >> 2;
     const int c_lane = threadIdx.x & 31, x4_0 = threadIdx.x >> 5;
     if (!UNPACK) {
+        float m = 0.f;
         for (int e4 = threadIdx.x; e4 < TT_C * W4; e4 += 256) {
             const int c = e4 / W4, x4 = e4 - c * W4;
-            *reinterpret_cast<f32x4*>(tile + c * RS + 4 * x4) =
-                *reinterpret_cast<const f32x4*>(nchw_c + (size_t)c * HW + 4 * x4);
+            const f32x4 v = *reinterpret_cast<const f32x4*>(nchw_c + (size_t)c * HW + 4 * x4);
+            *reinterpret_cast<f32x4*>(tile + c * RS + 4 * x4) = v;
+            if (BOUNDS)
+                m = fmaxf(fmaxf(m, __builtin_fabsf(v[0])),
+                          fmaxf(__builtin_fabsf(v[1]), fmaxf(__builtin_fabsf(v[2]), __builtin_fabsf(v[3]))));
         }
         __syncthreads();
         for (int x4 = x4_0; x4 < W4; x4 += 8) {
@@ -89,6 +97,7 @@
                 nhwc[((size_t)h * W + w) * TT_C + c_lane] = v[j];
             }
         }
+        if constexpr (BOUNDS) block_raise_max(m, 0.f, bounds + (plane % 6) / 3, nullptr);
     } else {
         for (int x4 = x4_0; x4 < W4; x4 += 8) {
             f32x4 v;
@@ -646,21 +655,44 @@
     }
 }
 
-extern "C" int tt_planes_pack(const float* space_cache, float* packed, int32_t n_prompts, int32_t plane_h,
-                              int32_t plane_w, void* stream) {
+static int planes_pack(const float* space_cache, float* packed, int32_t n_prompts, int32_t plane_h, int32_t plane_w,
+                       unsigned* bounds, hipStream_t s) {
     if (!space_cache || !packed || n_prompts <= 0 || plane_h <= 0 || plane_w <= 0) return TT_ERR_BAD_ARG;
     if (plane_h != plane_w) return TT_ERR_UNSUPPORTED;
+    if (bounds) {
+        const int st = tt_zero_words(bounds, 2, s);
+        if (st != TT_OK) return st;
+    }
     dim3 grid(plane_h, n_prompts * 6);
     if (plane_w % 4 == 0 && ((uintptr_t)space_cache & 15) == 0) {
         size_t lds = (size_t)TT_C * pack4_row_stride(plane_w) * sizeof(float);
-        hipLaunchKernelGGL(k_planes_pack4<false>, grid, dim3(256), lds, (hipStream_t)stream, space_cache, packed,
-                           plane_h, plane_w, 1, (size_t)0);
+        if (bounds)
+            hipLaunchKernelGGL((k_planes_pack4<false, true>), grid, dim3(256), lds, s, space_cache, packed, plane_h,
+                               plane_w, 1, (size_t)0, bounds);
+        else
+            hipLaunchKernelGGL(k_planes_pack4<false>, grid, dim3(256), lds, s, space_cache, packed, plane_h, plane_w, 1,
+                               (size_t)0, (unsigned*)nullptr);
     } else {
         size_t lds = (size_t)TT_C * (plane_w + 1) * sizeof(float);
-        hipLaunchKernelGGL(k_planes_pack<false>, grid, dim3(256), lds, (hipStream_t)stream, space_cache, packed,
-                           plane_h, plane_w, 1, (size_t)0);
+        if (bounds)
+            hipLaunchKernelGGL((k_planes_pack<false, true>), grid, dim3(256), lds, s, space_cache, packed, plane_h,
+                               plane_w, 1, (size_t)0, bounds);
+        else
+            hipLaunchKernelGGL(k_planes_pack<false>, grid, dim3(256), lds, s, space_cache, packed, plane_h, plane_w, 1,
+                               (size_t)0, (unsigned*)nullptr);
     }
     return tt_check_launch();
+}
+
+extern "C" int tt_planes_pack(const float* space_cache, float* packed, int32_t n_prompts, int32_t plane_h,
+                              int32_t plane_w, void* stream) {
+    return planes_pack(space_cache, packed, n_prompts, plane_h, plane_w, nullptr, (hipStream_t)stream);
+}
+
+extern "C" int tt_planes_pack_bounds(const float* space_cache, float* packed, int32_t n_prompts, int32_t plane_h,
+                                     int32_t plane_w, uint32_t* bounds, void* stream) {
+    if (!bounds) return TT_ERR_BAD_ARG;
+    return planes_pack(space_cache, packed, n_prompts, plane_h, plane_w, bounds, (hipStream_t)stream);
 }
 
 extern "C" int tt_planes_unpack_grad(const float* grad_packed, float* grad_space_cache, int32_t n_prompts,
@@ -673,11 +705,11 @@
     if (plane_w % 4 == 0 && ((uintptr_t)grad_space_cache & 15) == 0) {
         size_t lds = (size_t)TT_C * pack4_row_stride(plane_w) * sizeof(float);
         hipLaunchKernelGGL(k_planes_pack4<true>, grid, dim3(256), lds, (hipStream_t)stream, grad_packed,
-                           grad_space_cache, plane_h, plane_w, n_copies, copy_stride);
+                           grad_space_cache, plane_h, plane_w, n_copies, copy_stride, (unsigned*)nullptr);
     } else {
         size_t lds = (size_t)TT_C * (plane_w + 1) * sizeof(float);
         hipLaunchKernelGGL(k_planes_pack<true>, grid, dim3(256), lds, (hipStream_t)stream, grad_packed,
-                           grad_space_cache, plane_h, plane_w, n_copies, copy_stride);
+                           grad_space_cache, plane_h, plane_w, n_copies, copy_stride, (unsigned*)nullptr);
     }
     return tt_check_launch();
 }
diff --git a/triplaneturbo_amd/csrc/tt_host.cpp b/triplaneturbo_amd/csrc/tt_host.cpp
--- a/triplaneturbo_amd/csrc/tt_host.cpp
+++ b/triplaneturbo_amd/csrc/tt_host.cpp
@@ -102,6 +102,12 @@
     return slot;
 }
 
+int tt_zero_words(unsigned* words, int n, hipStream_t stream) {
+    if (!words || n <= 0 || n > kSlotInts) return TT_ERR_BAD_ARG;
+    hipLaunchKernelGGL(k_zero_slot, dim3(1), dim3(n), 0, stream, reinterpret_cast<int*>(words));
+    return tt_check_launch();
+}
+
 extern "C" int tt_debug_poison_queue(void* stream) {
     for (int r = 0; r < kRing; ++r) {
         int* slot = tt_queue_counters((hipStream_t)stream);
diff --git a/triplaneturbo_amd/csrc/tt_host.h b/triplaneturbo_amd/csrc/tt_host.h
--- a/triplaneturbo_amd/csrc/tt_host.h
+++ b/triplaneturbo_amd/csrc/tt_host.h
@@ -101,4 +101,6 @@
                         const float* opacity, const float* depth, const float* g_opacity, const float* g_depth,
                         const float* g_rgb_fg, const float* g_z_variance, const float* g_normal_acc,
                         const float* g_weights, const float* g_sdf, const float* g_sdf_grad, float* g_inv_std_rays,
-                        float* ws, hipStream_t stream);
+                        float* ws, unsigned* up_bounds, const unsigned* hand_src, unsigned* hand_dst, hipStream_t stream);
+
+int tt_zero_words(unsigned* words, int n, hipStream_t stream);
diff --git a/triplaneturbo_amd/csrc/tt_march.hip b/triplaneturbo_amd/csrc/tt_march.hip
--- a/triplaneturbo_amd/csrc/tt_march.hip
+++ b/triplaneturbo_amd/csrc/tt_march.hip
@@ -229,6 +229,9 @@
     const float* inv_std_dev;
     float* g_inv_std_rays;
     float* ws;
+    unsigned* up_bounds;
+    const unsigned* hand_src;
+    unsigned* hand_dst;
 };
 
 struct BwdIn {
@@ -310,13 +313,19 @@
     return o;
 }
 
+__device__ __forceinline__ void march_bound(const f32x4& o, float& m0, float& m1) {
+    m0 = fmaxf(m0, __builtin_fabsf(o[0]));
+    m1 = fmaxf(m1, fmaxf(__builtin_fabsf(o[1]), fmaxf(__builtin_fabsf(o[2]), __builtin_fabsf(o[3]))));
+}
+
 template <int NP>
-__global__ __launch_bounds__(256) void k_march_bwd(MarchBwdParams p) {
+__global__ __launch_bounds__(256) __attribute__((amdgpu_waves_per_eu(NP == 2 ? 4 : 1))) void k_march_bwd(MarchBwdParams p) {
     const int lane = threadIdx.x & 63;
     const long long wave = (long long)blockIdx.x * (blockDim.x >> 6) + (threadIdx.x >> 6);
     const long long n_waves = (long long)gridDim.x * (blockDim.x >> 6);
     const int S = p.S;
     const float kstd = load_inv_std(p.inv_std_dev, p.inv_std);
+    float m0 = 0.f, m1 = 0.f;
     for (long long ray = wave; ray < p.n_rays; ray += n_waves) {
         RayBar rb;
         rb.dx = p.rays_d[ray * 3 + 0];
@@ -345,7 +354,10 @@
             for (int k = NP - 1; k >= 0; --k) {
                 const int si = 64 * k + 63 - lane;
                 const f32x4 o = march_pass_bwd(p, kstd, in[k], si < S, lane, rb, Rcarry, dk);
-                if (si < S) *reinterpret_cast<f32x4*>(p.ws + (ray * S + si) * 4) = o;
+                if (si < S) {
+                    *reinterpret_cast<f32x4*>(p.ws + (ray * S + si) * 4) = o;
+                    march_bound(o, m0, m1);
+                }
             }
         } else {
             for (int base = ((S - 1) / 64) * 64; base >= 0; base -= 64) {
@@ -354,7 +366,10 @@
                 const long long sidx = ray * S + (valid ? si : 0);
                 const BwdIn v = march_load_bwd(p, sidx);
                 const f32x4 o = march_pass_bwd(p, kstd, v, valid, lane, rb, Rcarry, dk);
-                if (valid) *reinterpret_cast<f32x4*>(p.ws + sidx * 4) = o;
+                if (valid) {
+                    *reinterpret_cast<f32x4*>(p.ws + sidx * 4) = o;
+                    march_bound(o, m0, m1);
+                }
             }
         }
         if (p.g_inv_std_rays) {
@@ -362,6 +377,8 @@
             if (lane == 0) p.g_inv_std_rays[ray] = dk;
         }
     }
+    if (p.up_bounds) block_raise_max(m0, m1, p.up_bounds, p.up_bounds + 1);
+    if (p.hand_src && blockIdx.x == 0 && threadIdx.x == 0) *p.hand_dst = *p.hand_src;
 }
 
 static unsigned march_blocks(long long n_rays) {
@@ -412,7 +429,8 @@
                         const float* opacity, const float* depth, const float* g_opacity, const float* g_depth,
                         const float* g_rgb_fg, const float* g_z_variance, const float* g_normal_acc,
                         const float* g_weights, const float* g_sdf, const float* g_sdf_grad, float* g_inv_std_rays,
-                        float* ws, hipStream_t stream) {
+                        float* ws, unsigned* up_bounds, const unsigned* hand_src, unsigned* hand_dst,
+                        hipStream_t stream) {
     MarchBwdParams p;
     p.rays_d = rays_d;
     p.t_starts = t_starts;
@@ -439,6 +457,9 @@
     p.g_inv_std_rays = g_inv_std_rays;
     p.ratio = cfg->cos_anneal_ratio;
     p.ws = ws;
+    p.up_bounds = up_bounds;
+    p.hand_src = hand_src;
+    p.hand_dst = hand_dst;
     const dim3 grid(march_blocks(cfg->n_rays)), blk(256);
     if (p.S <= 64)
         hipLaunchKernelGGL(k_march_bwd<1>, grid, blk, 0, stream, p);
@@ -464,17 +485,41 @@
                                z_variance, normal_acc, weights, trans, (hipStream_t)stream);
 }
 
+static int march_bwd(const float* rays_d, const float* t_starts, const float* t_ends, const tt_render_cfg* cfg,
+                     const float* opacity, const float* depth, const float* trans, const float* sdf,
+                     const float* sdf_grad, const float* features, const float* g_opacity, const float* g_depth,
+                     const float* g_rgb_fg, const float* g_z_variance, const float* g_normal_acc, const float* g_weights,
+                     const float* g_sdf, const float* g_sdf_grad, float* g_inv_std_rays, float* out_grad,
+                     uint32_t* out_bounds, void* stream) {
+    int st = tt_validate_cfg(cfg);
+    if (st != TT_OK) return st;
+    if (!rays_d || !t_starts || !t_ends || !opacity || !depth || !trans || !sdf || !sdf_grad || !features || !out_grad)
+        return TT_ERR_BAD_ARG;
+    return tt_launch_march_bwd(rays_d, t_starts, t_ends, cfg, sdf, sdf_grad, features, trans, opacity, depth,
+                               g_opacity, g_depth, g_rgb_fg, g_z_variance, g_normal_acc, g_weights, g_sdf, g_sdf_grad,
+                               g_inv_std_rays, out_grad, out_bounds, nullptr, nullptr, (hipStream_t)stream);
+}
+
 extern "C" int tt_march_bwd(const float* rays_d, const float* t_starts, const float* t_ends, const tt_render_cfg* cfg,
                             const float* opacity, const float* depth, const float* trans, const float* sdf,
                             const float* sdf_grad, const float* features, const float* g_opacity,
                             const float* g_depth, const float* g_rgb_fg, const float* g_z_variance,
                             const float* g_normal_acc, const float* g_weights, const float* g_sdf,
                             const float* g_sdf_grad, float* g_inv_std_rays, float* out_grad, void* stream) {
-    int st = tt_validate_cfg(cfg);
-    if (st != TT_OK) return st;
-    if (!rays_d || !t_starts || !t_ends || !opacity || !depth || !trans || !sdf || !sdf_grad || !features || !out_grad)
-        return TT_ERR_BAD_ARG;
-    return tt_launch_march_bwd(rays_d, t_starts, t_ends, cfg, sdf, sdf_grad, features, trans, opacity, depth,
-                               g_opacity, g_depth, g_rgb_fg, g_z_variance, g_normal_acc, g_weights, g_sdf, g_sdf_grad,
-                               g_inv_std_rays, out_grad, (hipStream_t)stream);
-}
+    return march_bwd(rays_d, t_starts, t_ends, cfg, opacity, depth, trans, sdf, sdf_grad, features, g_opacity, g_depth,
+                     g_rgb_fg, g_z_variance, g_normal_acc, g_weights, g_sdf, g_sdf_grad, g_inv_std_rays, out_grad, nullptr,
+                     stream);
+}
+
+extern "C" int tt_march_bwd_bounds(const float* rays_d, const float* t_starts, const float* t_ends,
+                                   const tt_render_cfg* cfg, const float* opacity, const float* depth,
+                                   const float* trans, const float* sdf, const float* sdf_grad, const float* features,
+                                   const float* g_opacity, const float* g_depth, const float* g_rgb_fg,
+                                   const float* g_z_variance, const float* g_normal_acc, const float* g_weights,
+                                   const float* g_sdf, const float* g_sdf_grad, float* g_inv_std_rays, float* out_grad,
+                                   uint32_t* out_bounds, void* stream) {
+    if (!out_bounds) return TT_ERR_BAD_ARG;
+    return march_bwd(rays_d, t_starts, t_ends, cfg, opacity, depth, trans, sdf, sdf_grad, features, g_opacity, g_depth,
+                     g_rgb_fg, g_z_variance, g_normal_acc, g_weights, g_sdf, g_sdf_grad, g_inv_std_rays, out_grad,
+                     out_bounds, stream);
+}
diff --git a/triplaneturbo_amd/functional.py b/triplaneturbo_amd/functional.py
--- a/triplaneturbo_amd/functional.py
+++ b/triplaneturbo_amd/functional.py
@@ -75,7 +75,8 @@
                   rays_d: Tensor, t_starts: Tensor, t_ends: Tensor, bg_color: Tensor, camera_distances: Tensor,
                   c2w: Tensor, rc: ops.RenderConfig, training: bool = True,
                   normal_direction: str = "camera", comp_rgb_bg: Optional[Tensor] = None,
-                  packed: Optional[Tensor] = None, eval_termination_eps: float = 0.0) -> Dict[str, Tensor]:
+                  packed: Optional[Tensor] = None, eval_termination_eps: float = 0.0,
+                  plane_bounds: Optional[Tensor] = None) -> Dict[str, Tensor]:
     B, Hh, Ww, _ = rays_o.shape
     n_rays = B * Hh * Ww
     S = t_starts.shape[1]
@@ -88,7 +89,7 @@
                                 transmittance_eps=eval_termination_eps, weight_eps=eval_termination_eps / max(S, 1))
     else:
         r = ops.render_samples(space_cache, sdf_w, feat_w, ro, rd, t_starts, t_ends, Hh * Ww, rc, image_w=Ww,
-                               packed=packed)
+                               packed=packed, plane_bounds=plane_bounds)
     opacity, depth, comp_rgb_fg, z_variance = r["opacity"], r["depth"], r["rgb_fg"], r["z_variance"]
 
     if normal_direction not in ("camera", "front", "world"):
diff --git a/triplaneturbo_amd/ops.py b/triplaneturbo_amd/ops.py
--- a/triplaneturbo_amd/ops.py
+++ b/triplaneturbo_amd/ops.py
@@ -171,12 +171,16 @@
     fwd_mask: bool = True
 
 
-def planes_pack(space_cache: Tensor) -> Tensor:
+def planes_pack(space_cache: Tensor, with_bounds: bool = False):
     space_cache = _chk(space_cache, "space_cache", (None, 6, 32, None, None))
     P, _, _, H, W = space_cache.shape
     out = torch.empty((P, 6, H, W, 32), device=space_cache.device, dtype=torch.float32)
-    _launch("tt_planes_pack", space_cache, out, P, H, W)
-    return out
+    if not with_bounds:
+        _launch("tt_planes_pack", space_cache, out, P, H, W)
+        return out
+    bounds = torch.empty(2, device=space_cache.device, dtype=torch.int32)
+    _launch("tt_planes_pack_bounds", space_cache, out, P, H, W, bounds)
+    return out, bounds
 
 
 def planes_unpack_grad(grad_packed: Tensor) -> Tensor:
@@ -191,17 +195,21 @@
 class _PackPlanesFn(torch.autograd.Function):
 
     @staticmethod
-    def forward(ctx, space_cache):
-        return planes_pack(space_cache)
+    def forward(ctx, space_cache, with_bounds=False):
+        if not with_bounds:
+            return planes_pack(space_cache)
+        packed, bounds = planes_pack(space_cache, with_bounds=True)
+        ctx.mark_non_differentiable(bounds)
+        return packed, bounds
 
     @staticmethod
     @torch.autograd.function.once_differentiable
-    def backward(ctx, grad_packed):
-        return planes_unpack_grad(grad_packed.contiguous())
-
-
-def pack_planes(space_cache: Tensor) -> Tensor:
-    return _PackPlanesFn.apply(space_cache)
+    def backward(ctx, grad_packed, _g_bounds=None):
+        return planes_unpack_grad(grad_packed.contiguous()), None
+
+
+def pack_planes(space_cache: Tensor, with_bounds: bool = False):
+    return _PackPlanesFn.apply(space_cache, bool(with_bounds))
 
 
 def query_points(packed: Tensor, sdf_w: Sequence[Tensor], feat_w: Optional[Sequence[Tensor]], points: Tensor,
@@ -353,6 +361,15 @@
     return inv_std, t.data_ptr()
 
 
+def _chk_bounds(t: Optional[Tensor], name: str = "plane_bounds") -> Optional[Tensor]:
+    if t is None:
+        return None
+    _chk_gpu(t, name)
+    if t.dtype != torch.int32 or tuple(t.shape) != (2,) or not t.is_contiguous():
+        raise ValueError(f"{name} must be a contiguous (2,) int32 tensor")
+    return t
+
+
 def _make_cfg(packed: Tensor, n_rays: int, rays_per_view: int, n_samples: int, rc: RenderConfig,
               per_sample: bool, image_w: int = 0, stats_row: int = 0) -> "_lib.RenderCfg":
     P, _, H, W, _ = packed.shape
@@ -511,15 +528,20 @@
 def march_backward_raw(rays_d: Tensor, t_starts: Tensor, t_ends: Tensor, fwd: dict, sdf: Tensor, sdf_grad: Tensor,
                        features: Tensor, rc: RenderConfig, g_opacity=None, g_depth=None, g_rgb_fg=None,
                        g_z_variance=None, g_normal_acc=None, g_weights=None, g_sdf=None, g_sdf_grad=None,
-                       out: Optional[Tensor] = None, g_inv_std_rays: Optional[Tensor] = None):
+                       out: Optional[Tensor] = None, g_inv_std_rays: Optional[Tensor] = None,
+                       out_bounds: Optional[Tensor] = None):
     n_rays, S = t_starts.shape
     cfg = _march_cfg(rc, n_rays, S)
     if out is None:
         out = torch.empty((n_rays * S, 4), device=rays_d.device, dtype=torch.float32)
     gs = [_contig(t)
           for t in (g_opacity, g_depth, g_rgb_fg, g_z_variance, g_normal_acc, g_weights, g_sdf, g_sdf_grad)]
-    _launch("tt_march_bwd", rays_d, t_starts, t_ends, cfg, fwd["opacity"], fwd["depth"], fwd["trans"], sdf, sdf_grad,
-            features, *gs, g_inv_std_rays, out, label="tt_march_bwd")
+    args = (rays_d, t_starts, t_ends, cfg, fwd["opacity"], fwd["depth"], fwd["trans"], sdf, sdf_grad, features, *gs,
+            g_inv_std_rays, out)
+    if out_bounds is None:
+        _launch("tt_march_bwd", *args, label="tt_march_bwd")
+    else:
+        _launch("tt_march_bwd_bounds", *args, _chk_bounds(out_bounds, "out_bounds"), label="tt_march_bwd")
     return out
 
 
@@ -541,7 +563,8 @@
 
     @staticmethod
     def forward(ctx, packed, w1, w2, w3, v1, v2, v3, rays_o, rays_d, t_starts, t_ends, rays_per_view, rc,
-                image_w, inv_std_t=None):
+                image_w, inv_std_t=None, plane_bounds=None):
+        plane_bounds = _chk_bounds(plane_bounds)
         need_grad = any(ctx.needs_input_grad[:7]) or ctx.needs_input_grad[14]
         if inv_std_t is not None:
             rc = dataclasses.replace(rc, inv_std_t=inv_std_t.detach())
@@ -552,10 +575,12 @@
         ctx.rc = rc
         ctx.image_w = image_w
         ctx.inv_std_shape = None if inv_std_t is None else tuple(inv_std_t.shape)
+        ctx.has_plane_bounds = plane_bounds is not None
         if need_grad:
             ctx.save_for_backward(packed, w1, w2, w3, v1, v2, v3, rays_o, rays_d, t_starts, t_ends, raw["opacity"],
                                   raw["depth"], raw["trans"], raw["weights"], raw["features"], raw["sdf"],
-                                  raw["sdf_grad"], *([raw["h2_mask"]] if rc.fwd_mask else []))
+                                  raw["sdf_grad"], *([raw["h2_mask"]] if rc.fwd_mask else []),
+                                  *([plane_bounds] if ctx.has_plane_bounds else []))
         ctx.mark_non_differentiable(raw["trans"])
         return (raw["opacity"], raw["depth"], raw["rgb_fg"], raw["z_variance"], raw["normal_acc"], raw["weights"],
                 raw["sdf"], raw["sdf_grad"], raw["features"], raw["trans"])
@@ -565,7 +590,9 @@
     def backward(ctx, g_op, g_depth, g_rgb, g_zvar, g_nacc, g_weights, g_sdf, g_sdf_grad, g_features, _g_trans):
         (packed, w1, w2, w3, v1, v2, v3, rays_o, rays_d, t_starts, t_ends, opacity, depth, trans, weights,
          features, sdf, sdf_grad) = ctx.saved_tensors[:18]
-        h2_mask = ctx.saved_tensors[18:]
+        rest = list(ctx.saved_tensors[18:])
+        plane_bounds = rest.pop() if ctx.has_plane_bounds else None
+        h2_mask = rest
         n_rays, S = t_starts.shape
         cfg = _make_cfg(packed, n_rays, ctx.rays_per_view, S, ctx.rc, True, ctx.image_w, stats_row=1)
         cfg_tex = _make_cfg(packed, n_rays, ctx.rays_per_view, S, ctx.rc, True, ctx.image_w, stats_row=2)
@@ -581,37 +608,46 @@
         g_k_rays = None
         if ctx.needs_input_grad[14]:
             g_k_rays = torch.empty((n_rays,), device=packed.device, dtype=torch.float32)
-        _launch("tt_render_bwd_geo_h2mask" if h2_mask else "tt_render_bwd_geo", packed, wst, rays_o, rays_d, t_starts,
-                t_ends, cfg, opacity, depth, trans, sdf, sdf_grad, features, g_op, g_depth, g_rgb, g_zvar, g_nacc,
-                g_weights, g_sdf, g_sdf_grad, g_k_rays, workspace, grad_packed, gst, *h2_mask, label="tt_render_bwd_geo")
-        _launch("tt_render_bwd_tex", packed, wst, rays_o, rays_d, t_starts, t_ends, cfg_tex, weights, features, g_rgb,
-                g_features, grad_packed, gst, label="tt_render_bwd_tex")
+        geo = (packed, wst, rays_o, rays_d, t_starts, t_ends, cfg, opacity, depth, trans, sdf, sdf_grad, features, g_op,
+               g_depth, g_rgb, g_zvar, g_nacc, g_weights, g_sdf, g_sdf_grad, g_k_rays, workspace, grad_packed, gst)
+        tex = (packed, wst, rays_o, rays_d, t_starts, t_ends, cfg_tex, weights, features, g_rgb, g_features, grad_packed,
+               gst)
+        if plane_bounds is not None:
+            _launch("tt_render_bwd_geo_bounds", *geo, h2_mask[0] if h2_mask else None, plane_bounds,
+                    label="tt_render_bwd_geo")
+            _launch("tt_render_bwd_tex_bounds", *tex, plane_bounds, label="tt_render_bwd_tex")
+        else:
+            _launch("tt_render_bwd_geo_h2mask" if h2_mask else "tt_render_bwd_geo", *geo, *h2_mask,
+                    label="tt_render_bwd_geo")
+            _launch("tt_render_bwd_tex", *tex, label="tt_render_bwd_tex")
         g_packed = None
         if ctx.needs_input_grad[0]:
             g_packed = grad_packed[0] if copies == 1 else grad_packed.sum(dim=0)
         g_inv_std = None
         if g_k_rays is not None:
             g_inv_std = g_k_rays.double().sum().float().reshape(ctx.inv_std_shape)
-        return (g_packed, *gw, None, None, None, None, None, None, None, g_inv_std)
+        return (g_packed, *gw, None, None, None, None, None, None, None, g_inv_std, None)
 
 
 def render_samples(space_cache: Optional[Tensor], sdf_w: Sequence[Tensor], feat_w: Sequence[Tensor], rays_o: Tensor,
                    rays_d: Tensor, t_starts: Tensor, t_ends: Tensor, rays_per_view: int, rc: RenderConfig,
-                   image_w: int = 0, packed: Optional[Tensor] = None):
+                   image_w: int = 0, packed: Optional[Tensor] = None, plane_bounds: Optional[Tensor] = None):
     names = ("opacity", "depth", "rgb_fg", "z_variance", "normal_acc", "weights", "sdf", "sdf_grad", "features",
              "trans")
     if packed is None:
-        packed = pack_planes(space_cache)
+        packed, plane_bounds = pack_planes(space_cache, with_bounds=True)
     outs = _TriplaneRenderFn.apply(packed, sdf_w[0], sdf_w[1], sdf_w[2], feat_w[0], feat_w[1], feat_w[2],
                                    rays_o.contiguous(), rays_d.contiguous(), t_starts.contiguous(),
-                                   t_ends.contiguous(), rays_per_view, rc, int(image_w), rc.inv_std_t)
+                                   t_ends.contiguous(), rays_per_view, rc, int(image_w), rc.inv_std_t, plane_bounds)
     return dict(zip(names, outs))
 
 
 @torch.no_grad()
 def decode_rays(packed: Tensor, sdf_w: Sequence[Tensor], feat_w: Optional[Sequence[Tensor]], rays_o: Tensor,
                 rays_d: Tensor, t_starts: Tensor, t_ends: Tensor, rays_per_view: int, rc: RenderConfig,
-                need_normal: bool = False, need_features: bool = False, image_w: int = 0):
+                need_normal: bool = False, need_features: bool = False, image_w: int = 0,
+                plane_bounds: Optional[Tensor] = None):
+    _chk_bounds(plane_bounds)
     packed, rays_o, rays_d, t_starts, t_ends = _ray_args(packed, rays_o, rays_d, t_starts, t_ends)
     n_rays, S = t_starts.shape
     cfg = _make_cfg(packed, n_rays, rays_per_view, S, rc, False, image_w)
diff --git a/triplaneturbo_amd/renderer.py b/triplaneturbo_amd/renderer.py
--- a/triplaneturbo_amd/renderer.py
+++ b/triplaneturbo_amd/renderer.py
@@ -182,11 +182,12 @@
         assert B % P == 0, "batch of views must be a multiple of the number of prompts"
         grad_on = torch.is_grad_enabled()
         packed = kwargs.pop("packed", None)
+        plane_bounds = kwargs.pop("plane_bounds", None)
         tile_sb = kwargs.pop("tile_sb", None)
         pitch_w = kwargs.pop("ray_pitch_w", None)
         if packed is None:
             with (torch.enable_grad() if grad_on else torch.no_grad()):
-                packed = ops.pack_planes(space_cache)
+                packed, plane_bounds = ops.pack_planes(space_cache, with_bounds=True)
         importance_sampled = t_starts is None
         if t_starts is None:
             t_starts, t_ends = self.sample(space_cache, rays_o, rays_d, packed=packed)
@@ -207,7 +208,8 @@
             out = functional.volume_render(space_cache, sw, fw, rays_o, rays_d, t_starts, t_ends, bg_color,
                                            camera_distances, c2w, rc, training=self.training,
                                            normal_direction=self.cfg.normal_direction, comp_rgb_bg=comp_rgb_bg,
-                                           packed=packed, eval_termination_eps=self.eval_termination_eps)
+                                           packed=packed, eval_termination_eps=self.eval_termination_eps,
+                                           plane_bounds=plane_bounds)
         if self.training:
             out["inv_std"] = self.variance.inv_std
         return out
@@ -265,7 +267,7 @@
         sc = kwargs.get("space_cache")
         if torch.is_tensor(sc) and kwargs.get("packed") is None:
             with (torch.enable_grad() if torch.is_grad_enabled() else torch.no_grad()):
-                kwargs["packed"] = ops.pack_planes(sc)
+                kwargs["packed"], kwargs["plane_bounds"] = ops.pack_planes(sc, with_bounds=True)
         ds = self.cfg.global_downsample
         g_o = F.interpolate(rays_o.permute(0, 3, 1, 2).contiguous(), (H // ds, W // ds), mode="bilinear").permute(0, 2, 3, 1)
         g_d = F.interpolate(rays_d.permute(0, 3, 1, 2).contiguous(), (H // ds, W // ds), mode="bilinear").permute(0, 2, 3, 1)
```

Result: no change. 8.176 million (median of 6 runs) (+0.9%).
